# zacharie12/Hypernet-image-captioning

Measured on AMD Instinct MI355X. Metric: training images/sec at 1/2/4/8 MI355X, Flickr30k GRU+hypernet bs=128, higher is better.
Workload: dtype f32; 1 GPU; Flickr30k-shaped GRU+additive-attention decoder + hypernet (3 style domains), full training step (fwd, CE, bwd, clip 5.0, Adam); per_gpu_batch=128, global_batch=128, T=20, P=49, D=2048, F=200, E=200, H=200, V=9684, hypernet_params=144906720, parallelism=dp1, launch=eager, next_theta_in_adam_pass=True, next_precompute_beside_adam=True, spinup_steps=0, deterministic_gradients=True

## Files before the change

hypernet-image-captioning_amd/caphn/_lib.py:

```python
import ctypes as C
import os

import torch

_HERE = os.path.dirname(os.path.abspath(__file__))
LIB_PATH = os.environ.get("CAPHN_LIB_PATH") or os.path.join(_HERE, "libcaphn.so")
MAX_HEADS = 8

c_fp = C.c_void_p


class HyperDesc(C.Structure):
    _fields_ = [("he", C.c_int), ("n_heads", C.c_int),
                ("k", C.c_int * MAX_HEADS), ("w", C.c_int * MAX_HEADS),
                ("base_w0", c_fp), ("base_b0", c_fp), ("base_w2", c_fp), ("base_b2", c_fp),
                ("w1", c_fp * MAX_HEADS), ("b1", c_fp * MAX_HEADS),
                ("w2", c_fp * MAX_HEADS), ("b2", c_fp * MAX_HEADS),
                ("d_in", C.c_int), ("d_mid", C.c_int)]


class HyperGrads(C.Structure):
    _fields_ = [("g_base_w0", c_fp), ("g_base_b0", c_fp), ("g_base_w2", c_fp), ("g_base_b2", c_fp),
                ("g_w1", c_fp * MAX_HEADS), ("g_b1", c_fp * MAX_HEADS),
                ("g_w2", c_fp * MAX_HEADS), ("g_b2", c_fp * MAX_HEADS),
# ... 90 lines not shown
    "caphn_colsum_workspace_bytes": (C.c_size_t, [C.c_int, C.c_int]),
    "caphn_linear_wgrad_f32": (C.c_int, [C.c_int, C.c_int, C.c_int, c_fp, C.c_int, c_fp, C.c_int, c_fp, C.c_int, c_fp, c_fp, c_fp]),
    "caphn_colsum_f32": (C.c_int, [C.c_int, C.c_int, c_fp, C.c_int, c_fp, c_fp, c_fp]),
    "caphn_hyper_acts_floats": (C.c_int, [C.POINTER(HyperDesc)]),
    "caphn_hyper_forward": (C.c_int, [C.POINTER(HyperDesc), c_fp, c_fp, c_fp, c_fp]),
    "caphn_hyper_backward_workspace_bytes": (C.c_size_t, [C.POINTER(HyperDesc)]),
    "caphn_hyper_backward": (C.c_int, [C.POINTER(HyperDesc), c_fp, c_fp, C.POINTER(HyperGrads), c_fp, c_fp]),
    "caphn_decoder_workspace_bytes": (C.c_size_t, [C.POINTER(DecoderDims)]),
    "caphn_decoder_forward": (C.c_int, [C.POINTER(DecoderDims), C.POINTER(DecoderParams), c_fp, c_fp,
                                        c_fp, c_fp, c_fp, c_fp]),
    "caphn_decoder_pair_prep": (C.c_int, [C.POINTER(DecoderDims), C.POINTER(DecoderParams), c_fp, c_fp]),
    "caphn_decoder_pair_pack_desc": (C.c_int, [C.POINTER(DecoderDims), c_fp, C.POINTER(PairPack)]),
    "caphn_decoder_precompute": (C.c_int, [C.POINTER(DecoderDims), C.POINTER(DecoderParams), c_fp, c_fp, c_fp, c_fp]),
    "caphn_decoder_inputs": (C.c_int, [C.POINTER(DecoderDims), C.POINTER(DecoderParams), c_fp, c_fp, c_fp]),
    "caphn_decoder_lookup": (C.c_int, [C.POINTER(DecoderDims), C.POINTER(DecoderParams), c_fp, c_fp, c_fp]),
    "caphn_decoder_prepare_rows": (C.c_int, [C.POINTER(DecoderDims), c_fp, C.c_int64, c_fp, c_fp]),
    "caphn_decoder_forward_sampled": (C.c_int, [C.POINTER(DecoderDims), C.POINTER(DecoderParams), c_fp, c_fp,
                                                C.c_char_p, c_fp, c_fp, c_fp, c_fp]),
    "caphn_decoder_forward_sampled_train": (C.c_int, [C.POINTER(DecoderDims), C.POINTER(DecoderParams), c_fp, c_fp,
                                                      C.c_char_p, c_fp, c_fp, c_fp, c_fp]),
    "caphn_decoder_backward": (C.c_int, [C.POINTER(DecoderDims), C.POINTER(DecoderParams), c_fp, c_fp,
                                         c_fp, c_fp, C.POINTER(DecoderGrads), c_fp, c_fp]),
    "caphn_decoder_hyper_backward": (C.c_int, [C.POINTER(DecoderDims), C.POINTER(DecoderParams), c_fp, c_fp,
                                               c_fp, c_fp, C.POINTER(DecoderGrads), c_fp,
                                               C.POINTER(HyperDesc), c_fp, C.POINTER(HyperGrads), c_fp, c_fp]),
    "caphn_decoder_backward_milestone": (C.c_int, [C.c_int, c_fp]),
    "caphn_decoder_search_workspace_bytes": (C.c_size_t, [C.POINTER(DecoderDims), C.POINTER(SearchCfg)]),
    "caphn_decoder_search_begin": (C.c_int, [C.POINTER(DecoderDims), C.POINTER(DecoderParams), C.POINTER(SearchCfg),
                                             c_fp, c_fp, c_fp, c_fp]),
    "caphn_decoder_search_steps": (C.c_int, [C.POINTER(DecoderDims), C.POINTER(DecoderParams), C.POINTER(SearchCfg),
                                             C.c_int, C.c_int, c_fp, c_fp, c_fp, c_fp]),
    "caphn_decoder_search_result": (C.c_int, [C.POINTER(DecoderDims), C.POINTER(SearchCfg), C.c_int, c_fp, c_fp,
                                              c_fp, c_fp, c_fp, c_fp, c_fp, c_fp]),
    "caphn_plain_workspace_bytes": (C.c_size_t, [C.POINTER(PlainDims)]),
    "caphn_plain_forward": (C.c_int, [C.POINTER(PlainDims), C.POINTER(PlainParams), c_fp, c_fp, c_fp, c_fp, c_fp, c_fp, c_fp]),
    "caphn_bahdanau_fwd": (C.c_int, [C.c_int] * 4 + [c_fp] * 8),
    "caphn_bahdanau_bwd": (C.c_int, [C.c_int] * 4 + [c_fp] * 12),
    "caphn_plain_forward_sampled": (C.c_int, [C.POINTER(PlainDims), C.POINTER(PlainParams), c_fp, c_fp, c_fp, C.c_uint64, c_fp, c_fp,
                                               c_fp, c_fp]),
    "caphn_plain_backward": (C.c_int, [C.POINTER(PlainDims), C.POINTER(PlainParams), c_fp, c_fp, c_fp, c_fp, c_fp,
                                       C.POINTER(PlainGrads), c_fp, c_fp]),
    "caphn_layernorm_fwd": (C.c_int, [C.c_int, C.c_int, c_fp, c_fp, c_fp, C.c_float, c_fp, c_fp, c_fp, c_fp]),
    "caphn_layernorm_bwd_workspace_bytes": (C.c_size_t, [C.c_int, C.c_int]),
    "caphn_layernorm_bwd": (C.c_int, [C.c_int, C.c_int, c_fp, c_fp, c_fp, c_fp, c_fp, c_fp, c_fp, c_fp, c_fp, c_fp]),
    "caphn_attention_supported": (C.c_int, [C.POINTER(AttnDims)]),
    "caphn_attention_fwd": (C.c_int, [C.POINTER(AttnDims), c_fp, c_fp, c_fp, c_fp, c_fp, c_fp, c_fp, c_fp]),
    "caphn_attention_bwd": (C.c_int, [C.POINTER(AttnDims), c_fp, c_fp, c_fp, c_fp, c_fp, c_fp, c_fp, c_fp, c_fp, c_fp, c_fp, c_fp]),
    "caphn_ce_workspace_bytes": (C.c_size_t, [C.c_int]),
    "caphn_cross_entropy_rows": (C.c_int, [C.c_int, C.c_int, c_fp, c_fp, C.c_int64, c_fp, C.c_int, c_fp, c_fp, c_fp]),
    "caphn_cross_entropy_rows_ld": (C.c_int, [C.c_int, C.c_int, C.c_int, c_fp, c_fp, C.c_int64, c_fp, C.c_int, c_fp, c_fp, c_fp]),
    "caphn_cross_entropy_finish": (C.c_int, [C.c_int, c_fp, c_fp, c_fp, c_fp]),
    "caphn_decoder_profile_ptr": (C.c_void_p, [C.POINTER(DecoderDims), c_fp]),
    "caphn_decoder_rowcount_ptr": (C.c_void_p, [C.POINTER(DecoderDims), c_fp]),
    "caphn_cross_entropy_fwd_bwd": (C.c_int, [C.c_int, C.c_int, c_fp, c_fp, C.c_int64, c_fp, c_fp, C.c_int, c_fp, c_fp]),
    "caphn_embedding_gather": (C.c_int, [C.c_int, C.c_int, c_fp, c_fp, c_fp, c_fp]),
    "caphn_embedding_scatter_add": (C.c_int, [C.c_int, C.c_int, c_fp, c_fp, c_fp, c_fp]),
    "caphn_embedding_scatter_add_v": (C.c_int, [C.c_int, C.c_int, C.c_int, c_fp, c_fp, c_fp, c_fp]),
    "caphn_sumsq_blocks": (C.c_int, [C.c_size_t]),
    "caphn_sumsq_f32": (C.c_int, [C.c_size_t, c_fp, c_fp, c_fp]),
    "caphn_rank_sumsq_f32": (C.c_int, [C.c_int, C.c_int, C.c_int, c_fp, C.c_size_t, c_fp, C.c_size_t,
                                       c_fp, c_fp, c_fp]),
    "caphn_rank_sumsq_multi_f32": (C.c_int, [C.c_int, C.c_int, C.POINTER(C.c_int), C.POINTER(C.c_int),
                                             C.POINTER(C.c_void_p), C.POINTER(C.c_size_t), C.POINTER(C.c_void_p),
                                             C.POINTER(C.c_size_t), c_fp, c_fp, c_fp]),
    "caphn_grad_norm_workspace_bytes": (C.c_size_t, [C.c_size_t, C.c_int, C.c_int]),
    "caphn_grad_norm_coef": (C.c_int, [C.c_size_t, c_fp, C.c_int, C.c_int, C.POINTER(C.c_int), C.POINTER(C.c_int),
                                       C.POINTER(C.c_void_p), C.POINTER(C.c_size_t), C.POINTER(C.c_void_p),
                                       C.POINTER(C.c_size_t), C.c_double, C.c_double, c_fp, c_fp, c_fp]),
    "caphn_clip_coef": (C.c_int, [C.c_int, c_fp, c_fp, C.c_double, C.c_double, c_fp, c_fp]),
    "caphn_adam_dense_f32": (C.c_int, [C.c_size_t, c_fp, c_fp, c_fp, c_fp, c_fp, C.POINTER(AdamHParams), c_fp]),
    "caphn_grad_norm_adam_dense": (C.c_int, [C.c_size_t, c_fp, c_fp, c_fp, c_fp, C.c_int, C.c_int, C.POINTER(C.c_int), C.POINTER(C.c_int),
                                             C.POINTER(C.c_void_p), C.POINTER(C.c_size_t), C.POINTER(C.c_void_p), C.POINTER(C.c_size_t),
                                             C.c_double, C.c_double, c_fp, c_fp, C.POINTER(AdamHParams), C.c_int, c_fp, c_fp, c_fp, c_fp]),
    "caphn_grad_norm_multi_workspace_bytes": (C.c_size_t, [C.c_int, C.POINTER(C.c_size_t), C.c_int, C.c_int]),
    "caphn_grad_norm_multi": (C.c_int, [C.c_int, C.POINTER(C.c_void_p), C.POINTER(C.c_size_t), C.c_int, C.c_int,
                                        C.POINTER(C.c_int), C.POINTER(C.c_int), C.POINTER(C.c_void_p), C.POINTER(C.c_size_t),
                                        C.POINTER(C.c_void_p), C.POINTER(C.c_size_t), C.c_double, C.c_double, c_fp, c_fp, c_fp]),
    "caphn_adam_multi_f32": (C.c_int, [C.c_int, C.POINTER(C.c_void_p), C.POINTER(C.c_void_p), C.POINTER(C.c_void_p),
                                       C.POINTER(C.c_void_p), C.POINTER(C.c_size_t), c_fp, C.POINTER(AdamHParams), c_fp]),
    "caphn_adam_rank_f32": (C.c_int, [C.c_int, C.c_int, C.c_int, c_fp, c_fp, c_fp, c_fp, C.c_size_t,
                                      c_fp, C.c_size_t, c_fp, C.POINTER(AdamHParams), c_fp]),
    "caphn_adam_rank_gemv_f32": (C.c_int, [C.c_int, C.c_int, C.c_int, c_fp, c_fp, c_fp, c_fp, C.c_size_t,
                                           c_fp, C.c_size_t, c_fp, C.POINTER(AdamHParams), c_fp, c_fp, c_fp, c_fp]),
    "caphn_adam_rank_multi_f32": (C.c_int, [C.c_int, C.c_int, C.POINTER(RankJob), c_fp, C.POINTER(AdamHParams), c_fp]),
    "caphn_adam_rank_lag_f32": (C.c_int, [C.c_int, C.c_int, C.c_int, c_fp, c_fp, c_fp, c_fp, c_fp, c_fp, C.POINTER(AdamHParams),
                                          C.POINTER(RankLag), c_fp, c_fp, c_fp, c_fp]),
    "caphn_adam_rank_lag_multi_f32": (C.c_int, [C.c_int, C.c_int, C.POINTER(RankJob), C.POINTER(RankLag), c_fp,
                                                C.POINTER(AdamHParams), c_fp]),
    "caphn_adam_rank_settle_f32": (C.c_int, [C.c_int, C.c_int, c_fp, c_fp, C.c_float, C.c_float, C.POINTER(RankLag), c_fp]),
    "caphn_lazy_moments_period": (C.c_int, []),
    "caphn_hyper_forward_acts": (C.c_int, [C.POINTER(HyperDesc), c_fp, c_fp, c_fp]),
    "caphn_stream_copy_f32": (C.c_int, [C.c_size_t, c_fp, c_fp, c_fp]),
    "caphn_outer_f32": (C.c_int, [C.c_int, C.c_int, c_fp, c_fp, c_fp, c_fp]),
    "caphn_tune": (C.c_int, [C.c_int, C.c_int]),
}

_ERR = {-1: "CAPHN_EINVAL (bad argument)", -2: "CAPHN_ELAUNCH (HIP launch error)",
        -3: "CAPHN_ELIMIT (problem exceeds a hardware limit, e.g. 160 KB LDS)",
        -4: "CAPHN_ETIMEOUT (a recurrent kernel's partner workgroup never answered: that step's results are NaN; "
            "sticky until caphn_device_error(1))"}

_lib = None


class CaphnError(RuntimeError):
    pass
# ... 42 lines not shown
```

hypernet-image-captioning_amd/caphn/ops.py:

```python
import ctypes as C
from dataclasses import dataclass
from typing import Dict, List, Optional, Sequence, Tuple

import torch

from . import _lib as L

GEMM_BIAS, GEMM_RELU, GEMM_ACCUM, GEMM_MASK, GEMM_LRELU = 1, 2, 4, 8, 16


def _f32(*shape, device):
    return torch.empty(*shape, dtype=torch.float32, device=device)


def gemm(a: torch.Tensor, b: torch.Tensor, ta: bool = False, tb: bool = False,
         bias: Optional[torch.Tensor] = None, relu: bool = False, out: Optional[torch.Tensor] = None,
         accumulate: bool = False, mask: Optional[torch.Tensor] = None, splitk: int = 1, lrelu: bool = False) -> torch.Tensor:
    lib = L.load()
    assert a.dim() == 2 and b.dim() == 2 and a.stride(1) == 1 and b.stride(1) == 1
    M, K = (a.shape[1], a.shape[0]) if ta else (a.shape[0], a.shape[1])
    N, Kb = (b.shape[0], b.shape[1]) if tb else (b.shape[1], b.shape[0])
    if K != Kb:
        raise L.CaphnError(f"gemm inner dims differ: {K} vs {Kb}")
    if out is None:
# ... 522 lines not shown
    lib = L.load()
    cd = dims.c()
    ps = _dec_struct(L.DecoderParams, dims, params)
    gs = _dec_struct(L.DecoderGrads, dims, grads)
    L.check(lib.caphn_decoder_backward(C.byref(cd), C.byref(ps), L.ptr(features), L.ptr(captions, torch.int64),
                                       L.ptr(dlogits), L.ptr(dalphas, allow_none=True), C.byref(gs),
                                       C.c_void_p(ws.data_ptr()), L.stream_ptr()), "caphn_decoder_backward")


def cross_entropy_fwd_bwd(logits: torch.Tensor, targets: torch.Tensor, ignore_index: int = 0,
                          dlogits: Optional[torch.Tensor] = None, leave_ignored_rows: bool = False):
    lib = L.load()
    V = logits.shape[-1]
    rows = logits.numel() // V
    if dlogits is None:
        dlogits = torch.empty_like(logits)
    ws = torch.empty(lib.caphn_ce_workspace_bytes(rows), dtype=torch.uint8, device=logits.device)
    out = _f32(2, device=logits.device)
    L.check(lib.caphn_cross_entropy_fwd_bwd(rows, V, L.ptr(logits), L.ptr(targets.reshape(-1), torch.int64),
                                            ignore_index, L.ptr(dlogits), L.ptr(out), int(leave_ignored_rows),
                                            C.c_void_p(ws.data_ptr()),
                                            L.stream_ptr()), "caphn_cross_entropy_fwd_bwd")
    return out, dlogits


def cross_entropy_rows(logits: torch.Tensor, targets: torch.Tensor, ignore_index: int, dlogits: torch.Tensor,
                       ws: torch.Tensor, leave_ignored_rows: bool = False, n_valid_ptr: Optional[int] = None, V: Optional[int] = None) -> None:
    lib = L.load()
    ld = logits.shape[-1]
    rows = logits.numel() // ld
    V = ld if V is None else int(V)
    assert dlogits.shape[-1] == ld and V <= ld
    L.check(lib.caphn_cross_entropy_rows_ld(rows, V, ld, L.ptr(logits), L.ptr(targets.reshape(-1), torch.int64), ignore_index,
                                            L.ptr(dlogits), int(leave_ignored_rows),
                                            C.c_void_p(n_valid_ptr) if n_valid_ptr else None, C.c_void_p(ws.data_ptr()),
                                            L.stream_ptr()), "caphn_cross_entropy_rows_ld")


def cross_entropy_finish(rows: int, ws: torch.Tensor, out: torch.Tensor, n_valid_ptr: Optional[int] = None) -> None:
    lib = L.load()
    L.check(lib.caphn_cross_entropy_finish(rows, C.c_void_p(n_valid_ptr) if n_valid_ptr else None, L.ptr(out),
                                           C.c_void_p(ws.data_ptr()), L.stream_ptr()), "caphn_cross_entropy_finish")


def ce_workspace(rows: int, device) -> torch.Tensor:
    return torch.empty(L.load().caphn_ce_workspace_bytes(rows), dtype=torch.uint8, device=device)


def decoder_rowcount_ptr(dims: DecDims, ws: torch.Tensor) -> int:
    cd = dims.c()
    return int(L.load().caphn_decoder_rowcount_ptr(C.byref(cd), C.c_void_p(ws.data_ptr())) or 0)


def embedding_gather(table: torch.Tensor, idx: torch.Tensor) -> torch.Tensor:
    lib = L.load()
    rows, E = idx.numel(), table.shape[1]
    out = _f32(rows, E, device=table.device)
    L.check(lib.caphn_embedding_gather(rows, E, L.ptr(table), L.ptr(idx.reshape(-1), torch.int64), L.ptr(out),
                                       L.stream_ptr()), "caphn_embedding_gather")
    return out


def embedding_scatter_add(g: torch.Tensor, idx: torch.Tensor, table_grad: torch.Tensor) -> None:
    lib = L.load()
    rows, E = g.shape
    L.check(lib.caphn_embedding_scatter_add_v(rows, E, int(table_grad.shape[0]), L.ptr(g), L.ptr(idx.reshape(-1), torch.int64),
                                              L.ptr(table_grad), L.stream_ptr()), "caphn_embedding_scatter_add_v")


def sumsq_partials(x: torch.Tensor, partial: Optional[torch.Tensor] = None) -> torch.Tensor:
    lib = L.load()
    nb = lib.caphn_sumsq_blocks(x.numel())
    if partial is None:
        partial = torch.empty(nb, dtype=torch.float64, device=x.device)
    L.check(lib.caphn_sumsq_f32(x.numel(), L.ptr(x), L.ptr(partial, torch.float64), L.stream_ptr()), "caphn_sumsq_f32")
    return partial[:nb]


def rank_sumsq(gfac: torch.Tensor, afac: torch.Tensor, acc: torch.Tensor) -> None:
    lib = L.load()
    R, rows = gfac.shape
    k = afac.shape[1]
    ws = torch.empty(2 * R * R, dtype=torch.float64, device=gfac.device)
    L.check(lib.caphn_rank_sumsq_f32(R, rows, k, gfac.data_ptr(), gfac.stride(0), afac.data_ptr(), afac.stride(0),
                                     L.ptr(acc, torch.float64), L.ptr(ws, torch.float64), L.stream_ptr()),
            "caphn_rank_sumsq_f32")


def rank_sumsq_multi(pairs, acc: torch.Tensor, ws: Optional[torch.Tensor] = None) -> None:
    lib = L.load()
    n = len(pairs)
    R = pairs[0][0].shape[0]
    if ws is None:
        ws = torch.empty(2 * R * R * n, dtype=torch.float64, device=acc.device)
    rows = (C.c_int * n)(*[g.shape[1] for g, _ in pairs])
    ks = (C.c_int * n)(*[a.shape[1] for _, a in pairs])
    gp = (C.c_void_p * n)(*[g.data_ptr() for g, _ in pairs])
    ap = (C.c_void_p * n)(*[a.data_ptr() for _, a in pairs])
    ldg = (C.c_size_t * n)(*[g.stride(0) for g, _ in pairs])
    lda = (C.c_size_t * n)(*[a.stride(0) for _, a in pairs])
    L.check(lib.caphn_rank_sumsq_multi_f32(R, n, rows, ks, gp, ldg, ap, lda, L.ptr(acc, torch.float64),
                                           L.ptr(ws, torch.float64), L.stream_ptr()), "caphn_rank_sumsq_multi_f32")


class GradNorm:

# ... 466 lines not shown
```

hypernet-image-captioning_amd/csrc/decoder.hip:

```cpp
#include "common.h"
#include "decoder_internal.h"
#include "gemm_internal.h"
#include <algorithm>
#include <initializer_list>
#include <mutex>

int g_tune_deterministic = 0;
int g_tune_rec_pair = 1;
int g_tune_rec_rotate = 1;
int g_tune_vocab_order = 1;
int g_tune_branch_mask = 7;
int g_tune_splitk_target = 1280;
int g_tune_chain_main = 0;
int g_tune_hops = 0;
int g_tune_fork = 4;
int g_tune_join_chain = 0;
int g_tune_sk_dhs = 0, g_tune_sk_vocab_w = 0;
#define RUN(x) do { int _rc = (x); if (_rc != CAPHN_OK) return _rc; } while (0)

namespace {

struct Side {
    hipStream_t st[3];
    enum { D_FORK = 0, D_JOIN = 1, D_X = 4, D_MS = 10, D_PRE_F = 14, D_PRE_ALL = 15, D_COUNT = 16 };
    struct Dep { hipEvent_t ev; unsigned seq = 0; bool by_value = false; };
    Dep deps[D_COUNT];
    unsigned* vals = nullptr;
    unsigned counter = 0;
    bool values = false;
    bool pre_valid = false;
    const void* pre_ws = nullptr;
    bool ready = false, on = false;
    bool forked[3] = {false, false, false};
    hipStream_t main = nullptr;
    int init() {
        if (ready) return CAPHN_OK;
        static std::mutex mu;
        std::lock_guard<std::mutex> lock(mu);
        if (ready) return CAPHN_OK;
        for (auto& s : st) if (hipStreamCreateWithFlags(&s, hipStreamNonBlocking) != hipSuccess) return CAPHN_ELAUNCH;
        for (auto& d : deps) if (hipEventCreateWithFlags(&d.ev, hipEventDisableTiming) != hipSuccess) return CAPHN_ELAUNCH;
        void* p = nullptr;
        if (hipMalloc(&p, sizeof(unsigned) * D_COUNT) == hipSuccess && hipMemset(p, 0, sizeof(unsigned) * D_COUNT) == hipSuccess)
            vals = static_cast<unsigned*>(p);
        else (void)hipGetLastError();
        ready = true;
        return CAPHN_OK;
    }
    int post(int slot, hipStream_t from) {
        Dep& d = deps[slot];
        if (values) {
            d.seq = ++counter; d.by_value = true;
            return hipStreamWriteValue32(from, vals + slot, d.seq, 0) == hipSuccess ? CAPHN_OK : CAPHN_ELAUNCH;
        }
        d.by_value = false;
        return hipEventRecord(d.ev, from) == hipSuccess ? CAPHN_OK : CAPHN_ELAUNCH;
    }
    int await(int slot, hipStream_t to) {
        Dep& d = deps[slot];
        if (d.by_value)
            return hipStreamWaitValue32(to, vals + slot, d.seq, hipStreamWaitValueGte, 0xffffffffu) == hipSuccess ? CAPHN_OK : CAPHN_ELAUNCH;
        return hipStreamWaitEvent(to, d.ev, 0) == hipSuccess ? CAPHN_OK : CAPHN_ELAUNCH;
    }
    int milestone(int k, hipStream_t from) {
        if (init() != CAPHN_OK) return CAPHN_ELAUNCH;
        return post(D_MS + k, from);
    }
    int begin(hipStream_t m, bool enable) {
        main = m; on = enable;
// ... 15 lines not shown
        if (post(D_FORK, main) != CAPHN_OK) return CAPHN_ELAUNCH;
        for (int i : ids) {
            if (!((g_tune_branch_mask >> i) & 1)) continue;
            if (await(D_FORK, st[i]) != CAPHN_OK) return CAPHN_ELAUNCH;
            forked[i] = true;
        }
        return CAPHN_OK;
    }
    int jointo(int i) {
        if (!on || !((g_tune_branch_mask >> i) & 1)) return CAPHN_OK;
        forked[i] = false;
        if (post(D_JOIN + i, st[i]) != CAPHN_OK) return CAPHN_ELAUNCH;
        return await(D_JOIN + i, main);
    }
    int join_into(int i, int j) {
        if (!on || !((g_tune_branch_mask >> i) & 1)) return CAPHN_OK;
        if (!((g_tune_branch_mask >> j) & 1)) return jointo(i);
        forked[i] = false;
        if (post(D_JOIN + i, st[i]) != CAPHN_OK) return CAPHN_ELAUNCH;
        return await(D_JOIN + i, st[j]);
    }
    struct Scope {
        Side& s;
        explicit Scope(Side& side) : s(side) {}
        ~Scope() { for (int i = 0; i < 3; ++i) if (s.on && s.forked[i]) (void)s.jointo(i); }
    };
    hipStream_t xfrom[6] = {nullptr, nullptr, nullptr, nullptr, nullptr, nullptr};
    int record(int k, hipStream_t from) {
        if (!on) return CAPHN_OK;
        xfrom[k] = from;
        return post(D_X + k, from);
    }
    int wait(int k, hipStream_t to) {
        if (!on || xfrom[k] == to) return CAPHN_OK;
        return await(D_X + k, to);
    }
    int dep(hipStream_t from, hipStream_t to, int k) {
        if (!on || from == to) return CAPHN_OK;
        if (post(D_X + k, from) != CAPHN_OK) return CAPHN_ELAUNCH;
        return await(D_X + k, to);
    }
};
constexpr int MAX_DEVICES = 64;
Side g_sides[MAX_DEVICES];
inline Side* side_here() {
    int dev = 0;
    if (hipGetDevice(&dev) != hipSuccess || dev < 0 || dev >= MAX_DEVICES) return nullptr;
    return &g_sides[dev];
}

struct Ws {
    size_t Y1, f, meanf, h0, c0, Waf, G, Xe, Xg, Hs, Hprev, gates, hn, Cs, Cprev, uah, alphas, idx;
    size_t dHs, dgi, dgh, duah, de, dh0, dc0, ctx, dctx, dXe, dWaf, dmeanf, df, dY1, apart, vtmp, colws, colws_s[3], prof, rowmap;
    size_t xch, xch_floats;
    size_t wp;
    size_t H0s, dH0, h0L, dcarry, tgi, tgh, tmpA, tmpB;
    size_t Lin[CAPHN_MAX_DEC_LAYERS - 1], Lgates[CAPHN_MAX_DEC_LAYERS - 1], Lhn[CAPHN_MAX_DEC_LAYERS - 1],
           Ldgi[CAPHN_MAX_DEC_LAYERS - 1], Ldgh[CAPHN_MAX_DEC_LAYERS - 1];
    int L1;
    size_t total;
    int npc, pchunk, NG, arows;
};
inline bool use_pair(const caphn_decoder_dims* d) {
    const int NG = d->cell == CAPHN_CELL_LSTM ? 4 : 3;
    return g_tune_rec_pair && d->T > 1 && d->layers <= 1 && caphn_rec_pair_resident_gates(d->P, d->H, NG) >= 0;
}

inline size_t up4(size_t v) { return (v + 3) & ~(size_t)3; }

inline Ws layout(const caphn_decoder_dims* d) {
    Ws w;
    const size_t B = d->B, T = d->T, P = d->P, F = d->F, E = d->E, H = d->H, V = d->V, D = d->D;
    const bool lstm = d->cell == CAPHN_CELL_LSTM, raw = d->raw_features != 0;
    const size_t NG = lstm ? 4 : 3;
    w.NG = (int)NG;
    size_t o = 0;
    auto take = [&](size_t n) { size_t r = o; o += up4(n); return r; };
    w.Y1 = take(raw ? 0 : B * P * F); w.f = take(raw ? 0 : B * P * F); w.meanf = take(B * F); w.h0 = take(B * H);
    w.c0 = take(lstm ? B * H : 0);
    w.Waf = take(B * P * H); w.G = take(B * P * NG * H); w.Xe = take(B * T * (E + F)); w.Xg = take(B * T * NG * H);
    w.Hs = take(B * T * H); w.Hprev = take(B * T * H); w.gates = take(B * T * NG * H); w.hn = take(lstm ? 0 : B * T * H);
    w.Cs = take(lstm ? B * T * H : 0); w.Cprev = take(lstm ? B * T * H : 0);
    w.uah = take(B * T * H); w.alphas = take(B * T * P); w.idx = take(2 * B * T);
    w.dHs = take(B * T * H); w.dgi = take(B * T * NG * H); w.dgh = take(lstm ? 0 : B * T * NG * H); w.duah = take(B * T * H);
    w.de = take(B * T * P); w.dh0 = take(B * H); w.dc0 = take(lstm ? B * H : 0);
    w.ctx = w.Xe + E; w.dctx = take(raw ? 0 : B * T * F);
    w.dXe = take(B * T * E); w.dWaf = take(B * P * H); w.dmeanf = take(raw ? 0 : 2 * B * F); w.df = take(raw ? 0 : B * P * F);
    w.dY1 = take(raw ? 0 : B * P * F);
    w.pchunk = 1; w.npc = (int)((P + w.pchunk - 1) / w.pchunk);
    const size_t arows = std::max<size_t>(std::max<size_t>(w.npc, (size_t)caphn_rec_bwd_groups((int)P, (int)H)),
                                          (size_t)caphn_rec_pair_bwd_groups((int)P, (int)H));
    w.arows = (int)arows;
    w.apart = take(B * arows * (H + 1)); w.vtmp = take(H + 1);
    size_t cs = 0;
    auto need = [&](size_t M, size_t N) { cs = std::max(cs, caphn_colsum_workspace_bytes((int)M, (int)N) / sizeof(float)); };
    need(B * T, V); need(B * T, NG * H); need(B * T, H); need(B * P, H); need(B * P, F); need(B, H);
    need(B * arows, H + 1);
    if (d->layers > 1) need(B * (T + 1), 3 * H);
    w.colws = take(cs);
    {
        size_t c2 = 0;
        auto need2 = [&](size_t M, size_t N) { c2 = std::max(c2, caphn_colsum_workspace_bytes((int)M, (int)N) / sizeof(float)); };
        need2(B * T, NG * H); need2(B * T, H); need2(B * P, H); need2(B * P, F); need2(B, H); need2(B * arows, H + 1);
        if (d->layers > 1) need2(B * (T + 1), 3 * H);
        for (int i = 0; i < 3; ++i) w.colws_s[i] = take(c2);
    }
    w.prof = take(64);
    w.rowmap = take(B * T + 4);
    w.xch_floats = caphn_rec_pair_xch_bytes((int)B, (int)P, (int)H) / sizeof(float);
    w.xch = take(2 * w.xch_floats);
    o = (o + 31) & ~(size_t)31;
    w.wp = take(caphn_rec_pair_wp_floats((int)H, (int)NG));
    w.L1 = d->layers > 1 ? d->layers - 1 : 0;
    {
        const size_t on = w.L1 > 0 ? 1 : 0, S = T + 1;
        w.H0s = take(on * B * T * H); w.dH0 = take(on * B * T * H); w.h0L = take(on * B * H); w.dcarry = take(on * B * H);
        w.tgi = take(on * B * 3 * H); w.tgh = take(on * B * 3 * H); w.tmpA = take(on * B * H); w.tmpB = take(on * B * H);
        for (int l = 0; l < CAPHN_MAX_DEC_LAYERS - 1; ++l) {
            const size_t u = l < w.L1 ? 1 : 0;
            w.Lin[l] = take(u * B * S * H); w.Lgates[l] = take(u * B * S * 3 * H); w.Lhn[l] = take(u * B * S * H);
            w.Ldgi[l] = take(u * B * S * 3 * H); w.Ldgh[l] = take(u * B * S * 3 * H);
        }
    }
    w.total = o;
    (void)D;
    return w;
}

__global__ __launch_bounds__(1024) void valid_rows_kernel(int n, const int64_t* __restrict__ tgt, int64_t ignore, int* __restrict__ map) {
    __shared__ int wsum[16];
    __shared__ int base_s;
    const int tid = threadIdx.x, lane = tid & 63, wave = tid >> 6;
    if (tid == 0) base_s = 0;
    __syncthreads();
    for (int c0 = 0; c0 < n; c0 += 1024) {
        const int i = c0 + tid;
        const int v = (i < n && tgt[i] != ignore) ? 1 : 0;
        const unsigned long long ball = __ballot(v);
        const int before = __popcll(ball & ((1ull << lane) - 1ull));
        if (lane == 0) wsum[wave] = __popcll(ball);
        __syncthreads();
        int woff = 0, tot = 0;
        for (int q = 0; q < 16; ++q) { if (q < wave) woff += wsum[q]; tot += wsum[q]; }
        const int base = base_s;
        if (v) map[4 + base + woff + before] = i;
        __syncthreads();
        if (tid == 0) base_s = base + tot;
        __syncthreads();
    }
    if (tid == 0) map[0] = base_s;
}

__global__ void copy2_kernel(const float* __restrict__ src, int n, float* __restrict__ a, float* __restrict__ b) {
    const int i = blockIdx.x * blockDim.x + threadIdx.x;
    if (i < n) a[i] = src[i];
    else if (i == n) b[0] = src[n];
}

__global__ __launch_bounds__(256) void teacher_inputs_kernel(int T, int E, const int64_t* __restrict__ caps, const float* __restrict__ table,
                                                            int64_t* __restrict__ idx, float* __restrict__ out, int ostride) {
    const int i = blockIdx.x, t = i % T;
    const int64_t id = t < 2 ? (int64_t)-1 : caps[i - 1];
    if (threadIdx.x == 0) idx[i] = id;
    for (int e = threadIdx.x; e < E; e += 256) out[(size_t)i * ostride + e] = id < 0 ? 0.f : table[(size_t)id * E + e];
}

inline bool dims_ok(const caphn_decoder_dims* d) {
    if (d && !(d->dropout_p >= 0.f && d->dropout_p < 1.f)) return false;
    if (!(d && d->B > 0 && d->T > 0 && d->P > 0 && d->D > 0 && d->F > 0 && d->E > 0 && d->H > 0 && d->V > 0)) return false;
    if (d->cell != CAPHN_CELL_GRU && d->cell != CAPHN_CELL_LSTM) return false;
    if (d->raw_features && d->F != d->D) return false;
    if (d->layers < 0 || d->layers > CAPHN_MAX_DEC_LAYERS) return false;
    if (d->layers > 1 && d->cell != CAPHN_CELL_GRU) return false;
    if (d->logits_ld != 0 && d->logits_ld < d->V) return false;
    return true;
}
inline bool layer_params_ok(const caphn_decoder_dims* d, const caphn_decoder_params* p) {
    for (int l = 0; l + 1 < d->layers; ++l)
        if (!p->lw_ih[l] || !p->lw_hh[l] || !p->lb_ih[l] || !p->lb_hh[l]) return false;
    return true;
}

inline int pick_splitk(int M, int N, int K) {
    if (g_tune_deterministic) return 1;
    const long t128 = (long)((M + 127) / 128) * ((N + 127) / 128);
    if (t128 >= 1024) return 1;
    const long t64 = (long)((M + 63) / 64) * ((N + 63) / 64);
    const int nslab = (K + 31) / 32;
    long s = (g_tune_splitk_target + t64 - 1) / t64;
    if (s > nslab / 8) s = nslab / 8;
    if (s < 1) s = 1;
    if (s > 64) s = 64;
    return (int)s;
}


inline int gemm_auto(int ta, int tb, int M, int N, int K, const float* A, int lda, const float* B, int ldb,
                     float* C, int ldc, const float* bias, int flags, hipStream_t s,
                     const int* rowmap = nullptr, int map_mode = 0, bool prezeroed = false) {
    int sk = pick_splitk(M, N, K);
    if (rowmap) {
        if (sk > 1 && !prezeroed) {
            if (ldc == N) { RUN(caphn_zero_f32(C, (size_t)M * N, s)); }
            else if (hipMemset2DAsync(C, sizeof(float) * ldc, 0, sizeof(float) * N, M, s) != hipSuccess) return CAPHN_ELAUNCH;
        }
        return caphn_gemm_mapped(ta, tb, M, N, K, A, lda, B, ldb, C, ldc, bias, flags, sk, rowmap + 4, rowmap, map_mode, s);
    }
    if (sk > 1 && (flags & ~CAPHN_GEMM_BIAS) == 0) {
        if (prezeroed) {
        } else if (ldc == N) {
            RUN(caphn_zero_f32(C, (size_t)M * N, s));
        } else {
            if (hipMemset2DAsync(C, sizeof(float) * ldc, 0, sizeof(float) * N, M, s) != hipSuccess) return CAPHN_ELAUNCH;
        }
        return caphn_gemm_f32(ta, tb, M, N, K, A, lda, B, ldb, C, ldc, bias, nullptr, 0, flags, sk, s);
    }
    return caphn_gemm_f32(ta, tb, M, N, K, A, lda, B, ldb, C, ldc, bias, nullptr, 0, flags, 1, s);
}

inline int wgrad_bias(int M, int N, int K, const float* A, int lda, const float* B, int ldb, float* dW, int ldc, float* db,
                      const int* rowmap, void* cws, hipStream_t s, bool prezeroed) {
    int sk = pick_splitk(M, N, K);
    if (rowmap && g_tune_sk_vocab_w > 0 && !g_tune_deterministic) sk = g_tune_sk_vocab_w;
    return caphn_gemm_tn_colsum(M, N, K, A, lda, B, ldb, dW, ldc, db, sk, rowmap, cws, prezeroed, s);
}

static int decoder_precompute(const caphn_decoder_dims* d, const caphn_decoder_params* p, const Ws& w, float* ws,
                              const float* features, const float** f_out, hipStream_t s, int parts = 3, bool mark = false) {
    const int B = d->B, P = d->P, D = d->D, F = d->F, E = d->E, H = d->H;
    const bool lstm = d->cell == CAPHN_CELL_LSTM, raw = d->raw_features != 0;
    const int BP = B * P, GH = w.NG * H, EF = E + F;
    const float* f = raw ? features : ws + w.f;
    *f_out = f;
    if ((parts & 1) && !raw) {
        RUN(caphn_gemm_f32(0, 1, BP, F, D, features, D, p->fc0_w, D, ws + w.Y1, F, p->fc0_b, nullptr, 0,
                           CAPHN_GEMM_BIAS | CAPHN_GEMM_RELU, 1, s));
        RUN(caphn_gemm_f32(0, 1, BP, F, F, ws + w.Y1, F, p->fc2_w, F, ws + w.f, F, p->fc2_b, nullptr, 0, CAPHN_GEMM_BIAS, 1, s));
    }
    Side* sdp = side_here();
    if (!sdp) return CAPHN_ELAUNCH;
    Side& sd = *sdp;
    RUN(sd.begin(s, g_tune_fork != 0 && (parts & 1) && !mark));
    Side::Scope scope(sd);
    if (mark) RUN(sd.post(Side::D_PRE_F, s));
    if (parts & 1) {
        RUN(sd.fork_many({0, 1}));
        RUN(caphn_launch_init_state(B, P, F, H, f, p->inith_w, p->inith_b, lstm ? p->initc_w : nullptr, lstm ? p->initc_b : nullptr,
                                    ws + w.meanf, ws + w.h0, lstm ? ws + w.c0 : nullptr, sd.s(0)));
        RUN(caphn_gemm_f32(0, 1, BP, H, F, f, F, p->Wa_w, F, ws + w.Waf, H, p->Wa_b, nullptr, 0, CAPHN_GEMM_BIAS, 1, sd.s(1)));
    }
    if (parts & 2)
        RUN(caphn_gemm_f32(0, 1, BP, GH, F, f, F, p->w_ih + E, EF, ws + w.G, GH, nullptr, nullptr, 0, 0, 1, s));
    if (parts & 1) { RUN(sd.jointo(0)); RUN(sd.jointo(1)); }
    return CAPHN_OK;
}

__global__ __launch_bounds__(256) void next_token_kernel(int B, int T, int V, int mode, int col,
                                                         const int64_t* __restrict__ caps, const float* __restrict__ logits,
                                                         int64_t* __restrict__ idx_out, int ostride) {
    __shared__ float bv[4];
    __shared__ int bi[4];
    const int b = blockIdx.x, tid = threadIdx.x;
    int64_t* idx = idx_out + (size_t)b * ostride - b;
    if (mode == 0) { if (tid == 0) idx[b] = -1; return; }
    if (mode == 1) { if (tid == 0) idx[b] = caps[(size_t)b * T + col]; return; }
    const float* row = logits + ((size_t)b * T + col) * V;
    float best = -INFINITY; int besti = 0x7fffffff;
    for (int v = tid; v < V; v += 256) { const float x = row[v]; if (x > best) { best = x; besti = v; } }
#pragma unroll
    for (int m = 32; m >= 1; m >>= 1) {
        const float ob = __shfl_xor(best, m, 64); const int oi = __shfl_xor(besti, m, 64);
        if (ob > best || (ob == best && oi < besti)) { best = ob; besti = oi; }
    }
    if ((tid & 63) == 0) { bv[tid >> 6] = best; bi[tid >> 6] = besti; }
    __syncthreads();
    if (tid == 0) {
// ... 7 lines not shown
    const int B = d->B, H = d->H, G3 = 3 * d->H;
    const float* in = hin; int in_ld = hin_ld;
    for (int l = 0; l < w.L1; ++l) {
        const bool last = l == w.L1 - 1;
        float* out = last ? hout : ws + ((l & 1) ? w.tmpB : w.tmpA);
        const int out_ld = last ? hout_ld : H;
        RUN(caphn_gemm_f32(0, 1, B, G3, H, in, in_ld, p->lw_ih[l], H, ws + w.tgi, G3, p->lb_ih[l], nullptr, 0, CAPHN_GEMM_BIAS, 1, s));
        RUN(caphn_gemm_f32(0, 1, B, G3, H, in, in_ld, p->lw_hh[l], H, ws + w.tgh, G3, p->lb_hh[l], nullptr, 0, CAPHN_GEMM_BIAS, 1, s));
        LayerFwdArgs a;
        a.B = B; a.H = H; a.S = d->T + 1; a.slot = slot;
        a.gi = ws + w.tgi; a.gh = ws + w.tgh; a.hin = in; a.hin_ld = in_ld; a.hout = out; a.hout_ld = out_ld;
        a.sin = ws + w.Lin[l]; a.sgates = ws + w.Lgates[l]; a.shn = ws + w.Lhn[l];
        if (last && slot > 0) { a.drop_p = d->dropout_p; a.drop_seed = d->dropout_seed; a.T = d->T; a.t = slot - 1; }
        RUN(caphn_launch_layer_gru_fwd(a, s));
        in = out; in_ld = out_ld;
    }
    return CAPHN_OK;
}

static int layers_backward(const caphn_decoder_dims* d, const caphn_decoder_params* p, const Ws& w, float* ws, int slot,
                           const float* d1, int d1_ld, const float* d2, float* dout, int dout_ld, hipStream_t s) {
    const int B = d->B, H = d->H, G3 = 3 * d->H, S = d->T + 1;
    for (int l = w.L1 - 1; l >= 0; --l) {
        float* o = l == 0 ? dout : ws + ((l & 1) ? w.tmpB : w.tmpA);
        const int o_ld = l == 0 ? dout_ld : H;
        LayerBwdArgs a;
        a.B = B; a.H = H; a.S = S; a.slot = slot;
        a.d1 = d1; a.d1_ld = d1_ld; a.d2 = d2;
        a.sin = ws + w.Lin[l]; a.sgates = ws + w.Lgates[l]; a.shn = ws + w.Lhn[l];
        a.dgi = ws + w.Ldgi[l]; a.dgh = ws + w.Ldgh[l]; a.dout = o; a.dout_ld = o_ld;
        if (l == w.L1 - 1 && slot > 0) { a.drop_p = d->dropout_p; a.drop_seed = d->dropout_seed; a.T = d->T; a.t = slot - 1; }
        RUN(caphn_launch_layer_gru_bwd(a, s));
        RUN(caphn_gemm_f32(0, 0, B, H, G3, ws + w.Ldgi[l] + (size_t)slot * G3, S * G3, p->lw_ih[l], H, o, o_ld, nullptr, nullptr, 0,
                           CAPHN_GEMM_ACCUM, 1, s));
        RUN(caphn_gemm_f32(0, 0, B, H, G3, ws + w.Ldgh[l] + (size_t)slot * G3, S * G3, p->lw_hh[l], H, o, o_ld, nullptr, nullptr, 0,
                           CAPHN_GEMM_ACCUM, 1, s));
        d1 = o; d1_ld = o_ld; d2 = nullptr;
    }
    return CAPHN_OK;
}

}

extern "C" size_t caphn_decoder_workspace_bytes(const caphn_decoder_dims* d) {
    if (!dims_ok(d)) return 0;
    return layout(d).total * sizeof(float);
}

extern "C" const int* caphn_decoder_rowcount_ptr(const caphn_decoder_dims* d, void* ws_) {
    if (!dims_ok(d) || !ws_) return nullptr;
    return reinterpret_cast<const int*>(static_cast<float*>(ws_) + layout(d).rowmap);
}

extern "C" unsigned long long* caphn_decoder_profile_ptr(const caphn_decoder_dims* d, void* ws_) {
    if (!dims_ok(d) || !ws_) return nullptr;
    return reinterpret_cast<unsigned long long*>(static_cast<float*>(ws_) + layout(d).prof);
}

extern "C" int caphn_decoder_prepare_rows(const caphn_decoder_dims* d, const int64_t* targets, int64_t ignore_index,
                                          void* ws_, caphn_stream_t stream) {
    if (!dims_ok(d) || !targets || !ws_) return CAPHN_EINVAL;
    const Ws w = layout(d);
    hipLaunchKernelGGL(valid_rows_kernel, dim3(1), dim3(1024), 0, static_cast<hipStream_t>(stream), d->B * d->T, targets,
                       ignore_index, reinterpret_cast<int*>(static_cast<float*>(ws_) + w.rowmap));
    return caphn_launch_status();
}

static int decoder_inputs(const caphn_decoder_dims* d, const caphn_decoder_params* p, const Ws& w, float* ws,
                          const int64_t* captions, hipStream_t s, int parts = 3) {
    const int BT = d->B * d->T, E = d->E, GH = w.NG * d->H, EF = d->E + d->F;
    int64_t* idx = reinterpret_cast<int64_t*>(ws + w.idx);
    if ((parts & 1) && !(d->precomputed & 64))
        hipLaunchKernelGGL(teacher_inputs_kernel, dim3(BT), dim3(256), 0, s, d->T, E, captions, p->embed_w, idx, ws + w.Xe, EF);
    if (parts & 2)
    RUN(caphn_gemm_f32(0, 1, BT, GH, E, ws + w.Xe, EF, p->w_ih, EF, ws + w.Xg, GH, p->b_ih, nullptr, 0, CAPHN_GEMM_BIAS, 1, s));
    return CAPHN_OK;
}

extern "C" int caphn_decoder_precompute(const caphn_decoder_dims* d, const caphn_decoder_params* p, const float* features,
                                        const int64_t* captions, void* ws_, caphn_stream_t stream) {
    if (!dims_ok(d) || !p || !features || !ws_) return CAPHN_EINVAL;
    const bool raw = d->raw_features != 0;
    if (!raw && (!p->fc0_w || !p->fc0_b || !p->fc2_w || !p->fc2_b)) return CAPHN_EINVAL;
    if (d->cell == CAPHN_CELL_LSTM && (!p->initc_w || !p->initc_b)) return CAPHN_EINVAL;
    const Ws w = layout(d);
    hipStream_t s = static_cast<hipStream_t>(stream);
    const float* f = nullptr;
    RUN(decoder_precompute(d, p, w, static_cast<float*>(ws_), features, &f, s, (captions ? 3 : 1) & ~(d->precomputed & 1), true));
    if (captions && !(d->precomputed & 4)) RUN(decoder_inputs(d, p, w, static_cast<float*>(ws_), captions, s));
    Side* sd = side_here();
    if (!sd || sd->post(Side::D_PRE_ALL, s) != CAPHN_OK) return CAPHN_ELAUNCH;
    sd->pre_valid = true;
    sd->pre_ws = ws_;
    return caphn_launch_status();
}

extern "C" int caphn_decoder_pair_prep(const caphn_decoder_dims* d, const caphn_decoder_params* p, void* ws_, caphn_stream_t stream) {
    if (!dims_ok(d) || !p || !ws_ || !p->Ua_w || !use_pair(d)) return CAPHN_EINVAL;
    const Ws w = layout(d);
    float* ws = static_cast<float*>(ws_);
    RUN(caphn_launch_rec_pair_prep(reinterpret_cast<unsigned long long*>(ws + w.xch), 2 * w.xch_floats * sizeof(float) / sizeof(unsigned long long),
                                   p->Ua_w, nullptr, d->H, w.NG, ws + w.wp, ws + w.dHs, (size_t)d->B * d->T * d->H,
                                   static_cast<hipStream_t>(stream)));
    return caphn_launch_status();
}
extern "C" int caphn_decoder_pair_pack_desc(const caphn_decoder_dims* d, void* ws_, caphn_pair_pack* out) {
    if (!dims_ok(d) || !ws_ || !out || !use_pair(d)) return CAPHN_EINVAL;
    const Ws w = layout(d);
    out->wp = static_cast<float*>(ws_) + w.wp;
    out->H = d->H; out->HA = caphn_rec_pair_half_a(d->H); out->pitch = caphn_rec_pair_pitch(d->H);
    out->hrows = (w.NG + 1) * out->HA;
    return CAPHN_OK;
}

extern "C" int caphn_decoder_inputs(const caphn_decoder_dims* d, const caphn_decoder_params* p, const int64_t* captions,
                                    void* ws_, caphn_stream_t stream) {
    if (!dims_ok(d) || !p || !captions || !ws_ || !p->embed_w || !p->w_ih || !p->b_ih) return CAPHN_EINVAL;
// ... 24 lines not shown
    if (RG < 0) return CAPHN_ELIMIT;
    if (lstm && (!p->initc_w || !p->initc_b)) return CAPHN_EINVAL;
    if (!raw && (!p->fc0_w || !p->fc0_b || !p->fc2_w || !p->fc2_b)) return CAPHN_EINVAL;
    if (!layer_params_ok(d, p)) return CAPHN_EINVAL;

    const float* f = nullptr;
    const int pc = d->precomputed;
    if (!(pc & 4)) RUN(decoder_inputs(d, p, w, ws, captions, s));
    Side* sdw = (pc & 16) ? side_here() : nullptr;
    if (pc & 16) {
        if (!sdw || !sdw->pre_valid || sdw->pre_ws != ws_) return CAPHN_EINVAL;
        RUN(sdw->await(Side::D_PRE_F, s));
    }
    RUN(decoder_precompute(d, p, w, ws, features, &f, s, ((pc & 1) ? 0 : 1) | ((pc & 2) ? 0 : 2)));
    if (pc & 16)
        RUN(sdw->await(Side::D_PRE_ALL, s));

    RecFwdArgs a;
    a.B = B; a.T = T; a.P = P; a.H = H; a.RG = RG;
    a.Waf = ws + w.Waf; a.G = ws + w.G; a.Xg = ws + w.Xg; a.h0 = ws + w.h0; a.c0 = ws + w.c0;
    a.W_hh = p->w_hh; a.b_hh = p->b_hh; a.U_a = p->Ua_w; a.b_Ua = p->Ua_b; a.v_a = p->va_w; a.b_va = p->va_b;
    a.Hs = ws + w.Hs; a.Hprev = ws + w.Hprev; a.alphas = ws + w.alphas; a.gates = ws + w.gates; a.hn = ws + w.hn;
    a.Cs = ws + w.Cs; a.Cprev = ws + w.Cprev; a.uah = ws + w.uah;
    a.vecW = (H % 4 == 0) && caphn_aligned16(p->w_hh) && caphn_aligned16(p->Ua_w);
    a.vecS = (H % 4 == 0) && caphn_aligned16(ws);
    a.prof = reinterpret_cast<unsigned long long*>(ws + w.prof);
    a.rotate = g_tune_rec_rotate;
    a.drop_p = d->dropout_p; a.drop_seed = d->dropout_seed;
    if (pair) {
        a.xch = reinterpret_cast<unsigned long long*>(ws + w.xch);
        a.WP = ws + w.wp; a.wp_pitch = caphn_rec_pair_pitch(H);
        if (!(pc & 128))
        RUN(caphn_launch_rec_pair_prep(a.xch, 2 * w.xch_floats * sizeof(float) / sizeof(unsigned long long), p->Ua_w, p->w_hh, H, w.NG,
                                       ws + w.wp, (pc & 8) ? ws + w.dHs : nullptr, (size_t)BT * H, s));
        RUN(caphn_launch_rec_pair_fwd(a, lstm, s));
    } else if (w.L1 > 0) {
        RUN(layers_forward(d, p, w, ws, 0, ws + w.h0, H, ws + w.h0L, H, s));
        a.h0 = ws + w.h0L; a.Hs = ws + w.H0s; a.Hsrc = ws + w.Hs; a.drop_p = 0.f;
        for (int t = 0; t < T; ++t) {
            a.t0 = t; a.t1 = t + 1;
            RUN(caphn_launch_rec_fwd(a, lstm, s));
            RUN(layers_forward(d, p, w, ws, t + 1, ws + w.H0s + (size_t)t * H, T * H, ws + w.Hs + (size_t)t * H, T * H, s));
        }
    } else
    RUN(caphn_launch_rec_fwd(a, lstm, s));
    if ((pc & 8) && !pair) RUN(caphn_zero_f32(ws + w.dHs, (size_t)BT * H, s));

    const int LV = d->logits_ld > 0 ? d->logits_ld : V;
    if (d->row_subset)
        RUN(caphn_gemm_mapped(0, 1, BT, V, H, ws + w.Hs, H, p->out_w, H, logits, LV, p->out_b, CAPHN_GEMM_BIAS, 1,
                              reinterpret_cast<const int*>(ws + w.rowmap) + 4, reinterpret_cast<const int*>(ws + w.rowmap), 1, s));
    else
        RUN(caphn_gemm_f32(0, 1, BT, V, H, ws + w.Hs, H, p->out_w, H, logits, LV, p->out_b, nullptr, 0, CAPHN_GEMM_BIAS, 1, s));
    if (pc & 32) RUN(caphn_launch_ctx(B, T, P, F, ws + w.alphas, f, ws + w.ctx, EF, s));
    if (alphas)
        if (hipMemcpyAsync(alphas, ws + w.alphas, sizeof(float) * (size_t)BT * P, hipMemcpyDeviceToDevice, s) != hipSuccess)
            return CAPHN_ELAUNCH;
    return caphn_launch_status();
}

struct HyperHook { const caphn_hyper_desc* hd; const float* acts; const caphn_hyper_grads* hg; void* ws; };
static int decoder_backward_impl(const caphn_decoder_dims* d, const caphn_decoder_params* p,
                                 const float* features, const int64_t* captions, float* dlogits, const float* dalphas,
                                 const caphn_decoder_grads* g, void* ws_, const HyperHook* hook, caphn_stream_t stream);
extern "C" int caphn_decoder_backward(const caphn_decoder_dims* d, const caphn_decoder_params* p,
                                      const float* features, const int64_t* captions,
                                      float* dlogits, const float* dalphas,
                                      const caphn_decoder_grads* g, void* ws_, caphn_stream_t stream) {
    return decoder_backward_impl(d, p, features, captions, dlogits, dalphas, g, ws_, nullptr, stream);
}
extern "C" int caphn_decoder_hyper_backward(const caphn_decoder_dims* d, const caphn_decoder_params* p,
                                            const float* features, const int64_t* captions,
                                            float* dlogits, const float* dalphas,
                                            const caphn_decoder_grads* g, void* ws_,
                                            const caphn_hyper_desc* hd, const float* acts, const caphn_hyper_grads* hg, void* hyper_ws,
                                            caphn_stream_t stream) {
    if (!hd || !acts || !hg || !hyper_ws || !g) return CAPHN_EINVAL;
    const size_t NG = d && d->cell == CAPHN_CELL_LSTM ? 4 : 3;
    if (d) {
        const size_t GH = NG * d->H, EF = (size_t)d->E + d->F;
        if (g->w_hh != g->w_ih + GH * EF || g->b_ih != g->w_hh + GH * d->H || g->b_hh != g->b_ih + GH) return CAPHN_EINVAL;
    }
    HyperHook hook{hd, acts, hg, hyper_ws};
    return decoder_backward_impl(d, p, features, captions, dlogits, dalphas, g, ws_, &hook, stream);
}
static int decoder_backward_impl(const caphn_decoder_dims* d, const caphn_decoder_params* p,
                                 const float* features, const int64_t* captions, float* dlogits, const float* dalphas,
                                 const caphn_decoder_grads* g, void* ws_, const HyperHook* hook, caphn_stream_t stream) {
    if (!dims_ok(d) || !p || !features || !captions || !dlogits || !g || !ws_) return CAPHN_EINVAL;
    hipStream_t s = static_cast<hipStream_t>(stream);
    const Ws w = layout(d);
    float* ws = static_cast<float*>(ws_);
    const int B = d->B, T = d->T, P = d->P, D = d->D, F = d->F, E = d->E, H = d->H, V = d->V;
    const bool lstm = d->cell == CAPHN_CELL_LSTM, raw = d->raw_features != 0;
    const int BP = B * P, BT = B * T, GH = w.NG * H, EF = E + F;
    const bool pair = use_pair(d);
    const int RG = pair ? caphn_rec_pair_resident_gates(P, H, w.NG) : caphn_rec_resident_gates(P, H, w.NG);
    if (RG < 0) return CAPHN_ELIMIT;
    if (lstm && (!g->initc_w || !g->initc_b)) return CAPHN_EINVAL;
    if (!raw && (!g->fc0_w || !g->fc0_b || !g->fc2_w || !g->fc2_b)) return CAPHN_EINVAL;
    if (!layer_params_ok(d, p)) return CAPHN_EINVAL;
    for (int l = 0; l < w.L1; ++l) if (!g->lw_ih[l] || !g->lw_hh[l] || !g->lb_ih[l] || !g->lb_hh[l]) return CAPHN_EINVAL;
    void* cws = ws + w.colws;
    const int64_t* idx = reinterpret_cast<const int64_t*>(ws + w.idx);
    const float* f = raw ? features : ws + w.f;
    float* dgi = ws + w.dgi;
    float* dgh = lstm ? dgi : ws + w.dgh;

    Side* sdp = side_here();
    if (!sdp) return CAPHN_ELAUNCH;
    Side& sd = *sdp;
    RUN(sd.begin(s, g_tune_fork != 0));
    Side::Scope scope(sd);
    void* cw0 = ws + w.colws_s[0]; void* cw1 = ws + w.colws_s[1]; void* cw2 = ws + w.colws_s[2];

    const int* rmap = d->row_subset ? reinterpret_cast<const int*>(ws + w.rowmap) : nullptr;
    const int LV = d->logits_ld > 0 ? d->logits_ld : V;
    const int fork_mode = g_tune_fork == 4 ? (pair ? 2 : 1) : g_tune_fork;
    const bool late = fork_mode != 2;
    const bool gz = d->grads_zeroed != 0;
    const bool wg_first = !late && g_tune_vocab_order == 0;
    if (wg_first) {
        RUN(sd.forkto(0));
        RUN(wgrad_bias(V, H, BT, dlogits, LV, ws + w.Hs, H, g->out_w, H, g->out_b, rmap, cws, sd.s(0), gz));
        RUN(sd.milestone(CAPHN_MS_VOCAB, sd.s(0)));
    }
    const bool dhs_zero = (d->precomputed & 8) != 0;
    bool ctx_side = false;
    if (rmap) {
        if (!dhs_zero) RUN(caphn_zero_f32(ws + w.dHs, (size_t)BT * H, s));
        RUN(caphn_gemm_mapped(0, 0, BT, H, V, dlogits, LV, p->out_w, H, ws + w.dHs, H, nullptr, 0,
                              (g_tune_sk_dhs > 0 && !g_tune_deterministic) ? g_tune_sk_dhs : pick_splitk(BT, H, V),
                              rmap + 4, rmap, 1, s));
    } else
    RUN(gemm_auto(0, 0, BT, H, V, dlogits, LV, p->out_w, H, ws + w.dHs, H, nullptr, 0, s, nullptr, 0, dhs_zero));
    if (!late && !wg_first) {
        if (!(d->precomputed & 32) && sd.s(0) != s && sd.s(2) != s) {
            RUN(sd.fork_many({0, 2}));
            RUN(caphn_launch_ctx(B, T, P, F, ws + w.alphas, f, ws + w.ctx, EF, sd.s(2)));
            RUN(sd.record(5, sd.s(2)));
            ctx_side = true;
        } else
        RUN(sd.forkto(0));
        RUN(wgrad_bias(V, H, BT, dlogits, LV, ws + w.Hs, H, g->out_w, H, g->out_b, rmap, cws, sd.s(0), gz));
        RUN(sd.milestone(CAPHN_MS_VOCAB, sd.s(0)));
    }

    RecBwdArgs a;
    a.B = B; a.T = T; a.P = P; a.H = H; a.RG = RG;
    a.Waf = ws + w.Waf; a.G = ws + w.G; a.W_hh = p->w_hh; a.U_a = p->Ua_w; a.v_a = p->va_w;
    a.Hprev = ws + w.Hprev; a.alphas = ws + w.alphas; a.gates = ws + w.gates; a.hn = ws + w.hn; a.uah = ws + w.uah;
    a.Cs = ws + w.Cs; a.Cprev = ws + w.Cprev;
    a.dHs = ws + w.dHs; a.dalphas = dalphas;
    a.dgi = dgi; a.dgh = dgh; a.duah = ws + w.duah; a.de = ws + w.de; a.dh0 = ws + w.dh0; a.dc0 = ws + w.dc0;
    a.vecW = (H % 4 == 0) && caphn_aligned16(p->w_hh) && caphn_aligned16(p->Ua_w);
    a.vecS = (H % 4 == 0) && caphn_aligned16(ws);
    a.prof = reinterpret_cast<unsigned long long*>(ws + w.prof) + 8;
    a.rotate = g_tune_rec_rotate;
    a.drop_p = d->dropout_p; a.drop_seed = d->dropout_seed;
    const int ang = w.L1 > 0 ? 0 : pair ? caphn_rec_pair_bwd_groups(P, H) : caphn_rec_bwd_groups(P, H);
    if (ang > 0) { a.dWaf = ws + w.dWaf; a.apart = ws + w.apart; }
    if (w.L1 > 0) {
        RUN(caphn_zero_f32(ws + w.dcarry, (size_t)B * H, s));
        a.dHs = ws + w.dH0; a.dh0 = ws + w.dcarry; a.drop_p = 0.f;
        for (int t = T - 1; t >= 0; --t) {
            RUN(layers_backward(d, p, w, ws, t + 1, ws + w.dHs + (size_t)t * H, T * H, ws + w.dcarry, ws + w.dH0 + (size_t)t * H, T * H, s));
            a.t0 = t; a.t1 = t + 1;
            RUN(caphn_launch_rec_bwd(a, lstm, s));
        }
        RUN(layers_backward(d, p, w, ws, 0, ws + w.dcarry, H, nullptr, ws + w.dh0, H, s));
    } else if (pair) {
        a.xch = reinterpret_cast<unsigned long long*>(ws + w.xch) + w.xch_floats * sizeof(float) / sizeof(unsigned long long);
        a.apart_rows = ang;
        a.WP = ws + w.wp; a.wp_pitch = caphn_rec_pair_pitch(H);
        if (!raw) { a.inith_w = p->inith_w; a.initc_w = lstm ? p->initc_w : nullptr; a.dmean_part = ws + w.dmeanf; a.F = F; }
        RUN(caphn_launch_rec_pair_bwd(a, lstm, s));
    } else
    RUN(caphn_launch_rec_bwd(a, lstm, s));

    hipStream_t b0 = sd.s(0), b1 = sd.s(1), b2 = sd.s(2);
    const bool t_main = hook != nullptr && g_tune_chain_main != 0;
    hipStream_t sT = t_main ? s : b1, sF = t_main ? b1 : s;
    const bool hold_big = late && !raw && fork_mode == 3;
    RUN(sd.fork_many({0, 1, 2}));
    if (late && !hold_big) {
        RUN(wgrad_bias(V, H, BT, dlogits, LV, ws + w.Hs, H, g->out_w, H, g->out_b, rmap, cws, b0, gz));
        RUN(sd.milestone(CAPHN_MS_VOCAB, b0));
    }
    if (ctx_side) RUN(sd.wait(5, sT));
    else if (!(d->precomputed & 32)) RUN(caphn_launch_ctx(B, T, P, F, ws + w.alphas, f, ws + w.ctx, EF, sT));
    if (lstm) RUN(gemm_auto(1, 0, GH, EF, BT, dgi, GH, ws + w.Xe, EF, g->w_ih, EF, nullptr, 0, sT, nullptr, 0, gz));
    else RUN(wgrad_bias(GH, EF, BT, dgi, GH, ws + w.Xe, EF, g->w_ih, EF, g->b_ih, nullptr, cw1, sT, gz));
    RUN(wgrad_bias(GH, H, BT, dgh, GH, ws + w.Hprev, H, g->w_hh, H, g->b_hh, nullptr, cw2, b2, gz));
    if (lstm) RUN(caphn_colsum_f32(BT, GH, dgi, GH, g->b_ih, cw2, b2));
    RUN(sd.record(3, b2));
    hipStream_t se = late ? b2 : b0;
    RUN(caphn_gemm_f32(0, 0, BT, E, GH, dgi, GH, p->w_ih, EF, ws + w.dXe, E, nullptr, nullptr, 0, 0, 1, se));
    if (!gz) RUN(caphn_zero_f32(g->embed_w, (size_t)V * E, se));
    RUN(caphn_embedding_scatter_add_v(BT, E, V, ws + w.dXe, idx, g->embed_w, se));
    RUN(sd.milestone(CAPHN_MS_EMBED, se));
    RUN(sd.wait(3, sT));
    RUN(sd.milestone(CAPHN_MS_DTHETA, sT));
    if (hook && !hold_big) {
        RUN(caphn_hyper_backward(hook->hd, g->w_ih, hook->acts, hook->hg, hook->ws, sT));
    }
    if (!hold_big) RUN(sd.milestone(CAPHN_MS_HYPER, sT));
    if (!raw) {
        RUN(caphn_gemm_f32(0, 0, BT, F, GH, dgi, GH, p->w_ih + E, EF, ws + w.dctx, F, nullptr, nullptr, 0, 0, 1, sF));
        if (!pair)
            RUN(caphn_launch_dmean(B, H, F, ws + w.dh0, p->inith_w, lstm ? ws + w.dc0 : nullptr, lstm ? p->initc_w : nullptr,
                                   ws + w.dmeanf, sF));
    }
    AttnGradArgs ag;
    ag.T = T; ag.P = P; ag.H = H; ag.pchunk = w.pchunk;
    ag.Waf = ws + w.Waf; ag.uah = ws + w.uah; ag.de = ws + w.de; ag.v_a = p->va_w;
    ag.dWaf = ws + w.dWaf; ag.part = ws + w.apart;
    if (ang == 0) RUN(caphn_launch_attn_param_grads(ag, B, w.npc, sF));
    RUN(sd.record(2, sF));
    RUN(wgrad_bias(H, H, BT, ws + w.duah, H, ws + w.Hprev, H, g->Ua_w, H, g->Ua_b, nullptr, cws, b0, gz));
    for (int l = 0; l < w.L1; ++l) {
        const int BS = B * (T + 1), G3 = 3 * H;
        RUN(wgrad_bias(G3, H, BS, ws + w.Ldgi[l], G3, ws + w.Lin[l], H, g->lw_ih[l], H, g->lb_ih[l], nullptr, cws, b0, gz));
        RUN(wgrad_bias(G3, H, BS, ws + w.Ldgh[l], G3, ws + w.Lin[l], H, g->lw_hh[l], H, g->lb_hh[l], nullptr, cws, b0, gz));
    }
    RUN(wgrad_bias(H, F, B, ws + w.dh0, H, ws + w.meanf, F, g->inith_w, F, g->inith_b, nullptr, cws, b0, gz));
    if (lstm) RUN(wgrad_bias(H, F, B, ws + w.dc0, H, ws + w.meanf, F, g->initc_w, F, g->initc_b, nullptr, cws, b0, gz));
    if (!raw) {
        RUN(caphn_launch_df(B, T, P, F, ws + w.alphas, ws + w.dctx, ws + w.dmeanf, ws + w.df, sF, pair ? ws + w.dmeanf + (size_t)B * F : nullptr));
        RUN(caphn_gemm_f32(0, 0, BP, F, H, ws + w.dWaf, H, p->Wa_w, F, ws + w.df, F, nullptr, nullptr, 0, CAPHN_GEMM_ACCUM, 1, sF));
        RUN(sd.record(4, sF));
        if (hold_big) {
            RUN(sd.wait(4, b0));
            RUN(wgrad_bias(V, H, BT, dlogits, LV, ws + w.Hs, H, g->out_w, H, g->out_b, rmap, cws, b0, gz));
            RUN(sd.milestone(CAPHN_MS_VOCAB, b0));
            if (hook) {
                RUN(sd.wait(4, sT));
                RUN(caphn_hyper_backward(hook->hd, g->w_ih, hook->acts, hook->hg, hook->ws, sT));
            }
            RUN(sd.milestone(CAPHN_MS_HYPER, sT));
        }
        RUN(caphn_gemm_f32(0, 0, BP, F, F, ws + w.df, F, p->fc2_w, F, ws + w.dY1, F, nullptr, ws + w.Y1, F, CAPHN_GEMM_MASK, 1, sF));
        RUN(wgrad_bias(F, D, BP, ws + w.dY1, F, features, D, g->fc0_w, D, g->fc0_b, nullptr, cw0, sF, gz));
    }
    RUN(sd.wait(2, b2));
    RUN(caphn_colsum_f32(B * (ang > 0 ? ang : w.npc), H + 1, ws + w.apart, H + 1, ws + w.vtmp, cw2, b2));
    hipLaunchKernelGGL(copy2_kernel, dim3((H + 256) / 256), dim3(256), 0, b2, ws + w.vtmp, H, g->va_w, g->va_b);
    RUN(wgrad_bias(H, F, BP, ws + w.dWaf, H, f, F, g->Wa_w, F, g->Wa_b, nullptr, cw2, b2, gz));
    if (!raw) {
        RUN(sd.wait(4, b2));
        RUN(wgrad_bias(F, F, BP, ws + w.df, F, ws + w.Y1, F, g->fc2_w, F, g->fc2_b, nullptr, cw2, b2, gz));
    }
    if (g_tune_join_chain) { RUN(sd.join_into(0, 1)); RUN(sd.join_into(2, 1)); RUN(sd.jointo(1)); }
    else { RUN(sd.jointo(0)); RUN(sd.jointo(1)); RUN(sd.jointo(2)); }
    (void)captions;
    return caphn_launch_status();
}

extern "C" int caphn_decoder_backward_milestone(int which, caphn_stream_t waiter) {
    if (which < 0 || which >= CAPHN_MS_COUNT) return CAPHN_EINVAL;
    Side* sd = side_here();
    if (!sd) return CAPHN_ELAUNCH;
    if (!sd->ready) return CAPHN_OK;
    return sd->await(Side::D_MS + which, static_cast<hipStream_t>(waiter));
}

extern "C" int caphn_decoder_forward_sampled(const caphn_decoder_dims* d, const caphn_decoder_params* p,
                                             const float* features, const int64_t* captions,
                                             const unsigned char* use_sampling,
                                             float* logits, float* alphas, void* ws_, caphn_stream_t stream) {
    if (!dims_ok(d) || !p || !features || !captions || !use_sampling || !logits || !ws_ || d->logits_ld != 0) return CAPHN_EINVAL;
    if (d->dropout_p > 0.f) return CAPHN_EINVAL;
    hipStream_t s = static_cast<hipStream_t>(stream);
    const Ws w = layout(d);
    float* ws = static_cast<float*>(ws_);
    const int B = d->B, T = d->T, P = d->P, E = d->E, F = d->F, H = d->H, V = d->V;
    const bool lstm = d->cell == CAPHN_CELL_LSTM;
    const int GH = w.NG * H, EF = E + F;
    const int RG = caphn_rec_resident_gates(P, H, w.NG);
    if (RG < 0) return CAPHN_ELIMIT;
    if (lstm && (!p->initc_w || !p->initc_b)) return CAPHN_EINVAL;
    const float* f = nullptr;
    if (!layer_params_ok(d, p)) return CAPHN_EINVAL;
    RUN(decoder_precompute(d, p, w, ws, features, &f, s));
    if (w.L1 > 0) RUN(layers_forward(d, p, w, ws, 0, ws + w.h0, H, ws + w.h0L, H, s));
    int64_t* idx = reinterpret_cast<int64_t*>(ws + w.idx);
    int src_mode = 0, src_col = 0;
// ... 210 lines not shown
```

hypernet-image-captioning_amd/csrc/decoder_internal.h:

```cpp
#pragma once
#include "common.h"

struct RecFwdArgs {
    int B, T, P, H;
    int RG;
    const float* Waf;
    const float* G;
    const float* Xg;
    const float* h0;
    const float* c0;
    const float* W_hh; const float* b_hh;
    const float* U_a; const float* b_Ua;
    const float* v_a; const float* b_va;
    float* Hs; float* Hprev;
    float* alphas;
    float* gates;
    float* hn;
    float* Cs; float* Cprev;
    float* uah;
    unsigned long long* prof;
    int vecW, vecS, rotate;
    int slab_div = 1;
    unsigned long long* xch = nullptr;
    const float* WP = nullptr; int wp_pitch = 0;
    int t0 = 0, t1 = 0;
    float drop_p = 0.f; unsigned long long drop_seed = 0;
    int waf_lds = 0;
    int wc_rows = 0;
    unsigned epoch = 0; int* err = nullptr; long long xlimit = 0;
    const float* Hsrc = nullptr;
};
struct RecBwdArgs {
    int B, T, P, H;
    int RG;
    const float* Waf; const float* G;
    const float* W_hh; const float* U_a; const float* v_a;
    const float* Hprev; const float* alphas; const float* gates; const float* hn; const float* uah;
    const float* Cs; const float* Cprev;
    const float* dHs;
    const float* dalphas;
    float* dgi; float* dgh;
    float* duah;
    float* de;
    float* dh0;
    float* dc0;
    unsigned long long* prof;
    int vecW, vecS, rotate;
    float* dWaf = nullptr; float* apart = nullptr;
    unsigned long long* xch = nullptr;
    const float* WP = nullptr; int wp_pitch = 0;
    int apart_rows = 0;
    float drop_p = 0.f; unsigned long long drop_seed = 0;
    unsigned epoch = 0; int* err = nullptr; long long xlimit = 0;
    const float* inith_w = nullptr; const float* initc_w = nullptr; float* dmean_part = nullptr; int F = 0;
    int part_rows = 0, wc_rows = 0;
    int t0 = 0, t1 = 0;
};
struct AttnGradArgs {
    int T, P, H, pchunk;
    const float* Waf; const float* uah; const float* de; const float* v_a;
    float* dWaf;
    float* part;
};

struct LayerFwdArgs {
    int B, H, S, slot;
    const float* gi; const float* gh;
    const float* hin; int hin_ld;
    float* hout; int hout_ld;
    float* sin; float* sgates; float* shn;
    float drop_p = 0.f; unsigned long long drop_seed = 0; int T = 1, t = 0;
};
struct LayerBwdArgs {
    int B, H, S, slot;
    const float* d1; int d1_ld; const float* d2;
    const float* sin; const float* sgates; const float* shn;
    float* dgi; float* dgh;
    float* dout; int dout_ld;
    float drop_p = 0.f; unsigned long long drop_seed = 0; int T = 1, t = 0;
};
int caphn_launch_layer_gru_fwd(const LayerFwdArgs& a, hipStream_t s);
int caphn_launch_layer_gru_bwd(const LayerBwdArgs& a, hipStream_t s);

size_t caphn_rec_fwd_lds_bytes(int P, int H, int NG, int RG);
size_t caphn_rec_bwd_lds_bytes(int P, int H, int NG, int RG);
int caphn_rec_resident_gates(int P, int H, int NG);
int caphn_launch_rec_fwd(const RecFwdArgs& a, bool lstm, hipStream_t s);
int caphn_launch_rec_bwd(const RecBwdArgs& a, bool lstm, hipStream_t s);
bool caphn_rec_pair_ok(int P, int H, int NG, int RG);
int caphn_rec_pair_resident_gates(int P, int H, int NG);
size_t caphn_rec_pair_xch_bytes(int B, int P, int H);
int caphn_rec_pair_bwd_groups(int P, int H);
int caphn_rec_pair_pitch(int H);
int caphn_rec_pair_half_a(int H);
size_t caphn_rec_pair_wp_floats(int H, int NG);
int caphn_launch_rec_pair_prep(unsigned long long* xch, size_t nxch, const float* U_a, const float* W_hh, int H, int NG, float* WP,
                               float* zbuf, size_t nz, hipStream_t s);
int caphn_launch_rec_pair_fwd(const RecFwdArgs& a, bool lstm, hipStream_t s);
int caphn_launch_rec_pair_bwd(const RecBwdArgs& a, bool lstm, hipStream_t s);
int caphn_rec_bwd_groups(int P, int H);
int caphn_launch_attn_param_grads(const AttnGradArgs& a, int B, int npc, hipStream_t s);
int caphn_launch_ctx(int B, int T, int P, int F, const float* alphas, const float* f, float* ctx, int ldc, hipStream_t s);
int caphn_launch_df(int B, int T, int P, int F, const float* alphas, const float* dctx, const float* dmean, float* df, hipStream_t s,
                    const float* dmean2 = nullptr);
int caphn_launch_dmean(int B, int H, int F, const float* dh0, const float* Wh, const float* dc0, const float* Wc, float* out, hipStream_t s);
int caphn_launch_init_state(int B, int P, int F, int H, const float* f, const float* Wh, const float* bh, const float* Wc,
                            const float* bc, float* meanf, float* h0, float* c0, hipStream_t s);
int caphn_embedding_gather_strided(int rows, int E, const float* table, const int64_t* idx, int istride, float* out, int ostride, hipStream_t s);
int caphn_launch_mean_p(int B, int P, int F, const float* f, float* out, hipStream_t s);

constexpr int SEARCH_MAX_BEAM = 8;
struct SearchArgs {
    int n_images, beam, max_steps, H;
    int zero_pad_rule;
    int64_t end_token;
    float* h_cur; const float* h_new;
    float* score;
    int64_t* idx;
    const float* cand_val; const int* cand_idx;
    int* k_alive; int* n_comp;
    int64_t* seqs[2];
    int64_t* comp_seqs; int* comp_len; float* comp_score;
};
int caphn_launch_row_topk(int R, int V, int k, const float* logits, const float* score, float* cand_val, int* cand_idx, hipStream_t s);
int caphn_launch_beam_merge(const SearchArgs& a, int step, hipStream_t s);
int caphn_launch_search_init(const SearchArgs& a, const float* h0, int64_t first_token, int lookup_first, hipStream_t s);
int caphn_launch_search_result(const SearchArgs& a, int steps_done, int64_t* out_seq, int* out_len, float* out_score, int* finished,
                               int* n_active, hipStream_t s);
```

hypernet-image-captioning_amd/csrc/gemm_bf16x3.hip:

```cpp
#include "common.h"
#include "gemm_internal.h"
#include "split3.h"
#include <type_traits>

#ifdef CAPHN_GEMM_PROFILE
__device__ unsigned long long d_gemm_prof[10];
__device__ unsigned long long d_gemm_wgt[2 * 8192];
extern "C" int caphn_debug_gemm_wgtimes(unsigned long long* out, int n) {
    return hipMemcpyFromSymbol(out, HIP_SYMBOL(d_gemm_wgt), sizeof(unsigned long long) * 2 * (n < 8192 ? n : 8192)) == hipSuccess ? 0 : -1;
}
#define GSTAMP(i) do { if (gprof) { unsigned long long _n = clock64(); gpc[i] += _n - glast; glast = _n; } } while (0)
extern "C" int caphn_debug_gemm_prof(unsigned long long* out, int reset) {
    if (out && hipMemcpyFromSymbol(out, HIP_SYMBOL(d_gemm_prof), sizeof(unsigned long long) * 10) != hipSuccess) return -1;
    if (reset) { unsigned long long z[10] = {0, 0, 0, 0, 0, 0, 0, 0, 0, 0}; if (hipMemcpyToSymbol(HIP_SYMBOL(d_gemm_prof), z, sizeof(z)) != hipSuccess) return -1; }
    return 0;
}
#else
#define GSTAMP(i) do { } while (0)
#endif

extern int g_tune_gemm_waves;
namespace {

constexpr int BK = 32;
constexpr int PITCH = 32;
__device__ __forceinline__ int kc_off(int row, int k) { return row * PITCH + ((((k >> 3) ^ (row >> 2)) & 3) << 3) + (k & 7); }

template <int BMN, bool KC>
struct TileS {
    static constexpr int NV = BMN / 32;
    static constexpr int PITCHM = BMN + 32;
    static constexpr int PLANE = KC ? BMN * PITCH : BK * PITCHM;
    static constexpr int ELEMS = 3 * PLANE;

    __device__ static __forceinline__ void phys_rows(int (&pr)[NV], int rows, int r0, int tid, const int* __restrict__ rmap,
                                                     bool clamp) {
#pragma unroll
        for (int i = 0; i < NV; ++i) {
            int row = r0 + ((tid + 256 * i) >> 3);
            if (clamp) row = min(row, rows - 1);
            pr[i] = (rmap && row < rows) ? rmap[row] : row;
        }
    }
    __device__ static __forceinline__ void load(f32x4 (&r)[NV], const float* __restrict__ G, int ld,
                                                int rows, int K, int r0, int k0, int vec, int tid,
                                                const int (&pr)[NV], const int* __restrict__ kmap) {
#pragma unroll
        for (int i = 0; i < NV; ++i) {
            f32x4 v = {0.f, 0.f, 0.f, 0.f};
            const int idx = tid + 256 * i;
            if (KC) {
                const int row = r0 + (idx >> 3);
                const int k = k0 + (idx & 7) * 4;
                if (row < rows) {
                    const float* p = G + (size_t)pr[i] * ld + k;
                    if (vec && k + 3 < K) v = *reinterpret_cast<const f32x4*>(p);
                    else {
#pragma unroll
                        for (int e = 0; e < 4; ++e) if (k + e < K) v[e] = p[e];
                    }
                }
            } else {
                const int m = r0 + (idx % (BMN / 4)) * 4;
                const int k = k0 + idx / (BMN / 4);
                if (k < K) {
                    const float* p = G + (size_t)(kmap ? kmap[k] : k) * ld + m;
                    if (vec && m + 3 < rows) v = *reinterpret_cast<const f32x4*>(p);
                    else {
#pragma unroll
                        for (int e = 0; e < 4; ++e) if (m + e < rows) v[e] = p[e];
                    }
                }
            }
            r[i] = v;
// ... 168 lines not shown
    constexpr int TILE_ELEMS = TileA::ELEMS + TileB::ELEMS;
    extern __shared__ __attribute__((aligned(16))) __bf16 lds[];
    __bf16* As = lds;
    __bf16* Bs = lds + TileA::ELEMS;
    __bf16* As1 = DB ? lds + TILE_ELEMS : As;
    __bf16* Bs1 = DB ? lds + TILE_ELEMS + TileA::ELEMS : Bs;

    const bool producer = WS && threadIdx.x >= 256;
    const int tid = WS ? (threadIdx.x & 255) : threadIdx.x, lane = tid & 63, wave = tid >> 6;
    const int wm = wave >> 1, wn = wave & 1;
    const int li = lane & 31, kh = lane >> 5;
#ifdef CAPHN_GEMM_PROFILE
    const unsigned long long gstart = clock64();
    const unsigned gwg = blockIdx.x + gridDim.x * (blockIdx.y + gridDim.y * blockIdx.z);
    if (tid == 0 && gwg < 8192) d_gemm_wgt[2 * gwg] = wall_clock64();
#endif
    int bx = blockIdx.x, by = blockIdx.y, bz = blockIdx.z;
    if (g.flags & (1 << 20)) {
        const int nx = gridDim.x, ny = gridDim.y, nwg = nx * ny * (int)gridDim.z;
        const int orig = bx + nx * (by + ny * bz);
        const int xcd = orig & 7, q = nwg >> 3, r = nwg & 7;
        const int wgid = (xcd < r ? xcd * (q + 1) : r * (q + 1) + (xcd - r) * q) + (orig >> 3);
        if (g.flags & (1 << 22)) { by = wgid % ny; bx = (wgid / ny) % nx; }
        else { bx = wgid % nx; by = (wgid / nx) % ny; }
        bz = wgid / (nx * ny);
    }
    const int m0 = by * BM, n0 = bx * BN;
    const int* rmapA = nullptr; const int* kmap = nullptr;
    if (g.map_mode == 1) { g.M = min(g.M, g.dev_count[0]); rmapA = g.row_map; if (m0 >= g.M) return; }
    if (g.map_mode == 2) { g.K = min(g.K, g.dev_count[0]); kmap = g.row_map; }

    const int nslab_total = (g.K + BK - 1) / BK;
    int slab0 = 0, slab1 = nslab_total;
    if (g.splitk > 1) {
        const int sps = g.map_mode == 2 ? (nslab_total + g.splitk - 1) / g.splitk : g.slabs_per_split;
        slab0 = bz * sps;
        slab1 = min(nslab_total, slab0 + sps);
        if (slab0 >= slab1) return;
    }

    constexpr bool DUAL = TM * TN == 1;
    f32x16 acc[TM][TN], acc2[DUAL ? TM : 1][DUAL ? TN : 1];
#pragma unroll
    for (int a = 0; a < TM; ++a)
#pragma unroll
        for (int b = 0; b < TN; ++b)
#pragma unroll
            for (int r = 0; r < 16; ++r) { acc[a][b][r] = 0.f; if (DUAL) acc2[a][b][r] = 0.f; }

    f32x4 ra0[TileA::NV], rb0[TileB::NV], ra1[TileA::NV], rb1[TileB::NV];
    int pra[TileA::NV], prb[TileB::NV];
    const int* kl = nullptr;
    const int kbase = slab0 * BK;
    bool fast = !(g.flags & (1 << 21)) && g.vecA && g.vecB && g.M >= 4 && g.N >= 4 && g.K >= 4 && (g.K & 3) == 0 &&
                (!TA || (g.M & 3) == 0) && (TB || (g.N & 3) == 0);
    if (kmap) {
        const int need = (slab1 - slab0) * BK;
        if (fast && TA && !TB && g.kmap_lds >= need) {
            int* kls = reinterpret_cast<int*>(lds + (DB ? 2 : 1) * TILE_ELEMS);
            for (int i = tid; i < need; i += 256) kls[i] = kmap[min(kbase + i, g.K - 1)];
            __syncthreads();
            kl = kls;
        } else fast = false;
    }
    TileA::phys_rows(pra, g.M, m0, tid, rmapA, fast);
    TileB::phys_rows(prb, g.N, n0, tid, nullptr, fast);
    unsigned boa[TileA::NV], bob[TileB::NV];
    if (fast) { TileA::fast_bases(boa, g.lda, g.M, m0, tid, pra); TileB::fast_bases(bob, g.ldb, g.N, n0, tid, prb); }
    else {
#pragma unroll
        for (int i = 0; i < TileA::NV; ++i) boa[i] = 0;
#pragma unroll
        for (int i = 0; i < TileB::NV; ++i) bob[i] = 0;
    }
    auto gload = [&](f32x4 (&ra)[TileA::NV], f32x4 (&rb)[TileB::NV], int slab, auto fast_c) {
        if constexpr (decltype(fast_c)::value) {
            TileA::load_fast_b(ra, g.A, boa, g.lda, g.K, slab * BK, tid, kl, kbase);
            TileB::load_fast_b(rb, g.B, bob, g.ldb, g.K, slab * BK, tid, kl, kbase);
        } else {
            TileA::load(ra, g.A, g.lda, g.M, g.K, m0, slab * BK, g.vecA, tid, pra, kmap);
            TileB::load(rb, g.B, g.ldb, g.N, g.K, n0, slab * BK, g.vecB, tid, prb, kmap);
        }
    };
    auto multiply = [&](int slab, const __bf16* As, const __bf16* Bs) {
        const int nks = (g.K - slab * BK) > 16 ? 2 : 1;
#pragma unroll
        for (int ks = 0; ks < 2; ++ks) {
            if (ks < nks) {
                constexpr int NPL = SINGLE ? 1 : TWO ? 2 : 3;
                bf16x8 fa[TM][3], fb[TN][3];
#pragma unroll
                for (int a = 0; a < TM; ++a)
#pragma unroll
                    for (int p = 0; p < NPL; ++p) fa[a][p] = TileA::frag(As, p, wm * WM + a * 32, ks, lane);
#pragma unroll
                for (int b = 0; b < TN; ++b)
#pragma unroll
                    for (int p = 0; p < NPL; ++p) fb[b][p] = TileB::frag(Bs, p, wn * WN + b * 32, ks, lane);
                if constexpr (SINGLE) {
#pragma unroll
                    for (int a = 0; a < TM; ++a)
#pragma unroll
                        for (int b = 0; b < TN; ++b)
                            acc[a][b] = __builtin_amdgcn_mfma_f32_32x32x16_bf16(fa[a][0], fb[b][0], acc[a][b], 0, 0, 0);
                } else if constexpr (TWO) {
#pragma unroll
                    for (int a = 0; a < TM; ++a)
// ... 367 lines not shown
template <int BM, int BN, int PL>
int launch_cfg(const GemmArgs& g, int ta, int tb, hipStream_t s) {
    if (!ta && tb) return launch_one<BM, BN, false, true, PL>(g, s);
    if (!ta && !tb) return launch_one<BM, BN, false, false, PL>(g, s);
    if (ta && !tb) return launch_one<BM, BN, true, false, PL>(g, s);
    if constexpr (PL != 0) return CAPHN_EINVAL;
    else return launch_one<BM, BN, true, true, 0>(g, s);
}

}

extern int g_tune_gemm_planes;
int g_tune_gemm_tile = 0;
int g_tune_gemm_single = 0;
int g_tune_gemm_order = 1;
int g_tune_gemm_xcd = 1;
int g_tune_gemm_waves = 0;
int g_tune_gemm_ws = 0;
int g_tune_gemm_db = 0;
int g_tune_gemm_fast = 1;
bool caphn_gemm_planes_ok(const GemmArgs& g, int ta, int tb) {
    bool pl = g_tune_gemm_planes && g.Ap && g.Bp && !(ta && tb) && (g.K % 8) == 0 && g.K >= 8 && (g.ldap % 8) == 0 && (g.ldbp % 8) == 0 &&
              (g.psa % 8) == 0 && (g.psb % 8) == 0 && caphn_aligned16(g.Ap) && caphn_aligned16(g.Bp);
    if (pl && ta && (((g.M + 7) & ~7) > g.ldap || g.M < 8)) pl = false;
    if (pl && !tb && (((g.N + 7) & ~7) > g.ldbp || g.N < 8)) pl = false;
    if (pl && g.map_mode == 2) {
        const int nslab = (g.K + 31) / 32, sk = g.splitk > 1 ? g.splitk : 1;
        if (!(ta && !tb) || ((nslab + sk - 1) / sk) * 32 > 4096) pl = false;
    }
    return pl;
}
template <int BM, int BN, bool TA, bool TB>
static int occ_one() {
    using TileA = TileS<BM, !TA>;
    using TileB = TileS<BN, TB>;
    int n = 0;
    if (hipOccupancyMaxActiveBlocksPerMultiprocessor(&n, reinterpret_cast<const void*>(gemm_bf16x3_kernel<BM, BN, TA, TB, 0>), 256,
                                                     sizeof(__bf16) * (TileA::ELEMS + TileB::ELEMS)) != hipSuccess) return -1;
    return n;
}
extern "C" int caphn_debug_gemm_occupancy(int ta, int tb, int tile) {
    if (tile == 128) return !ta && tb ? occ_one<128, 128, false, true>() : !ta ? occ_one<128, 128, false, false>() : !tb ? occ_one<128, 128, true, false>() : occ_one<128, 128, true, true>();
    return !ta && tb ? occ_one<64, 64, false, true>() : !ta ? occ_one<64, 64, false, false>() : !tb ? occ_one<64, 64, true, false>() : occ_one<64, 64, true, true>();
}
int caphn_gemm_bf16x3_launch(GemmArgs g, int ta, int tb, hipStream_t s) {
    if (g_tune_gemm_xcd) g.flags |= 1 << 20;
    g.kmap_lds = 0;
    if (g.map_mode == 2 && ta && !tb) {
        const int nslab = (g.K + 31) / 32, sk = g.splitk > 1 ? g.splitk : 1;
        const int ints = ((nslab + sk - 1) / sk) * 32;
        if (ints <= 4096) g.kmap_lds = ints;
    }
    if (!g_tune_gemm_fast) g.flags |= 1 << 21;
    {
        const double ea = ta ? (double)g.K * g.lda : (double)g.M * g.lda, eb = tb ? (double)g.N * g.ldb : (double)g.K * g.ldb;
        if (ea * 4.0 >= 4.0e9 || eb * 4.0 >= 4.0e9) g.flags |= 1 << 21;
    }
    if (g_tune_gemm_order != 0 && g.splitk <= 1) {
        const double abytes = 4.0 * (double)g.M * g.K, bbytes = 4.0 * (double)g.N * g.K, l2 = 3.0 * 1024 * 1024;
        if (g_tune_gemm_order == 2 || (bbytes > l2 && abytes < bbytes)) g.flags |= 1 << 22;
    }
    long tiles128 = (long)((g.M + 127) / 128) * ((g.N + 127) / 128) * g.splitk;
    if (g.K < 512) tiles128 = 0;
    if (g_tune_gemm_tile == 64) tiles128 = 0; else if (g_tune_gemm_tile == 128) tiles128 = 1 << 20;
    const bool pl = caphn_gemm_planes_ok(g, ta, tb);
    if (!pl && g_tune_gemm_single == 0 && g_tune_gemm_tile == 0 && g_tune_gemm_ws == 0) {
        const int rc = caphn_gemm_kres_launch(g, ta, tb, s);
        if (rc != 1) return rc;
    }
    if (pl) {
        if (tiles128 >= 512) return launch_cfg<128, 128, 1>(g, ta, tb, s);
        return launch_cfg<64, 64, 1>(g, ta, tb, s);
    }
    if (g_tune_gemm_single == 1 && !(ta && tb)) {
        if (tiles128 >= 512) return launch_cfg<128, 128, 2>(g, ta, tb, s);
        return launch_cfg<64, 64, 2>(g, ta, tb, s);
    }
    if (g_tune_gemm_single == 2 && !(ta && tb)) {
        if (tiles128 >= 512) return launch_cfg<128, 128, 4>(g, ta, tb, s);
        return launch_cfg<64, 64, 4>(g, ta, tb, s);
    }
    if (g_tune_gemm_ws == 128 && !(ta && tb)) return launch_cfg<128, 128, 5>(g, ta, tb, s);
    if (g_tune_gemm_ws == 64 && !(ta && tb)) return launch_cfg<64, 64, 5>(g, ta, tb, s);
    if (tiles128 >= 512) return launch_cfg<128, 128, 0>(g, ta, tb, s);
    const int lay = (!ta && tb) ? 1 : (!ta && !tb) ? 2 : (ta && !tb) ? 4 : 0;
    if (g_tune_gemm_db & lay) return launch_cfg<64, 64, 3>(g, ta, tb, s);
    return launch_cfg<64, 64, 0>(g, ta, tb, s);
}

namespace {
struct SplitJobs { SplitJob j[8]; int n; long block0[9]; };
__global__ __launch_bounds__(256) void split3_kernel(SplitJobs jobs) {
    int ji = 0;
    for (int i = 1; i < jobs.n; ++i) if ((long)blockIdx.x >= jobs.block0[i]) ji = i;
    const SplitJob& J = jobs.j[ji];
    const int cpr = (J.cols + 7) >> 3;
    const long nchunk = (long)(J.rows + J.zero_rows) * cpr;
    const long stride = (jobs.block0[ji + 1] - jobs.block0[ji]) * 256;
    __bf16* dst = static_cast<__bf16*>(J.dst);
    const bool vec = (J.ld & 3) == 0 && caphn_aligned16_dev(J.src);
    for (long c = ((long)blockIdx.x - jobs.block0[ji]) * 256 + threadIdx.x; c < nchunk; c += stride) {
        const int row = (int)(c / cpr), col = (int)(c % cpr) * 8;
        const float* sp = J.src + (size_t)row * J.ld + col;
        f32x4 v0 = {0.f, 0.f, 0.f, 0.f}, v1 = {0.f, 0.f, 0.f, 0.f};
        if (row >= J.rows) { }
        else if (vec && col + 8 <= J.cols) { v0 = *reinterpret_cast<const f32x4*>(sp); v1 = *reinterpret_cast<const f32x4*>(sp + 4); }
// ... 33 lines not shown
```

hypernet-image-captioning_amd/csrc/hyper.hip:

```cpp
#include "common.h"
#include <algorithm>

namespace {

constexpr float LRELU = 0.01f;
__device__ __forceinline__ float lrelu(float v) { return v > 0.f ? v : LRELU * v; }
__device__ __forceinline__ float lrelu_grad(float post) { return post > 0.f ? 1.f : LRELU; }

struct GemvJob {
    const float* W; const float* b; const float* x; float* y;
    int rows, k, act, vec;
    int block0, nblocks;
    float* xcopy;
};
struct GemvJobs { GemvJob j[CAPHN_MAX_HEADS]; int n; };

template <int QMAX, int RB, bool NTL>
__device__ __forceinline__ void gemv_rows_wave(const GemvJob& J, int wave_g, int nwaves, int lane) {
    const int k4 = J.k >> 2;
    const f32x4* x4 = reinterpret_cast<const f32x4*>(J.x);
    f32x4 xr[QMAX];
#pragma unroll
    for (int q = 0; q < QMAX; ++q) {
        int c = lane + 64 * q;
// ... 781 lines not shown
        add(ws + W.dzb2, acts + L.a0, g->g_base_w2, d->he, d_mid(d));
        for (int i = 0; i < nh; ++i) add(ws + W.dz[i], acts + L.base, g->g_w1[i], d->k[i], d->he);
        if (oj.n) hipLaunchKernelGGL(outer_kernel, dim3((unsigned)b0), dim3(256), 0, s, oj);
        for (int i = 0; i < nh; ++i)
            if (g->g_w2[i]) {
                OuterJobs o2; o2.n = 1;
                OuterJob& J = o2.j[0];
                J.g = dtheta + toff[i]; J.a = acts + L.a[i]; J.out = g->g_w2[i]; J.rows = d->w[i]; J.k = d->k[i]; J.block0 = 0;
                long nb = ((long)J.rows * J.k + 1023) / 1024;
                hipLaunchKernelGGL(outer_kernel, dim3((unsigned)nb), dim3(256), 0, s, o2);
            }
    }
    return caphn_launch_status();
}

extern "C" int caphn_outer_f32(int rows, int k, const float* gv, const float* av, float* out, caphn_stream_t stream) {
    if (rows <= 0 || k <= 0 || !gv || !av || !out) return CAPHN_EINVAL;
    OuterJobs o2; o2.n = 1;
    OuterJob& J = o2.j[0];
    J.g = gv; J.a = av; J.out = out; J.rows = rows; J.k = k; J.block0 = 0;
    long nb = ((long)rows * k + 1023) / 1024;
    hipLaunchKernelGGL(outer_kernel, dim3((unsigned)nb), dim3(256), 0, static_cast<hipStream_t>(stream), o2);
    return caphn_launch_status();
}

extern int g_tune_adam;
extern int g_tune_gemm;
extern int g_tune_rec_rotate;
extern int g_tune_fork;
extern int g_tune_gemm_xcd;
extern int g_tune_gemm_fast;
extern int g_tune_gemm_planes;
extern int g_tune_rec_pair;
extern int g_tune_gemm_single;
extern int g_tune_gemm_tile;
extern int g_tune_deterministic;
extern int g_tune_adam_cap;
extern int g_tune_chain_main;
extern int g_tune_rec_cache;
extern int g_tune_splitk_target;
extern int g_tune_gemm_order;
extern int g_tune_branch_mask;
extern int g_tune_gemm_db;
extern int g_tune_gemm_ws;
extern int g_tune_adam_dense_cap;
extern int g_tune_sk_dhs, g_tune_sk_vocab_w;
extern int g_tune_join_chain;
extern int g_tune_gemm_kres;
extern int g_tune_gemm_waves;
extern int g_tune_hops;
extern int g_tune_vocab_order;
extern int g_det_vocab;
extern int g_tune_lazy_moments;
int caphn_rec_pair_debug_skip(int v);
int caphn_rec_pair_debug_opts(int v);
extern "C" int caphn_tune(int key, int value) {
    if (key == 0) { g_tune_gemv = value; return CAPHN_OK; }
    if (key == 1) { g_tune_adam = value; return CAPHN_OK; }
    if (key == 2) { g_tune_gemm = value; return CAPHN_OK; }
    if (key == 3) { g_tune_rec_rotate = value; return CAPHN_OK; }
    if (key == 4) { g_tune_fork = value; return CAPHN_OK; }
    if (key == 6) { g_tune_gemm_xcd = value; return CAPHN_OK; }
    if (key == 7) { g_tune_gemm_fast = value; return CAPHN_OK; }
    if (key == 8) { g_tune_gemm_planes = value; return CAPHN_OK; }
    if (key == 9) { g_tune_rec_pair = value; return CAPHN_OK; }
    if (key == 10) return caphn_rec_pair_debug_skip(value);
    if (key == 11) { g_tune_gemm_single = value; return CAPHN_OK; }
    if (key == 12) { g_tune_gemm_tile = value; return CAPHN_OK; }
    if (key == 13) { g_tune_deterministic = value > 0; g_det_vocab = value; return CAPHN_OK; }
    if (key == 21) { g_tune_vocab_order = value != 0; return CAPHN_OK; }
    if (key == 20) { if (value < 0 || value > 7) return CAPHN_EINVAL; g_tune_branch_mask = value; return CAPHN_OK; }
    if (key == 18) { if (value < 0 || value > 2) return CAPHN_EINVAL; g_tune_gemm_order = value; return CAPHN_OK; }
    if (key == 17) { if (value < 1 || value > 65536) return CAPHN_EINVAL; g_tune_splitk_target = value; return CAPHN_OK; }
    if (key == 16) { if (value < 0 || value > 2) return CAPHN_EINVAL; g_tune_rec_cache = value; return CAPHN_OK; }
    if (key == 15) { g_tune_chain_main = value != 0; return CAPHN_OK; }
    if (key == 26) { g_tune_hops = value != 0; return CAPHN_OK; }
    if (key == 27) { g_tune_hyper_tail = value != 0; return CAPHN_OK; }
    if (key == 28) { g_tune_acts_fused = value != 0; return CAPHN_OK; }
    if (key == 36) { g_tune_gemm_kres = value != 0; return CAPHN_OK; }
    if (key == 35) { g_tune_join_chain = value != 0; return CAPHN_OK; }
    if (key == 33) { if (value < 0 || value > 64) return CAPHN_EINVAL; g_tune_sk_dhs = value; return CAPHN_OK; }
    if (key == 34) { if (value < 0 || value > 64) return CAPHN_EINVAL; g_tune_sk_vocab_w = value; return CAPHN_OK; }
    if (key == 30) { if (value < 64 || value > 4096) return CAPHN_EINVAL; g_tune_vjp_blocks = value; return CAPHN_OK; }
    if (key == 31) { if (value < 64 || value > 65535) return CAPHN_EINVAL; g_tune_adam_dense_cap = value; return CAPHN_OK; }
    if (key == 29) { if (value != 0 && value != 64 && value != 128) return CAPHN_EINVAL; g_tune_gemm_ws = value; return CAPHN_OK; }
    if (key == 25) { if (value != 0 && value != 5 && value != 6) return CAPHN_EINVAL; g_tune_gemm_waves = value; return CAPHN_OK; }
    if (key == 24) return caphn_rec_pair_debug_opts(value);
    if (key == 23) { if (value < 0 || value > 7) return CAPHN_EINVAL; g_tune_gemm_db = value; return CAPHN_OK; }
    if (key == 22) { if (value < 1) return CAPHN_EINVAL; g_tune_xch_timeout = 100ll * value; return CAPHN_OK; }
    if (key == 37) { if (value < 1 || value > CAPHN_LAG_MAX + 1) return CAPHN_EINVAL; g_tune_lazy_moments = value; return CAPHN_OK; }
    if (key == 14) { if (value < 64 || value > 65535) return CAPHN_EINVAL; g_tune_adam_cap = value; return CAPHN_OK; }
    return CAPHN_EINVAL;
}
```

hypernet-image-captioning_amd/csrc/misc.hip:

```cpp
#include "common.h"
#include "gemm_internal.h"
#include <math.h>

namespace {
constexpr int RMAX = 8;


__global__ __launch_bounds__(256) void ce_count_kernel(int rows, const int64_t* __restrict__ tgt, int64_t ignore, float* nvalid) {
    __shared__ int cnt[4];
    int c = 0;
    for (int i = threadIdx.x; i < rows; i += 256) c += (tgt[i] != ignore);
    float cf = wave_sum((float)c);
    if ((threadIdx.x & 63) == 0) cnt[threadIdx.x >> 6] = (int)cf;
    __syncthreads();
    if (threadIdx.x == 0) nvalid[0] = (float)(cnt[0] + cnt[1] + cnt[2] + cnt[3]);
}

__global__ __launch_bounds__(256) void ce_row_kernel(int V, int ld, const float* logits, const int64_t* __restrict__ tgt,
                                                     int64_t ignore, const float* __restrict__ nvalid, const int* __restrict__ nvi,
                                                     float* dlogits, float* __restrict__ row_loss, int vec) {
    __shared__ float red[4];
    __shared__ float bc[2];
    const int row = blockIdx.x, tid = threadIdx.x;
    const float* x = logits + (size_t)row * ld;
// ... 142 lines not shown
        out[i] = x[i] + branch[i] * (p > 0.f ? caphn_keep_scale(seed, offset + i, p, inv_keep) : 1.f);
}

__global__ __launch_bounds__(256) void scale_kernel(size_t n, const float* __restrict__ x, const float* __restrict__ scale, float* __restrict__ out) {
    const float c = scale[0];
    const size_t stride = (size_t)gridDim.x * 256;
    for (size_t i = (size_t)blockIdx.x * 256 + threadIdx.x; i < n; i += stride) out[i] = x[i] * c;
}

__global__ __launch_bounds__(256) void lrelu_bwd_kernel(size_t n, const float* __restrict__ dy, const float* __restrict__ post, float* __restrict__ dx) {
    for (size_t i = (size_t)blockIdx.x * 256 + threadIdx.x; i < n; i += (size_t)gridDim.x * 256) dx[i] = dy[i] * (post[i] > 0.f ? 1.f : 0.01f);
}
__global__ __launch_bounds__(256) void axpy_kernel(size_t n, float alpha, const float* __restrict__ x, float* __restrict__ y) {
    const size_t stride = (size_t)gridDim.x * 256;
    for (size_t i = (size_t)blockIdx.x * 256 + threadIdx.x; i < n; i += stride) y[i] = fmaf(alpha, x[i], y[i]);
}

__global__ __launch_bounds__(256) void colsum_kernel(int M, int N, const float* __restrict__ A, int lda,
                                                     float* __restrict__ out, int rows_per) {
    __shared__ float red[4][65];
    const int c = threadIdx.x & 63, rl = threadIdx.x >> 6;
    const int n = blockIdx.x * 64 + c;
    const int m0 = blockIdx.y * rows_per, m1 = min(M, m0 + rows_per);
    float s0 = 0.f, s1 = 0.f;
    if (n < N) {
        int m = m0 + rl;
        for (; m + 4 < m1; m += 8) { s0 += A[(size_t)m * lda + n]; s1 += A[(size_t)(m + 4) * lda + n]; }
        if (m < m1) s0 += A[(size_t)m * lda + n];
    }
    red[rl][c] = s0 + s1;
    __syncthreads();
    if (rl == 0 && n < N) out[(size_t)blockIdx.y * N + n] = (red[0][c] + red[1][c]) + (red[2][c] + red[3][c]);
}
inline int colsum_slices(int M, int N) {
    const int colblocks = (N + 63) / 64;
    int S = 2048 / colblocks;
    if (S > (M + 31) / 32) S = (M + 31) / 32;
    if (S > 256) S = 256;
    if (S < 1) S = 1;
    return S;
}

__global__ __launch_bounds__(256) void embed_gather_kernel(int rows, int E, const float* __restrict__ table, const int64_t* __restrict__ idx, float* __restrict__ out) {
    const int r = blockIdx.x;
    const int64_t id = idx[r];
    for (int e = threadIdx.x; e < E; e += 256) out[(size_t)r * E + e] = id < 0 ? 0.f : table[(size_t)id * E + e];
}
__global__ __launch_bounds__(256) void embed_gather_strided_kernel(int rows, int E, const float* __restrict__ table, const int64_t* __restrict__ idx,
                                                                   int istride, float* __restrict__ out, int ostride) {
    const int r = blockIdx.x;
    const int64_t id = idx[(size_t)r * istride];
    for (int e = threadIdx.x; e < E; e += 256) out[(size_t)r * ostride + e] = id < 0 ? 0.f : table[(size_t)id * E + e];
}
__global__ __launch_bounds__(256) void embed_scatter_det_kernel(int rows, int E, int V, const float* __restrict__ g, const int64_t* __restrict__ idx,
                                                                float* __restrict__ tg) {
    const int v = blockIdx.x * 4 + (threadIdx.x >> 6), lane = threadIdx.x & 63;
    if (v >= V) return;
    bool any = false;
    for (int r0 = 0; r0 < rows; r0 += 64) {
        const int r = r0 + lane;
        const bool hit = r < rows && idx[r] == (int64_t)v;
        unsigned long long ball = __ballot(hit);
        while (ball) {
            const int b = __ffsll((long long)ball) - 1;
            ball &= ball - 1;
            const float* src = g + (size_t)(r0 + b) * E;
            for (int e = lane; e < E; e += 64) tg[(size_t)v * E + e] += src[e];
            any = true;
        }
    }
    (void)any;
}
__global__ __launch_bounds__(256) void embed_scatter_kernel(int rows, int E, const float* __restrict__ g, const int64_t* __restrict__ idx, float* __restrict__ tg) {
    const int r = blockIdx.x;
    const int64_t id = idx[r];
    if (id < 0) return;
    for (int e = threadIdx.x; e < E; e += 256) atomicAdd(&tg[(size_t)id * E + e], g[(size_t)r * E + e]);
}

constexpr int SUMSQ_CHUNK = 256 * 4 * 8;
__global__ __launch_bounds__(256) void sumsq_kernel(size_t n, const float* __restrict__ x, double* __restrict__ partial, int vec) {
    __shared__ double red[4];
    const size_t base = (size_t)blockIdx.x * SUMSQ_CHUNK;
    float s = 0.f;
    if (vec && base + SUMSQ_CHUNK <= n) {
        const f32x4* x4 = reinterpret_cast<const f32x4*>(x + base);
#pragma unroll
        for (int i = 0; i < 8; ++i) { f32x4 v = x4[threadIdx.x + 256 * i]; s += v[0] * v[0] + v[1] * v[1] + v[2] * v[2] + v[3] * v[3]; }
    } else {
        for (size_t i = base + threadIdx.x; i < n && i < base + SUMSQ_CHUNK; i += 256) s += x[i] * x[i];
    }
    double d = wave_sum_d((double)s);
    if ((threadIdx.x & 63) == 0) red[threadIdx.x >> 6] = d;
    __syncthreads();
    if (threadIdx.x == 0) partial[blockIdx.x] = red[0] + red[1] + red[2] + red[3];
}

constexpr int GRAM_CHUNKS = 64;
struct GramJob { const float* gfac; size_t ldg; const float* afac; size_t lda; int rows, k; };
struct GramJobs { GramJob j[CAPHN_MAX_HEADS]; int n; };
__global__ __launch_bounds__(256) void rank_gram_kernel(int R, GramJobs jobs, double* __restrict__ ws) {
    __shared__ double red[4];
    const int pair = blockIdx.x, job = blockIdx.y >> 1, which = blockIdx.y & 1;
    const GramJob& J = jobs.j[job];
    const int r = pair / R, s = pair % R;
    const float* u = which ? J.afac + (size_t)r * J.lda : J.gfac + (size_t)r * J.ldg;
    const float* v = which ? J.afac + (size_t)s * J.lda : J.gfac + (size_t)s * J.ldg;
    const int n = which ? J.k : J.rows;
    const int per = (n + GRAM_CHUNKS - 1) / GRAM_CHUNKS;
    const int i0 = blockIdx.z * per, i1 = min(n, i0 + per);
    if (i0 >= i1) return;
    double acc = 0.0;
    for (int i = i0 + threadIdx.x; i < i1; i += 256) acc += (double)u[i] * (double)v[i];
    acc = wave_sum_d(acc);
    if ((threadIdx.x & 63) == 0) red[threadIdx.x >> 6] = acc;
    __syncthreads();
    if (threadIdx.x == 0) atomicAdd(&ws[((size_t)job * 2 + which) * R * R + pair], red[0] + red[1] + red[2] + red[3]);
}
__global__ void rank_gram_finish_kernel(int R, int njobs, const double* __restrict__ ws, double* acc) {
    if (threadIdx.x == 0 && blockIdx.x == 0) {
        double t = 0.0;
        for (int j = 0; j < njobs; ++j)
            for (int i = 0; i < R * R; ++i) t += ws[((size_t)j * 2) * R * R + i] * ws[((size_t)j * 2 + 1) * R * R + i];
        acc[0] += t;
    }
}
__global__ __launch_bounds__(256) void clip_coef_kernel(int nparts, const double* __restrict__ partial, const double* extra,
                                                        double max_norm, double scale, float* coef_out) {
    __shared__ double red[4];
    double s = 0.0;
// ... 694 lines not shown
    return caphn_launch_status();
}
extern "C" int caphn_add_dropout_f32(size_t n, const float* x, const float* branch, float p, unsigned long long seed,
                                     unsigned long long offset, float* out, caphn_stream_t stream) {
    if (n == 0) return CAPHN_OK;
    if (!x || !branch || !out || !(p >= 0.f) || !(p < 1.f)) return CAPHN_EINVAL;
    size_t blocks = (n + 255) / 256;
    if (blocks > 4096) blocks = 4096;
    hipLaunchKernelGGL(add_dropout_kernel, dim3((unsigned)blocks), dim3(256), 0, static_cast<hipStream_t>(stream), n, p, 1.0f / (1.0f - p), seed,
                       offset, x, branch, out);
    return caphn_launch_status();
}
extern "C" int caphn_scale_f32(size_t n, const float* x, const float* scale_dev, float* out, caphn_stream_t stream) {
    if (n == 0) return CAPHN_OK;
    if (!x || !scale_dev || !out) return CAPHN_EINVAL;
    size_t blocks = (n + 255) / 256;
    if (blocks > 4096) blocks = 4096;
    hipLaunchKernelGGL(scale_kernel, dim3((unsigned)blocks), dim3(256), 0, static_cast<hipStream_t>(stream), n, x, scale_dev, out);
    return caphn_launch_status();
}
extern "C" int caphn_lrelu_bwd_f32(size_t n, const float* dy, const float* post, float* dx, caphn_stream_t stream) {
    if (n == 0) return CAPHN_OK;
    if (!dy || !post || !dx) return CAPHN_EINVAL;
    size_t blocks = (n + 255) / 256;
    if (blocks > 1024) blocks = 1024;
    hipLaunchKernelGGL(lrelu_bwd_kernel, dim3((unsigned)blocks), dim3(256), 0, static_cast<hipStream_t>(stream), n, dy, post, dx);
    return caphn_launch_status();
}
extern "C" int caphn_axpy_f32(size_t n, float alpha, const float* x, float* y, caphn_stream_t stream) {
    if (n == 0) return CAPHN_OK;
    if (!x || !y) return CAPHN_EINVAL;
    size_t blocks = (n + 255) / 256;
    if (blocks > 2048) blocks = 2048;
    hipLaunchKernelGGL(axpy_kernel, dim3((unsigned)blocks), dim3(256), 0, static_cast<hipStream_t>(stream), n, alpha, x, y);
    return caphn_launch_status();
}
extern "C" int caphn_embedding_gather(int rows, int E, const float* table, const int64_t* idx, float* out, caphn_stream_t stream) {
    if (rows <= 0 || E <= 0 || !table || !idx || !out) return CAPHN_EINVAL;
    hipLaunchKernelGGL(embed_gather_kernel, dim3(rows), dim3(256), 0, static_cast<hipStream_t>(stream), rows, E, table, idx, out);
    return caphn_launch_status();
}
int caphn_embedding_gather_strided(int rows, int E, const float* table, const int64_t* idx, int istride, float* out, int ostride, hipStream_t s) {
    if (rows <= 0 || E <= 0 || !table || !idx || !out) return CAPHN_EINVAL;
    hipLaunchKernelGGL(embed_gather_strided_kernel, dim3(rows), dim3(256), 0, s, rows, E, table, idx, istride, out, ostride);
    return caphn_launch_status();
}
extern int g_tune_deterministic;
int g_det_vocab = 0;
extern "C" int caphn_embedding_scatter_add_v(int rows, int E, int V, const float* g, const int64_t* idx, float* table_grad,
                                             caphn_stream_t stream) {
    if (rows <= 0 || E <= 0 || V <= 0 || !g || !idx || !table_grad) return CAPHN_EINVAL;
    if (g_tune_deterministic && rows > 1) {
        hipLaunchKernelGGL(embed_scatter_det_kernel, dim3((V + 3) / 4), dim3(256), 0, static_cast<hipStream_t>(stream), rows, E,
                           V, g, idx, table_grad);
        return caphn_launch_status();
    }
    hipLaunchKernelGGL(embed_scatter_kernel, dim3(rows), dim3(256), 0, static_cast<hipStream_t>(stream), rows, E, g, idx, table_grad);
    return caphn_launch_status();
}
extern "C" int caphn_embedding_scatter_add(int rows, int E, const float* g, const int64_t* idx, float* table_grad, caphn_stream_t stream) {
    if (rows <= 0 || E <= 0 || !g || !idx || !table_grad) return CAPHN_EINVAL;
    if (g_tune_deterministic && g_det_vocab > 0 && rows > 1) return caphn_embedding_scatter_add_v(rows, E, g_det_vocab, g, idx, table_grad, stream);
    hipLaunchKernelGGL(embed_scatter_kernel, dim3(rows), dim3(256), 0, static_cast<hipStream_t>(stream), rows, E, g, idx, table_grad);
    return caphn_launch_status();
}

extern "C" int caphn_sumsq_blocks(size_t n) { return (int)((n + SUMSQ_CHUNK - 1) / SUMSQ_CHUNK); }
extern "C" int caphn_sumsq_f32(size_t n, const float* x, double* partial, caphn_stream_t stream) {
    if (n == 0 || !x || !partial) return CAPHN_EINVAL;
    const int nb = caphn_sumsq_blocks(n);
    hipLaunchKernelGGL(sumsq_kernel, dim3(nb), dim3(256), 0, static_cast<hipStream_t>(stream), n, x, partial, (int)caphn_aligned16(x));
    return caphn_launch_status();
}
extern "C" int caphn_rank_sumsq_f32(int R, int rows, int k, const float* gfac, size_t ldg, const float* afac, size_t lda,
                                    double* acc, double* ws, caphn_stream_t stream) {
    if (R <= 0 || R > RMAX || rows <= 0 || k <= 0 || !gfac || !afac || !acc || !ws) return CAPHN_EINVAL;
    hipStream_t s = static_cast<hipStream_t>(stream);
    GramJobs jobs; jobs.n = 1;
    jobs.j[0] = GramJob{gfac, ldg, afac, lda, rows, k};
    if (hipMemsetAsync(ws, 0, sizeof(double) * 2 * R * R, s) != hipSuccess) return CAPHN_ELAUNCH;
    hipLaunchKernelGGL(rank_gram_kernel, dim3(R * R, 2, GRAM_CHUNKS), dim3(256), 0, s, R, jobs, ws);
    hipLaunchKernelGGL(rank_gram_finish_kernel, dim3(1), dim3(64), 0, s, R, 1, ws, acc);
    return caphn_launch_status();
}
extern "C" int caphn_rank_sumsq_multi_f32(int R, int n, const int* rows, const int* k, const float* const* gfac, const size_t* ldg,
                                          const float* const* afac, const size_t* lda, double* acc, double* ws,
                                          caphn_stream_t stream) {
    if (R <= 0 || R > RMAX || n <= 0 || n > CAPHN_MAX_HEADS || !rows || !k || !gfac || !ldg || !afac || !lda || !acc || !ws)
        return CAPHN_EINVAL;
    hipStream_t s = static_cast<hipStream_t>(stream);
    GramJobs jobs; jobs.n = n;
    for (int i = 0; i < n; ++i) {
        if (rows[i] <= 0 || k[i] <= 0 || !gfac[i] || !afac[i]) return CAPHN_EINVAL;
        jobs.j[i] = GramJob{gfac[i], ldg[i], afac[i], lda[i], rows[i], k[i]};
    }
    if (hipMemsetAsync(ws, 0, sizeof(double) * 2 * R * R * n, s) != hipSuccess) return CAPHN_ELAUNCH;
    hipLaunchKernelGGL(rank_gram_kernel, dim3(R * R, 2 * n, GRAM_CHUNKS), dim3(256), 0, s, R, jobs, ws);
    hipLaunchKernelGGL(rank_gram_finish_kernel, dim3(1), dim3(64), 0, s, R, n, ws, acc);
    return caphn_launch_status();
}
extern "C" size_t caphn_grad_norm_workspace_bytes(size_t n, int R, int njobs) {
    if (R <= 0 || R > RMAX || njobs < 0 || njobs > CAPHN_MAX_HEADS) return 0;
    return sizeof(double) * ((size_t)caphn_sumsq_blocks(n) + (size_t)njobs * 2 * R * R * NORM_CHUNKS);
}
extern "C" int caphn_grad_norm_coef(size_t n, const float* x, int R, int njobs, const int* rows, const int* k,
                                    const float* const* gfac, const size_t* ldg, const float* const* afac, const size_t* lda,
                                    double max_norm, double scale, float* coef_out, void* ws, caphn_stream_t stream) {
    if (n == 0 || !x || R <= 0 || R > RMAX || njobs < 0 || njobs > CAPHN_MAX_HEADS || !coef_out || !ws) return CAPHN_EINVAL;
    GramJobs jobs; jobs.n = njobs;
    for (int i = 0; i < njobs; ++i) {
        if (!rows || !k || !gfac || !ldg || !afac || !lda || rows[i] <= 0 || k[i] <= 0 || !gfac[i] || !afac[i]) return CAPHN_EINVAL;
        jobs.j[i] = GramJob{gfac[i], ldg[i], afac[i], lda[i], rows[i], k[i]};
    }
    const int nb_s = caphn_sumsq_blocks(n);
    const unsigned nb = (unsigned)nb_s + (unsigned)(njobs * 2 * R * R * NORM_CHUNKS);
    hipStream_t s = static_cast<hipStream_t>(stream);
// ... 333 lines not shown
```

hypernet-image-captioning_amd/csrc/recurrent_gru.hip:

```cpp
#include "common.h"
#include "decoder_internal.h"

namespace {

constexpr int NT = 1024;
#ifdef CAPHN_REC_PROFILE
#define PSTAMP(i) do { if (prof_on) { unsigned long long _n = clock64(); pc[i] += _n - plast; plast = _n; } } while (0)
#define PDECL const bool prof_on = (b == 0 && tid == 0 && a.prof != nullptr); \
    unsigned long long pc[8] = {0, 0, 0, 0, 0, 0, 0, 0}, plast = prof_on ? clock64() : 0
#define PFLUSH do { if (prof_on) for (int i = 0; i < 8; ++i) a.prof[i] = pc[i]; } while (0)
#else
#define PSTAMP(i) do { } while (0)
#define PDECL do { } while (0)
#define PFLUSH do { } while (0)
#endif

__device__ __forceinline__ void copy_to_lds(float* dst, const float* __restrict__ src, int n, int vec, int tid) {
    if (vec) {
        const f32x4* s4 = reinterpret_cast<const f32x4*>(src);
        f32x4* d4 = reinterpret_cast<f32x4*>(dst);
        for (int i = tid; i < (n >> 2); i += NT) d4[i] = s4[i];
    } else {
        for (int i = tid; i < n; i += NT) dst[i] = src[i];
    }
// ... 404 lines not shown

__global__ void attn_param_grads_kernel(AttnGradArgs a) {
    const int b = blockIdx.x, pc = blockIdx.y;
    const int P = a.P, H = a.H, T = a.T;
    const int p0 = pc * a.pchunk, p1 = min(P, p0 + a.pchunk);
    const size_t blk = (size_t)b * gridDim.y + pc;
    for (int k = threadIdx.x; k < H; k += blockDim.x) {
        const float vk = a.v_a[k];
        float dv = 0.f;
        for (int p = p0; p < p1; ++p) {
            const float w = a.Waf[((size_t)b * P + p) * H + k];
            float s = 0.f;
#pragma unroll 4
            for (int t = 0; t < T; ++t) {
                const float de = a.de[((size_t)b * T + t) * P + p];
                const float tv = caphn_tanh(w + a.uah[((size_t)b * T + t) * H + k]);
                s += de * (1.0f - tv * tv);
                dv += de * tv;
            }
            a.dWaf[((size_t)b * P + p) * H + k] = s * vk;
        }
        a.part[blk * (H + 1) + k] = dv;
    }
    if (threadIdx.x == 0) {
        float s = 0.f;
        for (int p = p0; p < p1; ++p)
            for (int t = 0; t < T; ++t) s += a.de[((size_t)b * T + t) * P + p];
        a.part[blk * (H + 1) + H] = s;
    }
}

__global__ __launch_bounds__(256) void dmean_kernel(int H, int F, const float* __restrict__ dh0, const float* __restrict__ Wh,
                                                    const float* __restrict__ dc0, const float* __restrict__ Wc, float* __restrict__ out) {
    extern __shared__ float dv[];
    const int b = blockIdx.x;
    for (int j = threadIdx.x; j < H; j += 256) { dv[j] = dh0[(size_t)b * H + j]; dv[H + j] = dc0 ? dc0[(size_t)b * H + j] : 0.f; }
    __syncthreads();
    for (int k = threadIdx.x; k < F; k += 256) {
        float s0 = 0.f, s1 = 0.f;
        int j = 0;
        for (; j + 8 <= H; j += 8) {
            float w[8], c[8];
#pragma unroll
            for (int u = 0; u < 8; ++u) { w[u] = Wh[(size_t)(j + u) * F + k]; c[u] = dc0 ? Wc[(size_t)(j + u) * F + k] : 0.f; }
#pragma unroll
            for (int u = 0; u < 8; ++u) { s0 += dv[j + u] * w[u]; s1 += dv[H + j + u] * c[u]; }
        }
        for (; j < H; ++j) { s0 += dv[j] * Wh[(size_t)j * F + k]; if (dc0) s1 += dv[H + j] * Wc[(size_t)j * F + k]; }
        out[(size_t)b * F + k] = s0 + s1;
    }
}

__global__ void ctx_kernel(int P, int F, int T, const float* __restrict__ alphas, const float* __restrict__ f, float* __restrict__ ctx,
                           int ldc) {
    const int b = blockIdx.x, t = blockIdx.y;
    const float* al = alphas + ((size_t)b * T + t) * P;
    for (int k = threadIdx.x; k < F; k += blockDim.x) {
        float s = 0.f;
        int p = 0;
        for (; p + 8 <= P; p += 8) {
            float v[8];
#pragma unroll
            for (int u = 0; u < 8; ++u) v[u] = f[((size_t)b * P + p + u) * F + k];
#pragma unroll
            for (int u = 0; u < 8; ++u) s += al[p + u] * v[u];
        }
        for (; p < P; ++p) s += al[p] * f[((size_t)b * P + p) * F + k];
        ctx[((size_t)b * T + t) * ldc + k] = s;
    }
}
__global__ void df_kernel(int P, int F, int T, const float* __restrict__ alphas, const float* __restrict__ dctx,
                          const float* __restrict__ dmean, const float* __restrict__ dmean2, float* __restrict__ df) {
    const int b = blockIdx.x, p = blockIdx.y;
    const float invP = 1.0f / (float)P;
    for (int k = threadIdx.x; k < F; k += blockDim.x) {
        float s = (dmean2 ? dmean[(size_t)b * F + k] + dmean2[(size_t)b * F + k] : dmean[(size_t)b * F + k]) * invP;
        int t = 0;
        for (; t + 8 <= T; t += 8) {
            float a[8], v[8];
#pragma unroll
            for (int u = 0; u < 8; ++u) { a[u] = alphas[((size_t)b * T + t + u) * P + p]; v[u] = dctx[((size_t)b * T + t + u) * F + k]; }
#pragma unroll
            for (int u = 0; u < 8; ++u) s += a[u] * v[u];
        }
        for (; t < T; ++t) s += alphas[((size_t)b * T + t) * P + p] * dctx[((size_t)b * T + t) * F + k];
        df[((size_t)b * P + p) * F + k] = s;
    }
}
__global__ __launch_bounds__(1024) void init_state_kernel(int P, int F, int H, const float* __restrict__ f,
                                                          const float* __restrict__ Wh, const float* __restrict__ bh,
                                                          const float* __restrict__ Wc, const float* __restrict__ bc,
                                                          float* __restrict__ meanf, float* __restrict__ h0, float* __restrict__ c0) {
    extern __shared__ float sm[];
    const int b = blockIdx.x, tid = threadIdx.x, lane = tid & 63, wave = tid >> 6;
    const int Fp = (F + 255) & ~255;
    for (int k0 = 0; k0 < F; k0 += 256) {
        const int k = k0 + (tid & 255), pl = tid >> 8;
        float s = 0.f;
        if (k < F) for (int p = pl; p < P; p += 4) s += f[((size_t)b * P + p) * F + k];
        sm[pl * Fp + k0 + (tid & 255)] = s;
    }
    __syncthreads();
    const float invP = 1.0f / (float)P;
    for (int k = tid; k < F; k += 1024) {
        const float m = ((sm[k] + sm[Fp + k]) + (sm[2 * Fp + k] + sm[3 * Fp + k])) * invP;
        sm[4 * Fp + k] = m;
        meanf[(size_t)b * F + k] = m;
    }
    __syncthreads();
    const float* mean = sm + 4 * Fp;
    for (int j = wave; j < H; j += 16) {
        float sh = 0.f, sc = 0.f;
        for (int k = lane; k < F; k += 64) {
            const float m = mean[k];
            sh += Wh[(size_t)j * F + k] * m;
            if (Wc) sc += Wc[(size_t)j * F + k] * m;
        }
        sh = wave_sum(sh);
        if (Wc) sc = wave_sum(sc);
        if (lane == 0) {
            h0[(size_t)b * H + j] = sh + bh[j];
            if (Wc) c0[(size_t)b * H + j] = sc + bc[j];
        }
    }
}
__global__ void mean_p_kernel(int P, int F, const float* __restrict__ f, float* __restrict__ out) {
    const int b = blockIdx.x;
    const float invP = 1.0f / (float)P;
    for (int k = threadIdx.x; k < F; k += blockDim.x) {
        float s = 0.f;
        for (int p = 0; p < P; ++p) s += f[((size_t)b * P + p) * F + k];
        out[(size_t)b * F + k] = s * invP;
    }
}

constexpr size_t LDS_LIMIT = 160 * 1024;
bool g_attr_set[64];
int ensure_lds_attr() {
// ... 12 lines not shown

static int kg_groups(int H) { return H >= NT ? 1 : NT / H; }
size_t caphn_rec_fwd_lds_bytes(int P, int H, int NG, int RG) {
    const size_t Ppad = (P + 63) & ~63;
    return sizeof(float) * ((size_t)RG * P * H + 4 * (size_t)H + (size_t)NG * H + Ppad + (size_t)kg_groups(H) * NG * H);
}
size_t caphn_rec_bwd_lds_bytes(int P, int H, int NG, int RG) {
    const size_t Ppad = (P + 63) & ~63;
    const int CH = (H % 4 == 0) ? 4 : 1;
    const int nch = (H + CH - 1) / CH;
    const int nch_eff = nch < NT ? nch : NT;
    int nsl = NT / nch_eff;
    if (kg_groups(H) > nsl) nsl = kg_groups(H);
    const int nsl1 = NT / (H < NT ? H : NT);
    if (nsl1 > nsl) nsl = nsl1;
    return sizeof(float) * ((size_t)RG * P * H + 5 * (size_t)H + 2 * (size_t)NG * H + 2 * Ppad + (size_t)nsl * H);
}
int caphn_rec_resident_gates(int P, int H, int NG) {
    for (int rg = NG; rg >= 0; --rg)
        if (caphn_rec_fwd_lds_bytes(P, H, NG, rg) <= LDS_LIMIT && caphn_rec_bwd_lds_bytes(P, H, NG, rg) <= LDS_LIMIT) return rg;
    return -1;
}

int caphn_launch_rec_fwd(const RecFwdArgs& a, bool lstm, hipStream_t s) {
    const size_t lds = caphn_rec_fwd_lds_bytes(a.P, a.H, lstm ? 4 : 3, a.RG);
    if (lds > LDS_LIMIT) return CAPHN_ELIMIT;
    int rc = ensure_lds_attr(); if (rc) return rc;
    if (lstm) hipLaunchKernelGGL(rec_attn_fwd_kernel<true>, dim3(a.B), dim3(NT), lds, s, a);
    else hipLaunchKernelGGL(rec_attn_fwd_kernel<false>, dim3(a.B), dim3(NT), lds, s, a);
    return caphn_launch_status();
}
int caphn_rec_bwd_groups(int P, int H) {
    if (H > NT) return 0;
    const int ng = NT / H;
    return (P + ng - 1) / ng <= PGM ? ng : 0;
}
int caphn_launch_rec_bwd(const RecBwdArgs& a, bool lstm, hipStream_t s) {
    if (a.dWaf && (!a.apart || caphn_rec_bwd_groups(a.P, a.H) == 0)) return CAPHN_EINVAL;
    const size_t lds = caphn_rec_bwd_lds_bytes(a.P, a.H, lstm ? 4 : 3, a.RG);
    if (lds > LDS_LIMIT) return CAPHN_ELIMIT;
    int rc = ensure_lds_attr(); if (rc) return rc;
    if (lstm) hipLaunchKernelGGL(rec_attn_bwd_kernel<true>, dim3(a.B), dim3(NT), lds, s, a);
    else hipLaunchKernelGGL(rec_attn_bwd_kernel<false>, dim3(a.B), dim3(NT), lds, s, a);
    return caphn_launch_status();
}
int caphn_launch_attn_param_grads(const AttnGradArgs& a, int B, int npc, hipStream_t s) {
    hipLaunchKernelGGL(attn_param_grads_kernel, dim3(B, npc), dim3(a.H >= 192 ? 256 : 64), 0, s, a);
    return caphn_launch_status();
}
int caphn_launch_dmean(int B, int H, int F, const float* dh0, const float* Wh, const float* dc0, const float* Wc, float* out, hipStream_t s) {
    hipLaunchKernelGGL(dmean_kernel, dim3(B), dim3(256), sizeof(float) * 2 * H, s, H, F, dh0, Wh, dc0, Wc, out);
    return caphn_launch_status();
}
int caphn_launch_ctx(int B, int T, int P, int F, const float* alphas, const float* f, float* ctx, int ldc, hipStream_t s) {
    hipLaunchKernelGGL(ctx_kernel, dim3(B, T), dim3(F >= 192 ? 256 : 64), 0, s, P, F, T, alphas, f, ctx, ldc);
    return caphn_launch_status();
}
int caphn_launch_df(int B, int T, int P, int F, const float* alphas, const float* dctx, const float* dmean, float* df, hipStream_t s,
                    const float* dmean2) {
    hipLaunchKernelGGL(df_kernel, dim3(B, P), dim3(F >= 192 ? 256 : 64), 0, s, P, F, T, alphas, dctx, dmean, dmean2, df);
    return caphn_launch_status();
}
int caphn_launch_init_state(int B, int P, int F, int H, const float* f, const float* Wh, const float* bh, const float* Wc,
                            const float* bc, float* meanf, float* h0, float* c0, hipStream_t s) {
    const int Fp = (F + 255) & ~255;
    hipLaunchKernelGGL(init_state_kernel, dim3(B), dim3(1024), sizeof(float) * (4 * Fp + F), s, P, F, H, f, Wh, bh, Wc, bc, meanf, h0, c0);
    return caphn_launch_status();
}
int caphn_launch_mean_p(int B, int P, int F, const float* f, float* out, hipStream_t s) {
    hipLaunchKernelGGL(mean_p_kernel, dim3(B), dim3(F >= 192 ? 256 : 64), 0, s, P, F, f, out);
    return caphn_launch_status();
}
```

hypernet-image-captioning_amd/csrc/recurrent_pair.hip:

```cpp
#include "common.h"
#include "decoder_internal.h"
#include <atomic>

namespace {

constexpr int NT = 512;
#ifdef CAPHN_REC_PROFILE
#define PSTAMP(i) do { if (prof_on) { unsigned long long _n = clock64(); pc[i] += _n - plast; plast = _n; } } while (0)
#define PDECL const bool prof_on = (w == 0 && tid == 0 && a.prof != nullptr); \
    unsigned long long pc[8] = {0, 0, 0, 0, 0, 0, 0, 0}, plast = prof_on ? clock64() : 0
#define PFLUSH do { if (prof_on) for (int i = 0; i < 8; ++i) a.prof[i] = pc[i]; } while (0)
#else
#define PSTAMP(i) do { } while (0)
#define PDECL do { } while (0)
#define PFLUSH do { } while (0)
#endif

typedef unsigned long long u64;

__device__ int d_pair_opts = 0;
__device__ __forceinline__ void xsend(u64* slot, float v, unsigned tag, bool near = false) {
    const u64 bits = ((u64)tag << 32) | (u64)__float_as_uint(v);
    if (near) __hip_atomic_store(slot, bits, __ATOMIC_RELAXED, __HIP_MEMORY_SCOPE_WORKGROUP);
    else __hip_atomic_store(slot, bits, __ATOMIC_RELAXED, __HIP_MEMORY_SCOPE_AGENT);
// ... 448 lines not shown

template <bool LSTM, int TCR>
__global__ __launch_bounds__(NT) void rec_pair_bwd_kernel(RecBwdArgs a) {
    constexpr int NG = LSTM ? 4 : 3;
    constexpr int PGM = 10;
    constexpr int TU = 8;
    extern __shared__ __attribute__((aligned(16))) float lds[];
    const int w = blockIdx.x, tid = threadIdx.x, lane = tid & 63, wave = tid >> 6;
    const int b = (w & 7) + 8 * (w >> 4), hh = (w >> 3) & 1;
    if (b >= a.B) return;
    const int P = a.P, H = a.H, GH = NG * a.H, T = a.T, RG = a.RG;
    const int Ppad = (P + 63) & ~63;
    const HalfK hk = half_of(H, hh);
    const int k0 = hk.k0, nk = hk.nk, nkm = half_a(H);
    const int H4 = (H + 3) & ~3;
    const float* WPh = a.WP + (size_t)hh * (NG + 1) * nkm * a.wp_pitch;
    float* G_s = lds;
    float* dh_s = G_s + (size_t)P * RG * nkm;
    float* dc_s = dh_s + nkm;
    float* uah_s = dc_s + nkm;
    float* va_s = uah_s + nkm;
    float* duah_s = va_s + nkm;
    float* dgh_s = duah_s + nk;
    float* dgi_s = duah_s + (NG + 1) * nkm;
    float* dal_s = dgi_s + NG * nkm;
    float* al_s = dal_s + Ppad;
    float* dhp_s = al_s + Ppad;
    float* part_s = dhp_s + H4;
    float* Wc_s = part_s + (size_t)a.part_rows * H4;

    u64* xmine = a.xch + (size_t)w * xch_stride(P, H);
    u64* xpart = a.xch + (size_t)(w ^ 8) * xch_stride(P, H);
    u64* xh_mine = xmine; u64* xe_mine = xmine + nkm;
    u64* xh_part = xpart; u64* xe_part = xpart + nkm;
    const unsigned ep = a.epoch << 16;
    const XCtl xc{a.err, a.xlimit};
    const bool mute = d_skip_xrecv == 2 && hh == 1;
    const bool near = partner_is_near(xmine + xch_ctl(P, H), xpart + xch_ctl(P, H), ep | 0xFFFFu, a.err, a.xlimit, tid, reinterpret_cast<int*>(dal_s));

    const float* Gb = a.G + (size_t)b * P * GH;
    const int vecS = a.vecS && (nk % 4 == 0) && (k0 % 4 == 0);
    if (vecS) {
        const int n4 = nk >> 2;
        for (int i = tid; i < P * RG * n4; i += NT) {
            const int c = i % n4, pq = i / n4, q = pq % RG, p = pq / RG;
            reinterpret_cast<f32x4*>(G_s + (size_t)pq * nk)[c] = reinterpret_cast<const f32x4*>(Gb + (size_t)p * GH + q * H + k0)[c];
        }
    } else {
        for (int i = tid; i < P * RG * nk; i += NT) {
            const int kk = i % nk, pq = i / nk, q = pq % RG, p = pq / RG;
            G_s[(size_t)pq * nk + kk] = Gb[(size_t)p * GH + q * H + k0 + kk];
        }
    }
    const int bt0 = a.t0, bt1 = a.t1 > 0 ? a.t1 : T;
    for (int kk = tid; kk < nk; kk += NT) {
        dh_s[kk] = 0.f; va_s[kk] = a.v_a[k0 + kk];
        dc_s[kk] = (LSTM && bt1 < T) ? a.dc0[(size_t)b * H + k0 + kk] : 0.f;
    }
    const float* Waf_b = a.Waf + (size_t)b * P * H;
    const int CH = (H % 4) == 0 ? 4 : 1;
    const KG m = kg_map(tid, nk);
    const int NR = (NG + 1) * nk;
    __syncthreads();
    const bool fuse = a.dWaf != nullptr && m.g >= 0;
    float dw[PGM];
#pragma unroll
    for (int i = 0; i < PGM; ++i) dw[i] = 0.f;
    float wafr[PGM];
#pragma unroll
    for (int i = 0; i < PGM; ++i) { const int p = m.g + i * m.ng; wafr[i] = (fuse && p < P) ? Waf_b[p * H + k0 + m.k] : 0.f; }
    float dva = 0.f, dbva = 0.f;
    PDECL;

    f32x4 wreg[TCR > 0 ? TCR : 1];
    const int tc_nch = (H + 3) / 4, tc_nsl = NT / (tc_nch < NT ? tc_nch : NT);
    const int tc_chunk = tid % tc_nch, tc_slice = tid / tc_nch;
    if constexpr (TCR > 0) {
#pragma unroll
        for (int u = 0; u < TCR; ++u) {
            const int r = a.wc_rows + tc_slice + u * tc_nsl;
            wreg[u] = (tc_slice < tc_nsl && r < NR) ? *reinterpret_cast<const f32x4*>(WPh + (size_t)r * a.wp_pitch + tc_chunk * 4)
                                                     : f32x4{0.f, 0.f, 0.f, 0.f};
        }
    }
    const float* dvec_s = duah_s;
    auto tmatvec = [&](int cb, int ce) {
        if constexpr (TCR > 0) {
            if (tc_slice < tc_nsl) {
                float acc[4] = {0.f, 0.f, 0.f, 0.f};
                for (int r = tc_slice; r < a.wc_rows;) {
                    f32x4 wv[4]; float dj[4];
#pragma unroll
                    for (int u = 0; u < 4; ++u) {
                        wv[u] = *reinterpret_cast<const f32x4*>(Wc_s + (size_t)r * H + tc_chunk * 4);
                        dj[u] = dvec_s[r];
                        r += tc_nsl;
                    }
#pragma unroll
                    for (int u = 0; u < 4; ++u) { acc[0] += wv[u][0] * dj[u]; acc[1] += wv[u][1] * dj[u]; acc[2] += wv[u][2] * dj[u]; acc[3] += wv[u][3] * dj[u]; }
                }
#pragma unroll
                for (int u0 = 0; u0 < TCR; u0 += 8) {
                    float dj[8];
#pragma unroll
                    for (int u = 0; u < 8; ++u) { const int r = a.wc_rows + tc_slice + (u0 + u) * tc_nsl; dj[u] = (u0 + u < TCR && r < NR) ? dvec_s[r] : 0.f; }
#pragma unroll
                    for (int u = 0; u < 8; ++u)
                        if (u0 + u < TCR) { const f32x4 w = wreg[u0 + u]; acc[0] += w[0] * dj[u]; acc[1] += w[1] * dj[u]; acc[2] += w[2] * dj[u]; acc[3] += w[3] * dj[u]; }
                }
                *reinterpret_cast<f32x4*>(part_s + (size_t)tc_slice * H4 + tc_chunk * 4) = f32x4{acc[0], acc[1], acc[2], acc[3]};
// ... 33 lines not shown
                while (r < NR) {
                    const float* rp[TU]; float dj[TU];
#pragma unroll
                    for (int u = 0; u < TU; ++u) {
                        const bool ok = r < NR;
                        rp[u] = col + (size_t)(ok ? r : 0) * a.wp_pitch;
                        dj[u] = ok ? dvec_s[r] : 0.f;
                        r += nsl;
                    }
                    if (CH == 4) {
                        f32x4 wv[TU];
#pragma unroll
                        for (int u = 0; u < TU; ++u) wv[u] = *reinterpret_cast<const f32x4*>(rp[u]);
#pragma unroll
                        for (int u = 0; u < TU; ++u) { acc[0] += wv[u][0] * dj[u]; acc[1] += wv[u][1] * dj[u]; acc[2] += wv[u][2] * dj[u]; acc[3] += wv[u][3] * dj[u]; }
                    } else {
#pragma unroll
                        for (int u = 0; u < TU; ++u) acc[0] += rp[u][0] * dj[u];
                    }
                }
                if (CH == 4) *reinterpret_cast<f32x4*>(part_s + (size_t)slice * H4 + c * 4) = f32x4{acc[0], acc[1], acc[2], acc[3]};
                else part_s[(size_t)slice * H4 + c] = acc[0];
            }
        }
        __syncthreads();
        for (int j = tid; j < ncol; j += NT) {
            float sum = 0.f;
            for (int sl = 0; sl < nsl; ++sl) sum += part_s[(size_t)sl * H4 + j];
            dhp_s[cb + j] = sum;
        }
        __syncthreads();
    };
    if (a.wc_rows > 0) {
        const int n4 = H >> 2;
        for (int idx = tid; idx < a.wc_rows * n4; idx += NT) {
            const int r = idx / n4, c = idx - r * n4;
            reinterpret_cast<f32x4*>(Wc_s)[idx] = reinterpret_cast<const f32x4*>(WPh + (size_t)r * a.wp_pitch)[c];
        }
        __syncthreads();
    }
    const bool pfk = nk <= NT && P <= NT;
    float pf[8] = {0.f, 0.f, 0.f, 0.f, 0.f, 0.f, 0.f, 0.f}, pfa = 0.f;
    auto prefetch = [&](int t) {
        const size_t bt = (size_t)b * T + t;
        if (tid < P) pfa = a.alphas[bt * P + tid];
        if (tid < nk) {
            const int k = k0 + tid;
            pf[0] = a.dHs[bt * H + k]; pf[1] = a.uah[bt * H + k];
            pf[2] = a.gates[bt * GH + k]; pf[3] = a.gates[bt * GH + H + k]; pf[4] = a.gates[bt * GH + 2 * H + k];
            if (LSTM) { pf[5] = a.gates[bt * GH + (3 % NG) * H + k]; pf[6] = a.Cprev[bt * H + k]; pf[7] = a.Cs[bt * H + k]; }
            else { pf[5] = a.hn[bt * H + k]; pf[6] = a.Hprev[bt * H + k]; }
        }
    };
    if (pfk) prefetch(bt1 - 1);

    for (int t = bt1 - 1; t >= bt0; --t) {
        const size_t bt = (size_t)b * T + t;
        if (pfk) { if (tid < P) al_s[tid] = pfa; }
        else for (int p = tid; p < P; p += NT) al_s[p] = a.alphas[bt * P + p];
        for (int kk = tid; kk < nk; kk += NT) {
            const int k = k0 + kk;
            float dh = dh_s[kk] + (pfk ? pf[0] : a.dHs[bt * H + k]);
            if (a.drop_p > 0.f) dh *= caphn_keep_scale(a.drop_seed, (unsigned long long)bt * H + k, a.drop_p, 1.0f / (1.0f - a.drop_p));
            uah_s[kk] = pfk ? pf[1] : a.uah[bt * H + k];
            if (LSTM) {
                const float gi = pfk ? pf[2] : a.gates[bt * GH + k], gf = pfk ? pf[3] : a.gates[bt * GH + H + k];
                const float gg = pfk ? pf[4] : a.gates[bt * GH + 2 * H + k];
                const float go = pfk ? pf[5] : a.gates[bt * GH + (3 % NG) * H + k];
                const float cp = pfk ? pf[6] : a.Cprev[bt * H + k];
                const float tc = caphn_tanh(pfk ? pf[7] : a.Cs[bt * H + k]);
                const float d_o = dh * tc;
                const float dc = dc_s[kk] + dh * go * (1.0f - tc * tc);
                const float dip = dc * gg * gi * (1.0f - gi);
                const float dfp = dc * cp * gf * (1.0f - gf);
                const float dgp = dc * gi * (1.0f - gg * gg);
                const float dop = d_o * go * (1.0f - go);
                dc_s[kk] = dc * gf;
                dh_s[kk] = 0.f;
                dgi_s[kk] = dip; dgi_s[nk + kk] = dfp; dgi_s[2 * nk + kk] = dgp; dgi_s[(3 % NG) * nk + kk] = dop;
                dgh_s[kk] = dip; dgh_s[nk + kk] = dfp; dgh_s[2 * nk + kk] = dgp; dgh_s[(3 % NG) * nk + kk] = dop;
                a.dgi[bt * GH + k] = dip; a.dgi[bt * GH + H + k] = dfp; a.dgi[bt * GH + 2 * H + k] = dgp;
                a.dgi[bt * GH + (3 % NG) * H + k] = dop;
            } else {
                const float r = pfk ? pf[2] : a.gates[bt * GH + k], z = pfk ? pf[3] : a.gates[bt * GH + H + k];
                const float n = pfk ? pf[4] : a.gates[bt * GH + 2 * H + k];
                const float hnv = pfk ? pf[5] : a.hn[bt * H + k], hp = pfk ? pf[6] : a.Hprev[bt * H + k];
                const float dn = dh * (1.0f - z);
                const float dz = dh * (hp - n);
                const float dnp = dn * (1.0f - n * n);
                const float drp = dnp * hnv * r * (1.0f - r);
                const float dzp = dz * z * (1.0f - z);
                dh_s[kk] = dh * z;
                dgi_s[kk] = drp; dgi_s[nk + kk] = dzp; dgi_s[2 * nk + kk] = dnp;
                dgh_s[kk] = drp; dgh_s[nk + kk] = dzp; dgh_s[2 * nk + kk] = dnp * r;
                a.dgi[bt * GH + k] = drp; a.dgi[bt * GH + H + k] = dzp; a.dgi[bt * GH + 2 * H + k] = dnp;
                a.dgh[bt * GH + k] = drp; a.dgh[bt * GH + H + k] = dzp; a.dgh[bt * GH + 2 * H + k] = dnp * r;
            }
        }
        if (pfk && t > bt0) prefetch(t - 1);
        __syncthreads();
        PSTAMP(0);
        if (RG == NG && P <= 8 * (NT / 64) && nk <= 128) {
            float sp[8], dg[NG][2];
#pragma unroll
            for (int q = 0; q < NG; ++q)
#pragma unroll
                for (int c = 0; c < 2; ++c) { const int kk = lane + 64 * c; dg[q][c] = kk < nk ? dgi_s[q * nk + kk] : 0.f; }
// ... 357 lines not shown
```

include/caphn.h:

```cpp
#ifndef CAPHN_H
#define CAPHN_H
#include <stdint.h>
#include <stddef.h>

#ifdef __cplusplus
extern "C" {
#endif

typedef void* caphn_stream_t;

#define CAPHN_OK 0
#define CAPHN_EINVAL (-1)
#define CAPHN_ELAUNCH (-2)
#define CAPHN_ELIMIT (-3)
#define CAPHN_ETIMEOUT (-4)

int caphn_abi_version(void);
int caphn_device_error(int clear);
int caphn_device_arch(char* buf, int buflen);

#define CAPHN_GEMM_BIAS 1
#define CAPHN_GEMM_RELU 2
#define CAPHN_GEMM_ACCUM 4
#define CAPHN_GEMM_MASK 8
// ... 64 lines not shown
    int raw_features;
    int row_subset;
    int grads_zeroed;
    int precomputed;
    int layers;
    float dropout_p;
    unsigned long long dropout_seed;
    int logits_ld;
} caphn_decoder_dims;

#define CAPHN_MAX_DEC_LAYERS 4
typedef struct caphn_decoder_params {
    const float* fc0_w; const float* fc0_b;
    const float* fc2_w; const float* fc2_b;
    const float* embed_w;
    const float* out_w; const float* out_b;
    const float* Wa_w; const float* Wa_b;
    const float* Ua_w; const float* Ua_b;
    const float* va_w; const float* va_b;
    const float* inith_w; const float* inith_b;
    const float* w_ih; const float* w_hh;
    const float* b_ih; const float* b_hh;
    const float* initc_w; const float* initc_b;
    const float* lw_ih[CAPHN_MAX_DEC_LAYERS - 1]; const float* lw_hh[CAPHN_MAX_DEC_LAYERS - 1];
    const float* lb_ih[CAPHN_MAX_DEC_LAYERS - 1]; const float* lb_hh[CAPHN_MAX_DEC_LAYERS - 1];
} caphn_decoder_params;

typedef struct caphn_decoder_grads {
    float* fc0_w; float* fc0_b; float* fc2_w; float* fc2_b;
    float* embed_w;
    float* out_w; float* out_b;
    float* Wa_w; float* Wa_b; float* Ua_w; float* Ua_b; float* va_w; float* va_b;
    float* inith_w; float* inith_b;
    float* w_ih; float* w_hh; float* b_ih; float* b_hh;
    float* initc_w; float* initc_b;
    float* lw_ih[CAPHN_MAX_DEC_LAYERS - 1]; float* lw_hh[CAPHN_MAX_DEC_LAYERS - 1];
    float* lb_ih[CAPHN_MAX_DEC_LAYERS - 1]; float* lb_hh[CAPHN_MAX_DEC_LAYERS - 1];
} caphn_decoder_grads;

size_t caphn_decoder_workspace_bytes(const caphn_decoder_dims* d);
int caphn_decoder_forward(const caphn_decoder_dims* d, const caphn_decoder_params* p,
                          const float* features, const int64_t* captions,
                          float* logits, float* alphas, void* ws, caphn_stream_t stream);
int caphn_decoder_precompute(const caphn_decoder_dims* d, const caphn_decoder_params* p, const float* features,
                             const int64_t* captions , void* ws, caphn_stream_t stream);
int caphn_decoder_inputs(const caphn_decoder_dims* d, const caphn_decoder_params* p, const int64_t* captions, void* ws,
                         caphn_stream_t stream);
int caphn_decoder_lookup(const caphn_decoder_dims* d, const caphn_decoder_params* p, const int64_t* captions, void* ws,
                         caphn_stream_t stream);
typedef struct caphn_pair_pack { float* wp; int H, HA, pitch, hrows; } caphn_pair_pack;
int caphn_decoder_pair_prep(const caphn_decoder_dims* d, const caphn_decoder_params* p, void* ws, caphn_stream_t stream);
int caphn_decoder_pair_pack_desc(const caphn_decoder_dims* d, void* ws, caphn_pair_pack* out);
const int* caphn_decoder_rowcount_ptr(const caphn_decoder_dims* d, void* ws);
int caphn_decoder_prepare_rows(const caphn_decoder_dims* d, const int64_t* targets, int64_t ignore_index,
                               void* ws, caphn_stream_t stream);
unsigned long long* caphn_decoder_profile_ptr(const caphn_decoder_dims* d, void* ws);
int caphn_decoder_forward_sampled(const caphn_decoder_dims* d, const caphn_decoder_params* p,
                                  const float* features, const int64_t* captions,
                                  const unsigned char* use_sampling,
                                  float* logits, float* alphas, void* ws, caphn_stream_t stream);
int caphn_decoder_forward_sampled_train(const caphn_decoder_dims* d, const caphn_decoder_params* p,
                                        const float* features, const int64_t* captions,
                                        const unsigned char* use_sampling,
                                        float* logits, float* alphas, void* ws, caphn_stream_t stream);
int caphn_decoder_backward(const caphn_decoder_dims* d, const caphn_decoder_params* p,
                           const float* features, const int64_t* captions,
                           float* dlogits, const float* dalphas,
                           const caphn_decoder_grads* g, void* ws, caphn_stream_t stream);

int caphn_decoder_hyper_backward(const caphn_decoder_dims* d, const caphn_decoder_params* p,
                                 const float* features, const int64_t* captions,
                                 float* dlogits, const float* dalphas,
                                 const caphn_decoder_grads* g, void* ws,
                                 const caphn_hyper_desc* hd, const float* acts, const caphn_hyper_grads* hg, void* hyper_ws,
                                 caphn_stream_t stream);

#define CAPHN_MS_DTHETA 0
#define CAPHN_MS_VOCAB 1
#define CAPHN_MS_EMBED 2
#define CAPHN_MS_HYPER 3
#define CAPHN_MS_COUNT 4
int caphn_decoder_backward_milestone(int which, caphn_stream_t waiter);

typedef struct {
    int n_images, beam, max_steps;
    int zero_pad_rule, lookup_first;
    int64_t first_token, end_token;
} caphn_search_cfg;
size_t caphn_decoder_search_workspace_bytes(const caphn_decoder_dims* d, const caphn_search_cfg* c);
int caphn_decoder_search_begin(const caphn_decoder_dims* d, const caphn_decoder_params* p, const caphn_search_cfg* c,
                               const float* features, void* ws, void* search_ws, caphn_stream_t stream);
int caphn_decoder_search_steps(const caphn_decoder_dims* d, const caphn_decoder_params* p, const caphn_search_cfg* c,
                               int step0, int nsteps, float* alphas, void* ws, void* search_ws, caphn_stream_t stream);
int caphn_decoder_search_result(const caphn_decoder_dims* d, const caphn_search_cfg* c, int steps_done, void* ws, void* search_ws,
                                int64_t* seqs, int* lengths, float* scores, int* finished, int* n_active,
                                caphn_stream_t stream);

#define CAPHN_MAX_LAYERS 4
typedef struct caphn_plain_dims { int B, T, E, H, V, L, cell; } caphn_plain_dims;
typedef struct caphn_plain_params {
    const float* embed_w; const float* out_w; const float* out_b;
    const float* w_ih[CAPHN_MAX_LAYERS]; const float* w_hh[CAPHN_MAX_LAYERS];
    const float* b_ih[CAPHN_MAX_LAYERS]; const float* b_hh[CAPHN_MAX_LAYERS];
} caphn_plain_params;
typedef struct caphn_plain_grads {
    float* embed_w; float* out_w; float* out_b;
// ... 133 lines not shown
```

Baseline: 89930 images/s.

## Skip dead timesteps past each caption's last valid target in decoder backward

Computes a per-sample live_end (last non-ignored target step) and a compacted step map alongside the existing valid-row map. The backward pass then uses this to trim the recurrent pair backward loop, the ctx/df kernels, the weight-gradient GEMMs, the dXe/dctx GEMM (merged into one mapped GEMM on an interleaved pitch) and the embedding scatter to live steps only. This targets wasted work on padded timesteps after a caption ends, whose gradients should be zero anyway. It adds a serial per-sample scan in the single-block row-prep kernel and relies on padded steps contributing nothing to gradients.

Result: faster. 94300 images/s, median of 6 (+4.9%).

```diff
diff --git a/hypernet-image-captioning_amd/caphn/_lib.py b/hypernet-image-captioning_amd/caphn/_lib.py
--- a/hypernet-image-captioning_amd/caphn/_lib.py
+++ b/hypernet-image-captioning_amd/caphn/_lib.py
@@ -166,6 +166,7 @@
     "caphn_cross_entropy_finish": (C.c_int, [C.c_int, c_fp, c_fp, c_fp, c_fp]),
     "caphn_decoder_profile_ptr": (C.c_void_p, [C.POINTER(DecoderDims), c_fp]),
     "caphn_decoder_rowcount_ptr": (C.c_void_p, [C.POINTER(DecoderDims), c_fp]),
+    "caphn_decoder_livemap_ptr": (C.c_void_p, [C.POINTER(DecoderDims), c_fp, C.c_int]),
     "caphn_cross_entropy_fwd_bwd": (C.c_int, [C.c_int, C.c_int, c_fp, c_fp, C.c_int64, c_fp, c_fp, C.c_int, c_fp, c_fp]),
     "caphn_embedding_gather": (C.c_int, [C.c_int, C.c_int, c_fp, c_fp, c_fp, c_fp]),
     "caphn_embedding_scatter_add": (C.c_int, [C.c_int, C.c_int, c_fp, c_fp, c_fp, c_fp]),
diff --git a/hypernet-image-captioning_amd/caphn/ops.py b/hypernet-image-captioning_amd/caphn/ops.py
--- a/hypernet-image-captioning_amd/caphn/ops.py
+++ b/hypernet-image-captioning_amd/caphn/ops.py
@@ -598,6 +598,11 @@
     return int(L.load().caphn_decoder_rowcount_ptr(C.byref(cd), C.c_void_p(ws.data_ptr())) or 0)
 
 
+def decoder_livemap_ptr(dims: DecDims, ws: torch.Tensor, which: int) -> int:
+    cd = dims.c()
+    return int(L.load().caphn_decoder_livemap_ptr(C.byref(cd), C.c_void_p(ws.data_ptr()), which) or 0)
+
+
 def embedding_gather(table: torch.Tensor, idx: torch.Tensor) -> torch.Tensor:
     lib = L.load()
     rows, E = idx.numel(), table.shape[1]
diff --git a/hypernet-image-captioning_amd/csrc/decoder.hip b/hypernet-image-captioning_amd/csrc/decoder.hip
--- a/hypernet-image-captioning_amd/csrc/decoder.hip
+++ b/hypernet-image-captioning_amd/csrc/decoder.hip
@@ -15,6 +15,7 @@
 int g_tune_hops = 0;
 int g_tune_fork = 4;
 int g_tune_join_chain = 0;
+int g_tune_live_steps = 2;
 int g_tune_sk_dhs = 0, g_tune_sk_vocab_w = 0;
 #define RUN(x) do { int _rc = (x); if (_rc != CAPHN_OK) return _rc; } while (0)
 
@@ -136,6 +137,8 @@
 struct Ws {
     size_t Y1, f, meanf, h0, c0, Waf, G, Xe, Xg, Hs, Hprev, gates, hn, Cs, Cprev, uah, alphas, idx;
     size_t dHs, dgi, dgh, duah, de, dh0, dc0, ctx, dctx, dXe, dWaf, dmeanf, df, dY1, apart, vtmp, colws, colws_s[3], prof, rowmap;
+    size_t stepmap, liveend;
+    int dxpitch;
     size_t xch, xch_floats;
     size_t wp;
     size_t H0s, dH0, h0L, dcarry, tgi, tgh, tmpA, tmpB;
@@ -151,6 +154,7 @@
 }
 
 inline size_t up4(size_t v) { return (v + 3) & ~(size_t)3; }
+inline bool ctx_live(const caphn_decoder_dims* d) { return d->row_subset && g_tune_live_steps > 0 && g_tune_gemm == 1; }
 
 inline Ws layout(const caphn_decoder_dims* d) {
     Ws w;
@@ -168,8 +172,8 @@
     w.uah = take(B * T * H); w.alphas = take(B * T * P); w.idx = take(2 * B * T);
     w.dHs = take(B * T * H); w.dgi = take(B * T * NG * H); w.dgh = take(lstm ? 0 : B * T * NG * H); w.duah = take(B * T * H);
     w.de = take(B * T * P); w.dh0 = take(B * H); w.dc0 = take(lstm ? B * H : 0);
-    w.ctx = w.Xe + E; w.dctx = take(raw ? 0 : B * T * F);
-    w.dXe = take(B * T * E); w.dWaf = take(B * P * H); w.dmeanf = take(raw ? 0 : 2 * B * F); w.df = take(raw ? 0 : B * P * F);
+    w.ctx = w.Xe + E; w.dxpitch = (int)(raw ? E : E + F);
+    w.dXe = take(B * T * (size_t)w.dxpitch); w.dctx = w.dXe + E; w.dWaf = take(B * P * H); w.dmeanf = take(raw ? 0 : 2 * B * F); w.df = take(raw ? 0 : B * P * F);
     w.dY1 = take(raw ? 0 : B * P * F);
     w.pchunk = 1; w.npc = (int)((P + w.pchunk - 1) / w.pchunk);
     const size_t arows = std::max<size_t>(std::max<size_t>(w.npc, (size_t)caphn_rec_bwd_groups((int)P, (int)H)),
@@ -191,6 +195,8 @@
     }
     w.prof = take(64);
     w.rowmap = take(B * T + 4);
+    w.stepmap = take(B * T + 4);
+    w.liveend = take(B);
     w.xch_floats = caphn_rec_pair_xch_bytes((int)B, (int)P, (int)H) / sizeof(float);
     w.xch = take(2 * w.xch_floats);
     o = (o + 31) & ~(size_t)31;
@@ -211,28 +217,38 @@
     return w;
 }
 
-__global__ __launch_bounds__(1024) void valid_rows_kernel(int n, const int64_t* __restrict__ tgt, int64_t ignore, int* __restrict__ map) {
-    __shared__ int wsum[16];
-    __shared__ int base_s;
+__global__ __launch_bounds__(1024) void valid_rows_kernel(int n, int T, const int64_t* __restrict__ tgt, int64_t ignore, int* __restrict__ map,
+                                                          int* __restrict__ live_end, int* __restrict__ smap) {
+    __shared__ int wsum[16], wsum2[16];
+    __shared__ int base_s, base2_s;
     const int tid = threadIdx.x, lane = tid & 63, wave = tid >> 6;
-    if (tid == 0) base_s = 0;
+    if (tid == 0) { base_s = 0; base2_s = 0; }
+    const int B = n / T;
+    for (int b = tid; b < B; b += 1024) {
+        int le = 0;
+        for (int t = 0; t < T; ++t) le = tgt[(size_t)b * T + t] != ignore ? t + 1 : le;
+        live_end[b] = le;
+    }
     __syncthreads();
     for (int c0 = 0; c0 < n; c0 += 1024) {
         const int i = c0 + tid;
         const int v = (i < n && tgt[i] != ignore) ? 1 : 0;
-        const unsigned long long ball = __ballot(v);
-        const int before = __popcll(ball & ((1ull << lane) - 1ull));
-        if (lane == 0) wsum[wave] = __popcll(ball);
+        const int v2 = (i < n && (i % T) < live_end[i / T]) ? 1 : 0;
+        const unsigned long long ball = __ballot(v), ball2 = __ballot(v2);
+        const unsigned long long below = (1ull << lane) - 1ull;
+        const int before = __popcll(ball & below), before2 = __popcll(ball2 & below);
+        if (lane == 0) { wsum[wave] = __popcll(ball); wsum2[wave] = __popcll(ball2); }
         __syncthreads();
-        int woff = 0, tot = 0;
-        for (int q = 0; q < 16; ++q) { if (q < wave) woff += wsum[q]; tot += wsum[q]; }
-        const int base = base_s;
+        int woff = 0, tot = 0, woff2 = 0, tot2 = 0;
+        for (int q = 0; q < 16; ++q) { if (q < wave) { woff += wsum[q]; woff2 += wsum2[q]; } tot += wsum[q]; tot2 += wsum2[q]; }
+        const int base = base_s, base2 = base2_s;
         if (v) map[4 + base + woff + before] = i;
+        if (v2) smap[4 + base2 + woff2 + before2] = i;
         __syncthreads();
-        if (tid == 0) base_s = base + tot;
+        if (tid == 0) { base_s = base + tot; base2_s = base2 + tot2; }
         __syncthreads();
     }
-    if (tid == 0) map[0] = base_s;
+    if (tid == 0) { map[0] = base_s; smap[0] = base2_s; }
 }
 
 __global__ void copy2_kernel(const float* __restrict__ src, int n, float* __restrict__ a, float* __restrict__ b) {
@@ -303,9 +319,9 @@
 }
 
 inline int wgrad_bias(int M, int N, int K, const float* A, int lda, const float* B, int ldb, float* dW, int ldc, float* db,
-                      const int* rowmap, void* cws, hipStream_t s, bool prezeroed) {
+                      const int* rowmap, void* cws, hipStream_t s, bool prezeroed, bool vocab = false) {
     int sk = pick_splitk(M, N, K);
-    if (rowmap && g_tune_sk_vocab_w > 0 && !g_tune_deterministic) sk = g_tune_sk_vocab_w;
+    if (vocab && rowmap && g_tune_sk_vocab_w > 0 && !g_tune_deterministic) sk = g_tune_sk_vocab_w;
     return caphn_gemm_tn_colsum(M, N, K, A, lda, B, ldb, dW, ldc, db, sk, rowmap, cws, prezeroed, s);
 }
 
@@ -419,6 +435,12 @@
     return reinterpret_cast<const int*>(static_cast<float*>(ws_) + layout(d).rowmap);
 }
 
+extern "C" const int* caphn_decoder_livemap_ptr(const caphn_decoder_dims* d, void* ws_, int which) {
+    if (!dims_ok(d) || !ws_ || which < 0 || which > 1) return nullptr;
+    const Ws w = layout(d);
+    return reinterpret_cast<const int*>(static_cast<float*>(ws_) + (which == 0 ? w.liveend : w.stepmap));
+}
+
 extern "C" unsigned long long* caphn_decoder_profile_ptr(const caphn_decoder_dims* d, void* ws_) {
     if (!dims_ok(d) || !ws_) return nullptr;
     return reinterpret_cast<unsigned long long*>(static_cast<float*>(ws_) + layout(d).prof);
@@ -428,8 +450,10 @@
                                           void* ws_, caphn_stream_t stream) {
     if (!dims_ok(d) || !targets || !ws_) return CAPHN_EINVAL;
     const Ws w = layout(d);
-    hipLaunchKernelGGL(valid_rows_kernel, dim3(1), dim3(1024), 0, static_cast<hipStream_t>(stream), d->B * d->T, targets,
-                       ignore_index, reinterpret_cast<int*>(static_cast<float*>(ws_) + w.rowmap));
+    float* ws = static_cast<float*>(ws_);
+    hipLaunchKernelGGL(valid_rows_kernel, dim3(1), dim3(1024), 0, static_cast<hipStream_t>(stream), d->B * d->T, d->T, targets,
+                       ignore_index, reinterpret_cast<int*>(ws + w.rowmap), reinterpret_cast<int*>(ws + w.liveend),
+                       reinterpret_cast<int*>(ws + w.stepmap));
     return caphn_launch_status();
 }
 
@@ -560,7 +584,8 @@
                               reinterpret_cast<const int*>(ws + w.rowmap) + 4, reinterpret_cast<const int*>(ws + w.rowmap), 1, s));
     else
         RUN(caphn_gemm_f32(0, 1, BT, V, H, ws + w.Hs, H, p->out_w, H, logits, LV, p->out_b, nullptr, 0, CAPHN_GEMM_BIAS, 1, s));
-    if (pc & 32) RUN(caphn_launch_ctx(B, T, P, F, ws + w.alphas, f, ws + w.ctx, EF, s));
+    if (pc & 32) RUN(caphn_launch_ctx(B, T, P, F, ws + w.alphas, f, ws + w.ctx, EF, s,
+                                      ctx_live(d) ? reinterpret_cast<const int*>(ws + w.liveend) : nullptr));
     if (alphas)
         if (hipMemcpyAsync(alphas, ws + w.alphas, sizeof(float) * (size_t)BT * P, hipMemcpyDeviceToDevice, s) != hipSuccess)
             return CAPHN_ELAUNCH;
@@ -623,6 +648,13 @@
     void* cw0 = ws + w.colws_s[0]; void* cw1 = ws + w.colws_s[1]; void* cw2 = ws + w.colws_s[2];
 
     const int* rmap = d->row_subset ? reinterpret_cast<const int*>(ws + w.rowmap) : nullptr;
+    const int ang_ = w.L1 > 0 ? 0 : pair ? caphn_rec_pair_bwd_groups(P, H) : caphn_rec_bwd_groups(P, H);
+    int lmode = (d->row_subset && !dalphas && g_tune_gemm == 1) ? g_tune_live_steps : 0;
+    if (lmode == 2 && !(pair && w.L1 == 0 && !lstm && ang_ > 0)) lmode = 1;
+    const int* smap = lmode > 0 ? reinterpret_cast<const int*>(ws + w.stepmap) : nullptr;
+    const int* live_end = lmode > 0 ? reinterpret_cast<const int*>(ws + w.liveend) : nullptr;
+    const int DXP = w.dxpitch;
+    const bool ctx_left = (d->precomputed & 32) && !(lmode == 0 && ctx_live(d));
     const int LV = d->logits_ld > 0 ? d->logits_ld : V;
     const int fork_mode = g_tune_fork == 4 ? (pair ? 2 : 1) : g_tune_fork;
     const bool late = fork_mode != 2;
@@ -630,7 +662,7 @@
     const bool wg_first = !late && g_tune_vocab_order == 0;
     if (wg_first) {
         RUN(sd.forkto(0));
-        RUN(wgrad_bias(V, H, BT, dlogits, LV, ws + w.Hs, H, g->out_w, H, g->out_b, rmap, cws, sd.s(0), gz));
+        RUN(wgrad_bias(V, H, BT, dlogits, LV, ws + w.Hs, H, g->out_w, H, g->out_b, rmap, cws, sd.s(0), gz, true));
         RUN(sd.milestone(CAPHN_MS_VOCAB, sd.s(0)));
     }
     const bool dhs_zero = (d->precomputed & 8) != 0;
@@ -643,14 +675,14 @@
     } else
     RUN(gemm_auto(0, 0, BT, H, V, dlogits, LV, p->out_w, H, ws + w.dHs, H, nullptr, 0, s, nullptr, 0, dhs_zero));
     if (!late && !wg_first) {
-        if (!(d->precomputed & 32) && sd.s(0) != s && sd.s(2) != s) {
+        if (!ctx_left && sd.s(0) != s && sd.s(2) != s) {
             RUN(sd.fork_many({0, 2}));
-            RUN(caphn_launch_ctx(B, T, P, F, ws + w.alphas, f, ws + w.ctx, EF, sd.s(2)));
+            RUN(caphn_launch_ctx(B, T, P, F, ws + w.alphas, f, ws + w.ctx, EF, sd.s(2), live_end));
             RUN(sd.record(5, sd.s(2)));
             ctx_side = true;
         } else
         RUN(sd.forkto(0));
-        RUN(wgrad_bias(V, H, BT, dlogits, LV, ws + w.Hs, H, g->out_w, H, g->out_b, rmap, cws, sd.s(0), gz));
+        RUN(wgrad_bias(V, H, BT, dlogits, LV, ws + w.Hs, H, g->out_w, H, g->out_b, rmap, cws, sd.s(0), gz, true));
         RUN(sd.milestone(CAPHN_MS_VOCAB, sd.s(0)));
     }
 
@@ -666,7 +698,7 @@
     a.prof = reinterpret_cast<unsigned long long*>(ws + w.prof) + 8;
     a.rotate = g_tune_rec_rotate;
     a.drop_p = d->dropout_p; a.drop_seed = d->dropout_seed;
-    const int ang = w.L1 > 0 ? 0 : pair ? caphn_rec_pair_bwd_groups(P, H) : caphn_rec_bwd_groups(P, H);
+    const int ang = ang_;
     if (ang > 0) { a.dWaf = ws + w.dWaf; a.apart = ws + w.apart; }
     if (w.L1 > 0) {
         RUN(caphn_zero_f32(ws + w.dcarry, (size_t)B * H, s));
@@ -682,6 +714,7 @@
         a.apart_rows = ang;
         a.WP = ws + w.wp; a.wp_pitch = caphn_rec_pair_pitch(H);
         if (!raw) { a.inith_w = p->inith_w; a.initc_w = lstm ? p->initc_w : nullptr; a.dmean_part = ws + w.dmeanf; a.F = F; }
+        if (lmode == 2) a.live_end = live_end;
         RUN(caphn_launch_rec_pair_bwd(a, lstm, s));
     } else
     RUN(caphn_launch_rec_bwd(a, lstm, s));
@@ -692,20 +725,24 @@
     const bool hold_big = late && !raw && fork_mode == 3;
     RUN(sd.fork_many({0, 1, 2}));
     if (late && !hold_big) {
-        RUN(wgrad_bias(V, H, BT, dlogits, LV, ws + w.Hs, H, g->out_w, H, g->out_b, rmap, cws, b0, gz));
+        RUN(wgrad_bias(V, H, BT, dlogits, LV, ws + w.Hs, H, g->out_w, H, g->out_b, rmap, cws, b0, gz, true));
         RUN(sd.milestone(CAPHN_MS_VOCAB, b0));
     }
     if (ctx_side) RUN(sd.wait(5, sT));
-    else if (!(d->precomputed & 32)) RUN(caphn_launch_ctx(B, T, P, F, ws + w.alphas, f, ws + w.ctx, EF, sT));
-    if (lstm) RUN(gemm_auto(1, 0, GH, EF, BT, dgi, GH, ws + w.Xe, EF, g->w_ih, EF, nullptr, 0, sT, nullptr, 0, gz));
-    else RUN(wgrad_bias(GH, EF, BT, dgi, GH, ws + w.Xe, EF, g->w_ih, EF, g->b_ih, nullptr, cw1, sT, gz));
-    RUN(wgrad_bias(GH, H, BT, dgh, GH, ws + w.Hprev, H, g->w_hh, H, g->b_hh, nullptr, cw2, b2, gz));
+    else if (!ctx_left) RUN(caphn_launch_ctx(B, T, P, F, ws + w.alphas, f, ws + w.ctx, EF, sT, live_end));
+    if (lstm) RUN(gemm_auto(1, 0, GH, EF, BT, dgi, GH, ws + w.Xe, EF, g->w_ih, EF, nullptr, 0, sT, smap, 2, gz));
+    else RUN(wgrad_bias(GH, EF, BT, dgi, GH, ws + w.Xe, EF, g->w_ih, EF, g->b_ih, smap, cw1, sT, gz));
+    RUN(wgrad_bias(GH, H, BT, dgh, GH, ws + w.Hprev, H, g->w_hh, H, g->b_hh, smap, cw2, b2, gz));
     if (lstm) RUN(caphn_colsum_f32(BT, GH, dgi, GH, g->b_ih, cw2, b2));
     RUN(sd.record(3, b2));
     hipStream_t se = late ? b2 : b0;
-    RUN(caphn_gemm_f32(0, 0, BT, E, GH, dgi, GH, p->w_ih, EF, ws + w.dXe, E, nullptr, nullptr, 0, 0, 1, se));
+    if (smap) {
+        RUN(caphn_gemm_mapped(0, 0, BT, DXP, GH, dgi, GH, p->w_ih, EF, ws + w.dXe, DXP, nullptr, 0, 1, smap + 4, smap, 1, sF));
+        RUN(sd.dep(sF, se, 1));
+    } else
+    RUN(caphn_gemm_f32(0, 0, BT, E, GH, dgi, GH, p->w_ih, EF, ws + w.dXe, DXP, nullptr, nullptr, 0, 0, 1, se));
     if (!gz) RUN(caphn_zero_f32(g->embed_w, (size_t)V * E, se));
-    RUN(caphn_embedding_scatter_add_v(BT, E, V, ws + w.dXe, idx, g->embed_w, se));
+    RUN(caphn_embedding_scatter_add_live(BT, E, V, ws + w.dXe, DXP, idx, g->embed_w, T, live_end, se));
     RUN(sd.milestone(CAPHN_MS_EMBED, se));
     RUN(sd.wait(3, sT));
     RUN(sd.milestone(CAPHN_MS_DTHETA, sT));
@@ -714,7 +751,7 @@
     }
     if (!hold_big) RUN(sd.milestone(CAPHN_MS_HYPER, sT));
     if (!raw) {
-        RUN(caphn_gemm_f32(0, 0, BT, F, GH, dgi, GH, p->w_ih + E, EF, ws + w.dctx, F, nullptr, nullptr, 0, 0, 1, sF));
+        if (!smap) RUN(caphn_gemm_f32(0, 0, BT, F, GH, dgi, GH, p->w_ih + E, EF, ws + w.dctx, DXP, nullptr, nullptr, 0, 0, 1, sF));
         if (!pair)
             RUN(caphn_launch_dmean(B, H, F, ws + w.dh0, p->inith_w, lstm ? ws + w.dc0 : nullptr, lstm ? p->initc_w : nullptr,
                                    ws + w.dmeanf, sF));
@@ -725,7 +762,7 @@
     ag.dWaf = ws + w.dWaf; ag.part = ws + w.apart;
     if (ang == 0) RUN(caphn_launch_attn_param_grads(ag, B, w.npc, sF));
     RUN(sd.record(2, sF));
-    RUN(wgrad_bias(H, H, BT, ws + w.duah, H, ws + w.Hprev, H, g->Ua_w, H, g->Ua_b, nullptr, cws, b0, gz));
+    RUN(wgrad_bias(H, H, BT, ws + w.duah, H, ws + w.Hprev, H, g->Ua_w, H, g->Ua_b, smap, cws, b0, gz));
     for (int l = 0; l < w.L1; ++l) {
         const int BS = B * (T + 1), G3 = 3 * H;
         RUN(wgrad_bias(G3, H, BS, ws + w.Ldgi[l], G3, ws + w.Lin[l], H, g->lw_ih[l], H, g->lb_ih[l], nullptr, cws, b0, gz));
@@ -734,12 +771,13 @@
     RUN(wgrad_bias(H, F, B, ws + w.dh0, H, ws + w.meanf, F, g->inith_w, F, g->inith_b, nullptr, cws, b0, gz));
     if (lstm) RUN(wgrad_bias(H, F, B, ws + w.dc0, H, ws + w.meanf, F, g->initc_w, F, g->initc_b, nullptr, cws, b0, gz));
     if (!raw) {
-        RUN(caphn_launch_df(B, T, P, F, ws + w.alphas, ws + w.dctx, ws + w.dmeanf, ws + w.df, sF, pair ? ws + w.dmeanf + (size_t)B * F : nullptr));
+        RUN(caphn_launch_df(B, T, P, F, ws + w.alphas, ws + w.dctx, ws + w.dmeanf, ws + w.df, sF, pair ? ws + w.dmeanf + (size_t)B * F : nullptr,
+                            DXP, live_end));
         RUN(caphn_gemm_f32(0, 0, BP, F, H, ws + w.dWaf, H, p->Wa_w, F, ws + w.df, F, nullptr, nullptr, 0, CAPHN_GEMM_ACCUM, 1, sF));
         RUN(sd.record(4, sF));
         if (hold_big) {
             RUN(sd.wait(4, b0));
-            RUN(wgrad_bias(V, H, BT, dlogits, LV, ws + w.Hs, H, g->out_w, H, g->out_b, rmap, cws, b0, gz));
+            RUN(wgrad_bias(V, H, BT, dlogits, LV, ws + w.Hs, H, g->out_w, H, g->out_b, rmap, cws, b0, gz, true));
             RUN(sd.milestone(CAPHN_MS_VOCAB, b0));
             if (hook) {
                 RUN(sd.wait(4, sT));
diff --git a/hypernet-image-captioning_amd/csrc/decoder_internal.h b/hypernet-image-captioning_amd/csrc/decoder_internal.h
--- a/hypernet-image-captioning_amd/csrc/decoder_internal.h
+++ b/hypernet-image-captioning_amd/csrc/decoder_internal.h
@@ -55,6 +55,7 @@
     const float* inith_w = nullptr; const float* initc_w = nullptr; float* dmean_part = nullptr; int F = 0;
     int part_rows = 0, wc_rows = 0;
     int t0 = 0, t1 = 0;
+    const int* live_end = nullptr;
 };
 struct AttnGradArgs {
     int T, P, H, pchunk;
@@ -100,9 +101,13 @@
 int caphn_launch_rec_pair_bwd(const RecBwdArgs& a, bool lstm, hipStream_t s);
 int caphn_rec_bwd_groups(int P, int H);
 int caphn_launch_attn_param_grads(const AttnGradArgs& a, int B, int npc, hipStream_t s);
-int caphn_launch_ctx(int B, int T, int P, int F, const float* alphas, const float* f, float* ctx, int ldc, hipStream_t s);
+int caphn_launch_ctx(int B, int T, int P, int F, const float* alphas, const float* f, float* ctx, int ldc, hipStream_t s,
+                     const int* live_end = nullptr);
 int caphn_launch_df(int B, int T, int P, int F, const float* alphas, const float* dctx, const float* dmean, float* df, hipStream_t s,
-                    const float* dmean2 = nullptr);
+                    const float* dmean2 = nullptr,
+                    int ldd = 0, const int* live_end = nullptr);
+int caphn_embedding_scatter_add_live(int rows, int E, int V, const float* g, int ldg, const int64_t* idx, float* table_grad, int T,
+                                     const int* live_end, hipStream_t s);
 int caphn_launch_dmean(int B, int H, int F, const float* dh0, const float* Wh, const float* dc0, const float* Wc, float* out, hipStream_t s);
 int caphn_launch_init_state(int B, int P, int F, int H, const float* f, const float* Wh, const float* bh, const float* Wc,
                             const float* bc, float* meanf, float* h0, float* c0, hipStream_t s);
diff --git a/hypernet-image-captioning_amd/csrc/gemm_bf16x3.hip b/hypernet-image-captioning_amd/csrc/gemm_bf16x3.hip
--- a/hypernet-image-captioning_amd/csrc/gemm_bf16x3.hip
+++ b/hypernet-image-captioning_amd/csrc/gemm_bf16x3.hip
@@ -20,6 +20,7 @@
 #endif
 
 extern int g_tune_gemm_waves;
+extern int g_tune_live_steps;
 namespace {
 
 constexpr int BK = 32;
@@ -294,7 +295,9 @@
     int pra[TileA::NV], prb[TileB::NV];
     const int* kl = nullptr;
     const int kbase = slab0 * BK;
-    bool fast = !(g.flags & (1 << 21)) && g.vecA && g.vecB && g.M >= 4 && g.N >= 4 && g.K >= 4 && (g.K & 3) == 0 &&
+    const bool k_any = TA && !TB && (g.flags & (1 << 23));
+    bool fast = !(g.flags & (1 << 21)) && g.vecA && g.vecB && g.M >= 4 && g.N >= 4 &&
+                (k_any ? g.K >= 1 : (g.K >= 4 && (g.K & 3) == 0)) &&
                 (!TA || (g.M & 3) == 0) && (TB || (g.N & 3) == 0);
     if (kmap) {
         const int need = (slab1 - slab0) * BK;
@@ -768,6 +771,7 @@
         if (ints <= 4096) g.kmap_lds = ints;
     }
     if (!g_tune_gemm_fast) g.flags |= 1 << 21;
+    if (g_tune_live_steps > 0 && ta && !tb) g.flags |= 1 << 23;
     {
         const double ea = ta ? (double)g.K * g.lda : (double)g.M * g.lda, eb = tb ? (double)g.N * g.ldb : (double)g.K * g.ldb;
         if (ea * 4.0 >= 4.0e9 || eb * 4.0 >= 4.0e9) g.flags |= 1 << 21;
diff --git a/hypernet-image-captioning_amd/csrc/hyper.hip b/hypernet-image-captioning_amd/csrc/hyper.hip
--- a/hypernet-image-captioning_amd/csrc/hyper.hip
+++ b/hypernet-image-captioning_amd/csrc/hyper.hip
@@ -857,6 +857,7 @@
 extern int g_tune_vocab_order;
 extern int g_det_vocab;
 extern int g_tune_lazy_moments;
+extern int g_tune_live_steps;
 int caphn_rec_pair_debug_skip(int v);
 int caphn_rec_pair_debug_opts(int v);
 extern "C" int caphn_tune(int key, int value) {
@@ -894,6 +895,7 @@
     if (key == 23) { if (value < 0 || value > 7) return CAPHN_EINVAL; g_tune_gemm_db = value; return CAPHN_OK; }
     if (key == 22) { if (value < 1) return CAPHN_EINVAL; g_tune_xch_timeout = 100ll * value; return CAPHN_OK; }
     if (key == 37) { if (value < 1 || value > CAPHN_LAG_MAX + 1) return CAPHN_EINVAL; g_tune_lazy_moments = value; return CAPHN_OK; }
+    if (key == 38) { if (value < 0 || value > 2) return CAPHN_EINVAL; g_tune_live_steps = value; return CAPHN_OK; }
     if (key == 14) { if (value < 64 || value > 65535) return CAPHN_EINVAL; g_tune_adam_cap = value; return CAPHN_OK; }
     return CAPHN_EINVAL;
 }
diff --git a/hypernet-image-captioning_amd/csrc/misc.hip b/hypernet-image-captioning_amd/csrc/misc.hip
--- a/hypernet-image-captioning_amd/csrc/misc.hip
+++ b/hypernet-image-captioning_amd/csrc/misc.hip
@@ -218,30 +218,32 @@
     const int64_t id = idx[(size_t)r * istride];
     for (int e = threadIdx.x; e < E; e += 256) out[(size_t)r * ostride + e] = id < 0 ? 0.f : table[(size_t)id * E + e];
 }
-__global__ __launch_bounds__(256) void embed_scatter_det_kernel(int rows, int E, int V, const float* __restrict__ g, const int64_t* __restrict__ idx,
-                                                                float* __restrict__ tg) {
+__global__ __launch_bounds__(256) void embed_scatter_det_kernel(int rows, int E, int V, const float* __restrict__ g, int ldg, const int64_t* __restrict__ idx,
+                                                                float* __restrict__ tg, int T, const int* __restrict__ live_end) {
     const int v = blockIdx.x * 4 + (threadIdx.x >> 6), lane = threadIdx.x & 63;
     if (v >= V) return;
     bool any = false;
     for (int r0 = 0; r0 < rows; r0 += 64) {
         const int r = r0 + lane;
-        const bool hit = r < rows && idx[r] == (int64_t)v;
+        const bool hit = r < rows && idx[r] == (int64_t)v && (!live_end || (r % T) < live_end[r / T]);
         unsigned long long ball = __ballot(hit);
         while (ball) {
             const int b = __ffsll((long long)ball) - 1;
             ball &= ball - 1;
-            const float* src = g + (size_t)(r0 + b) * E;
+            const float* src = g + (size_t)(r0 + b) * ldg;
             for (int e = lane; e < E; e += 64) tg[(size_t)v * E + e] += src[e];
             any = true;
         }
     }
     (void)any;
 }
-__global__ __launch_bounds__(256) void embed_scatter_kernel(int rows, int E, const float* __restrict__ g, const int64_t* __restrict__ idx, float* __restrict__ tg) {
+__global__ __launch_bounds__(256) void embed_scatter_kernel(int rows, int E, const float* __restrict__ g, int ldg, const int64_t* __restrict__ idx,
+                                                            float* __restrict__ tg, int T, const int* __restrict__ live_end) {
     const int r = blockIdx.x;
     const int64_t id = idx[r];
     if (id < 0) return;
-    for (int e = threadIdx.x; e < E; e += 256) atomicAdd(&tg[(size_t)id * E + e], g[(size_t)r * E + e]);
+    if (live_end && (r % T) >= live_end[r / T]) return;
+    for (int e = threadIdx.x; e < E; e += 256) atomicAdd(&tg[(size_t)id * E + e], g[(size_t)r * ldg + e]);
 }
 
 constexpr int SUMSQ_CHUNK = 256 * 4 * 8;
@@ -1042,16 +1044,25 @@
     if (rows <= 0 || E <= 0 || V <= 0 || !g || !idx || !table_grad) return CAPHN_EINVAL;
     if (g_tune_deterministic && rows > 1) {
         hipLaunchKernelGGL(embed_scatter_det_kernel, dim3((V + 3) / 4), dim3(256), 0, static_cast<hipStream_t>(stream), rows, E,
-                           V, g, idx, table_grad);
+                           V, g, E, idx, table_grad, 1, nullptr);
         return caphn_launch_status();
     }
-    hipLaunchKernelGGL(embed_scatter_kernel, dim3(rows), dim3(256), 0, static_cast<hipStream_t>(stream), rows, E, g, idx, table_grad);
+    hipLaunchKernelGGL(embed_scatter_kernel, dim3(rows), dim3(256), 0, static_cast<hipStream_t>(stream), rows, E, g, E, idx, table_grad, 1, nullptr);
+    return caphn_launch_status();
+}
+int caphn_embedding_scatter_add_live(int rows, int E, int V, const float* g, int ldg, const int64_t* idx, float* table_grad, int T,
+                                     const int* live_end, hipStream_t s) {
+    if (rows <= 0 || E <= 0 || V <= 0 || ldg < E || T <= 0 || !g || !idx || !table_grad) return CAPHN_EINVAL;
+    if (g_tune_deterministic && rows > 1)
+        hipLaunchKernelGGL(embed_scatter_det_kernel, dim3((V + 3) / 4), dim3(256), 0, s, rows, E, V, g, ldg, idx, table_grad, T, live_end);
+    else
+        hipLaunchKernelGGL(embed_scatter_kernel, dim3(rows), dim3(256), 0, s, rows, E, g, ldg, idx, table_grad, T, live_end);
     return caphn_launch_status();
 }
 extern "C" int caphn_embedding_scatter_add(int rows, int E, const float* g, const int64_t* idx, float* table_grad, caphn_stream_t stream) {
     if (rows <= 0 || E <= 0 || !g || !idx || !table_grad) return CAPHN_EINVAL;
     if (g_tune_deterministic && g_det_vocab > 0 && rows > 1) return caphn_embedding_scatter_add_v(rows, E, g_det_vocab, g, idx, table_grad, stream);
-    hipLaunchKernelGGL(embed_scatter_kernel, dim3(rows), dim3(256), 0, static_cast<hipStream_t>(stream), rows, E, g, idx, table_grad);
+    hipLaunchKernelGGL(embed_scatter_kernel, dim3(rows), dim3(256), 0, static_cast<hipStream_t>(stream), rows, E, g, E, idx, table_grad, 1, nullptr);
     return caphn_launch_status();
 }
 
diff --git a/hypernet-image-captioning_amd/csrc/recurrent_gru.hip b/hypernet-image-captioning_amd/csrc/recurrent_gru.hip
--- a/hypernet-image-captioning_amd/csrc/recurrent_gru.hip
+++ b/hypernet-image-captioning_amd/csrc/recurrent_gru.hip
@@ -480,8 +480,9 @@
 }
 
 __global__ void ctx_kernel(int P, int F, int T, const float* __restrict__ alphas, const float* __restrict__ f, float* __restrict__ ctx,
-                           int ldc) {
+                           int ldc, const int* __restrict__ live_end) {
     const int b = blockIdx.x, t = blockIdx.y;
+    if (live_end && t >= live_end[b]) return;
     const float* al = alphas + ((size_t)b * T + t) * P;
     for (int k = threadIdx.x; k < F; k += blockDim.x) {
         float s = 0.f;
@@ -497,9 +498,12 @@
         ctx[((size_t)b * T + t) * ldc + k] = s;
     }
 }
-__global__ void df_kernel(int P, int F, int T, const float* __restrict__ alphas, const float* __restrict__ dctx,
-                          const float* __restrict__ dmean, const float* __restrict__ dmean2, float* __restrict__ df) {
+__global__ void df_kernel(int P, int F, int T, const float* __restrict__ alphas, const float* __restrict__ dctx, int ldd,
+                          const float* __restrict__ dmean, const float* __restrict__ dmean2, float* __restrict__ df,
+                          const int* __restrict__ live_end) {
     const int b = blockIdx.x, p = blockIdx.y;
+    const int Tfull = T;
+    if (live_end) T = max(0, min(T, live_end[b]));
     const float invP = 1.0f / (float)P;
     for (int k = threadIdx.x; k < F; k += blockDim.x) {
         float s = (dmean2 ? dmean[(size_t)b * F + k] + dmean2[(size_t)b * F + k] : dmean[(size_t)b * F + k]) * invP;
@@ -507,11 +511,11 @@
         for (; t + 8 <= T; t += 8) {
             float a[8], v[8];
 #pragma unroll
-            for (int u = 0; u < 8; ++u) { a[u] = alphas[((size_t)b * T + t + u) * P + p]; v[u] = dctx[((size_t)b * T + t + u) * F + k]; }
+            for (int u = 0; u < 8; ++u) { a[u] = alphas[((size_t)b * Tfull + t + u) * P + p]; v[u] = dctx[((size_t)b * Tfull + t + u) * ldd + k]; }
 #pragma unroll
             for (int u = 0; u < 8; ++u) s += a[u] * v[u];
         }
-        for (; t < T; ++t) s += alphas[((size_t)b * T + t) * P + p] * dctx[((size_t)b * T + t) * F + k];
+        for (; t < T; ++t) s += alphas[((size_t)b * Tfull + t) * P + p] * dctx[((size_t)b * Tfull + t) * ldd + k];
         df[((size_t)b * P + p) * F + k] = s;
     }
 }
@@ -630,13 +634,15 @@
     hipLaunchKernelGGL(dmean_kernel, dim3(B), dim3(256), sizeof(float) * 2 * H, s, H, F, dh0, Wh, dc0, Wc, out);
     return caphn_launch_status();
 }
-int caphn_launch_ctx(int B, int T, int P, int F, const float* alphas, const float* f, float* ctx, int ldc, hipStream_t s) {
-    hipLaunchKernelGGL(ctx_kernel, dim3(B, T), dim3(F >= 192 ? 256 : 64), 0, s, P, F, T, alphas, f, ctx, ldc);
+int caphn_launch_ctx(int B, int T, int P, int F, const float* alphas, const float* f, float* ctx, int ldc, hipStream_t s,
+                     const int* live_end) {
+    hipLaunchKernelGGL(ctx_kernel, dim3(B, T), dim3(F >= 192 ? 256 : 64), 0, s, P, F, T, alphas, f, ctx, ldc, live_end);
     return caphn_launch_status();
 }
 int caphn_launch_df(int B, int T, int P, int F, const float* alphas, const float* dctx, const float* dmean, float* df, hipStream_t s,
-                    const float* dmean2) {
-    hipLaunchKernelGGL(df_kernel, dim3(B, P), dim3(F >= 192 ? 256 : 64), 0, s, P, F, T, alphas, dctx, dmean, dmean2, df);
+                    const float* dmean2, int ldd, const int* live_end) {
+    hipLaunchKernelGGL(df_kernel, dim3(B, P), dim3(F >= 192 ? 256 : 64), 0, s, P, F, T, alphas, dctx, ldd > 0 ? ldd : F, dmean, dmean2, df,
+                       live_end);
     return caphn_launch_status();
 }
 int caphn_launch_init_state(int B, int P, int F, int H, const float* f, const float* Wh, const float* bh, const float* Wc,
diff --git a/hypernet-image-captioning_amd/csrc/recurrent_pair.hip b/hypernet-image-captioning_amd/csrc/recurrent_pair.hip
--- a/hypernet-image-captioning_amd/csrc/recurrent_pair.hip
+++ b/hypernet-image-captioning_amd/csrc/recurrent_pair.hip
@@ -524,10 +524,13 @@
             G_s[(size_t)pq * nk + kk] = Gb[(size_t)p * GH + q * H + k0 + kk];
         }
     }
-    const int bt0 = a.t0, bt1 = a.t1 > 0 ? a.t1 : T;
+    const int bt1w = a.t1 > 0 ? a.t1 : T;
+    int bt1_ = bt1w;
+    if (a.live_end) bt1_ = max(a.t0, min(bt1_, a.live_end[b]));
+    const int bt0 = a.t0, bt1 = bt1_;
     for (int kk = tid; kk < nk; kk += NT) {
         dh_s[kk] = 0.f; va_s[kk] = a.v_a[k0 + kk];
-        dc_s[kk] = (LSTM && bt1 < T) ? a.dc0[(size_t)b * H + k0 + kk] : 0.f;
+        dc_s[kk] = (LSTM && bt1w < T) ? a.dc0[(size_t)b * H + k0 + kk] : 0.f;
     }
     const float* Waf_b = a.Waf + (size_t)b * P * H;
     const int CH = (H % 4) == 0 ? 4 : 1;
@@ -667,7 +670,7 @@
             else { pf[5] = a.hn[bt * H + k]; pf[6] = a.Hprev[bt * H + k]; }
         }
     };
-    if (pfk) prefetch(bt1 - 1);
+    if (pfk && bt1 > bt0) prefetch(bt1 - 1);
 
     for (int t = bt1 - 1; t >= bt0; --t) {
         const size_t bt = (size_t)b * T + t;
diff --git a/include/caphn.h b/include/caphn.h
--- a/include/caphn.h
+++ b/include/caphn.h
@@ -140,6 +140,7 @@
 int caphn_decoder_pair_prep(const caphn_decoder_dims* d, const caphn_decoder_params* p, void* ws, caphn_stream_t stream);
 int caphn_decoder_pair_pack_desc(const caphn_decoder_dims* d, void* ws, caphn_pair_pack* out);
 const int* caphn_decoder_rowcount_ptr(const caphn_decoder_dims* d, void* ws);
+const int* caphn_decoder_livemap_ptr(const caphn_decoder_dims* d, void* ws, int which);
 int caphn_decoder_prepare_rows(const caphn_decoder_dims* d, const int64_t* targets, int64_t ignore_index,
                                void* ws, caphn_stream_t stream);
 unsigned long long* caphn_decoder_profile_ptr(const caphn_decoder_dims* d, void* ws);
```
